# robotic-vision-lab/Edge-Informed-Contrast-Maximization

Measured on AMD Instinct MI355X. Metric: warped-events/sec/GPU + loss+grad eval ms, 1e6 events @ 346x260, higher is better.
Workload: dtype f32

## Files before the change

edge-informed-contrast-maximization_amd/csrc/eincm_api.hip:

```cpp
#include <hip/hip_runtime.h>
#include <hip/hip_ext.h>

#include <algorithm>
#include <array>
#include <chrono>
#include <cmath>
#include <cstdarg>
#include <cstdio>
#include <cstdlib>
#include <cstring>
#include <string>
#include <utility>
#include <vector>

#include "eincm.h"
#include "eincm_plan.h"
#include "eincm_kernels.hip.h"
#include "eincm_kernels_f64.hip.h"
#include "eincm_binning.hip.h"
#include "eincm_edges.hip.h"
#include "eincm_objectives.hip.h"
#include "eincm_splat_window.hip.h"
#include "eincm_canny.hip.h"
#include "eincm_preprocess.hip.h"
#include "eincm_gtflow.hip.h"
#include "eincm_dsec.hip.h"
#include "eincm_floweval.hip.h"
#include "eincm_bfgs.hip.h"
#include "eincm_lbfgs.hip.h"
#include "eincm_motion.hip.h"
#include "eincm_event_support.hip.h"
#include "eincm_event_filter.hip.h"
#include "eincm_event_scores.h"
#include "eincm_event_scores.hip.h"

using namespace eincm;

namespace {

thread_local std::string g_create_error;

struct Mem {
    struct Block { void* p; size_t bytes; };
    std::vector<Block> dev, pinned;
    size_t dev_bytes = 0, pinned_bytes = 0;

    template <typename T> hipError_t alloc_dev(T*& p, size_t n, bool zero = false) {
        p = nullptr;
        hipError_t e = hipMalloc(reinterpret_cast<void**>(&p), n * sizeof(T));
        if (e == hipSuccess && p && zero) e = hipMemset(p, 0, n * sizeof(T));
        return own(dev, dev_bytes, p, n * sizeof(T), e, hipFree);
    }
    template <typename T> hipError_t alloc_pinned(T*& p, size_t n, bool zero = false) {
        p = nullptr;
        const hipError_t e = hipHostMalloc(reinterpret_cast<void**>(&p), n * sizeof(T), hipHostMallocDefault);
        if (e == hipSuccess && p && zero) memset(p, 0, n * sizeof(T));
        return own(pinned, pinned_bytes, p, n * sizeof(T), e, hipHostFree);
    }
    void release(void* p) {
        if (!p) return;
        if (!drop(dev, dev_bytes, p, hipFree)) drop(pinned, pinned_bytes, p, hipHostFree);
    }
    void release_all() {
        for (const Block& b : dev) (void)hipFree(b.p);
        for (const Block& b : pinned) (void)hipHostFree(b.p);
        dev.clear(); pinned.clear();
        dev_bytes = pinned_bytes = 0;
    }

private:
    template <typename T> static hipError_t own(std::vector<Block>& v, size_t& total, T*& p, size_t bytes, hipError_t e, hipError_t (*free_fn)(void*)) {
        if (e != hipSuccess) { if (p) (void)free_fn(p); p = nullptr; return e; }
        if (p) { v.push_back(Block{p, bytes}); total += bytes; }
        return hipSuccess;
    }
    static bool drop(std::vector<Block>& v, size_t& total, void* p, hipError_t (*free_fn)(void*)) {
        for (size_t i = 0; i < v.size(); ++i)
            if (v[i].p == p) { (void)free_fn(p); total -= v[i].bytes; v.erase(v.begin() + i); return true; }
        return false;
    }
};

template <typename T, bool PINNED = false> struct Grow {
    T* p = nullptr;
    size_t n = 0;
};

struct StageArgs {
    int B, R; const int64_t* n_events;
    const int16_t* const* xs; const int16_t* const* ys; const double* const* ts; const double* const* edges; const double* edge_ts;
    uint32_t flags;
    const float* const* weights = nullptr;
};

struct StageScratch {
    std::vector<unsigned> cntmax; std::vector<double> dtmax;
    bool edge_ts_uploaded = false;
    std::vector<BinBlock> blks; std::vector<int32_t> win_blk; int32_t misc[4]; std::vector<double> mom;
    std::vector<uint32_t> sxy; std::vector<double> st; std::vector<float> ef; std::vector<float> sw;
    std::vector<int> ishift;
};

struct Flight {
    enum State { IDLE, FORWARD, LAUNCHED } state = IDLE;
    EvalPlan plan{};
    DevIo io{};
    const double* theta_dev = nullptr; ThetaArg targ{};
    int copy_mode = 0;
    int n_pieces = 0;
    size_t piece_len = 0;
    std::vector<uint8_t> theta_nan;
    bool timed_now = true;
    int ring_cur = 0;
    bool idle() const { return state == IDLE; }
    bool launched() const { return state == LAUNCHED; }
    void land() { state = IDLE; io = DevIo{}; }
    void abandon(hipStream_t stream) { (void)hipStreamSynchronize(stream); land(); }
};

}

struct eincm_ctx : PlanCtx {
    int device = 0;
    int maxR = 0, maxB = 0;
    int64_t maxN = 0;
    uint32_t cflags = 0;
    hipStream_t stream = nullptr;
    std::string err;
    Mem mem;

    bool staged = false;
    std::vector<int64_t> win_events;

    uint32_t* d_xy = nullptr;
    double* d_t = nullptr;
    uint32_t* d_xy_g = nullptr;
    double* d_t_g = nullptr;
    float* d_w = nullptr;
    float* d_w_g = nullptr;
    std::vector<int32_t> h_tilecount;
    bool policy_evaluated = false;
    int16_t* d_raw_x = nullptr; int16_t* d_raw_y = nullptr; double* d_raw_t = nullptr;
    BinBlock* d_binblocks = nullptr; int32_t* d_win_blk = nullptr; uint32_t* d_blockhist = nullptr;
    int32_t* d_tilecount = nullptr; int32_t* d_tilebase = nullptr; int32_t* d_bin_misc = nullptr;
    double* d_edges_raw = nullptr; double* d_edge_moments = nullptr;
    int64_t max_binblocks = 0;
    int64_t max_items = 0;
    float* d_edges = nullptr;
    double* d_edge_ts = nullptr;
    unsigned long long* d_acc = nullptr;
    float* d_iwe = nullptr;
    float* d_G = nullptr;
    float* d_zero_iwe = nullptr;
    double* d_Theta = nullptr;
    double* d_theta_in = nullptr;
    long long* d_gTheta = nullptr;
    double* d_g11 = nullptr;
    double* d_dtmax = nullptr;
    unsigned* d_gmax = nullptr;
    unsigned* d_cntmax = nullptr;
    unsigned* d_gticket = nullptr;
    double* d_tvg = nullptr;
    uint8_t* d_mask = nullptr;
    double* d_tmm = nullptr;
    StatPart* d_parts = nullptr;
    double* d_divparts = nullptr;
    double* d_g2parts = nullptr;
    Grow<float> d_gdiv;
    Grow<double> d_dgparts;
    double* d_tvparts = nullptr;
    WinConst* d_wc = nullptr;
    OutScal* d_outs = nullptr;
    Grow<long long> d_gth;
    double* d_grad = nullptr;
    Grow<double> d_AH, d_AW;
    int2* d_rowtap = nullptr; int2* d_coltap = nullptr;
    TileRange* d_tilerng = nullptr;
    int cur_h = -1, cur_w = -1, cur_method = -1;
    int64_t coarse_cap = 0;

    bool objc_valid = false;
    std::vector<ObjConst> h_objc;
    Grow<ObjConst> d_objc;
    Grow<double> d_oparts;
    Grow<double, true> h_ovals;

    Grow<char> scratch;
    struct {
        Grow<int32_t> p_nlm;
        std::vector<int32_t> h_pre_tab, h_nlm_tab;
        float nlm_hh = 0.0f;
        int nlm_tw = 0, nlm_sw = 0;
    } pre;
    struct {
        Grow<uint32_t> r_map;
        bool rect_map_set = false;
    } rect;
    struct {
        Grow<double> last_t;
        double last_time = es_no_event();
    } es;
    struct {
        Grow<double> maps;
        double last_time = es_no_event();
    } ef;
    struct {
        Grow<char> f_eval;
        int fe_n = 0;
        std::vector<int64_t> fe_ngt;
    } fe;

    double* h_theta = nullptr;
    double* h_grad = nullptr;
    OutScal* h_outs = nullptr;
    WinConst* h_wc = nullptr;
// ... 97 lines not shown
struct HostPhase {
    eincm_ctx* c; int phase; hp_clock::time_point t0;
    HostPhase(eincm_ctx* c_, int p) : c(c_), phase(p), t0(hp_clock::now()) {}
    ~HostPhase() { c->hp_us[phase] += std::chrono::duration<double, std::micro>(hp_clock::now() - t0).count(); }
};

int fail(eincm_ctx* c, int code, const char* fmt, ...) {
    char buf[512];
    va_list ap;
    va_start(ap, fmt);
    vsnprintf(buf, sizeof buf, fmt, ap);
    va_end(ap);
    if (c) c->err = buf; else g_create_error = buf;
    return code;
}

#define HIPCHK(c, expr)                                                                            \
    do {                                                                                           \
        hipError_t e_ = (expr);                                                                    \
        if (e_ != hipSuccess)                                                                      \
            return fail((c), EINCM_ERR_HIP, "%s failed: %s (%s:%d)", #expr, hipGetErrorString(e_), \
                        __FILE__, __LINE__);                                                       \
    } while (0)

template <typename T, bool PINNED> hipError_t ensure(eincm_ctx* c, Grow<T, PINNED>& g, size_t n, bool zero = false) {
    if (n <= g.n) return hipSuccess;
    if (const hipError_t e = hipStreamSynchronize(c->stream)) return e;
    c->mem.release(g.p);
    g.p = nullptr; g.n = 0;
    if (const hipError_t e = PINNED ? c->mem.alloc_pinned(g.p, n, zero) : c->mem.alloc_dev(g.p, n, zero)) return e;
    g.n = n;
    return hipSuccess;
}

hipError_t ensure_coarse(eincm_ctx* c, size_t cells) {
    if (const hipError_t e = ensure(c, c->d_gth, (size_t)2 * c->maxB * cells, true)) return e;
    c->coarse_cap = (int64_t)(c->d_gth.n / ((size_t)2 * c->maxB));
    return hipSuccess;
}

int not_in_flight(eincm_ctx* c, const char* who) {
    if (!c->fl.idle()) return fail(c, EINCM_ERR_STATE, "%s: an evaluation is in flight", who);
    return EINCM_OK;
}

struct FlightGuard {
    eincm_ctx* c; bool armed = true;
    explicit FlightGuard(eincm_ctx* c_) : c(c_) {}
    FlightGuard(const FlightGuard&) = delete;
    ~FlightGuard() { if (armed) c->fl.abandon(c->stream); }
    int keep(int rc = EINCM_OK) { armed = false; return rc; }
};

struct OneShot {
    eincm_ctx* c; size_t total = 0; bool pending = false;
    std::vector<std::vector<char>> host;
    explicit OneShot(eincm_ctx* c_) : c(c_) {}
    OneShot(const OneShot&) = delete;
    ~OneShot() { if (pending) (void)hipStreamSynchronize(c->stream); }
    template <typename T> struct Piece {
        const OneShot* op; size_t off; bool on;
        operator T*() const { return on ? reinterpret_cast<T*>(op->c->scratch.p + off) : nullptr; }
    };
    template <typename T> Piece<T> piece(size_t n, bool wanted = true) {
        const size_t off = total;
        if (wanted) total += (n * sizeof(T) + 255) & ~(size_t)255;
        return {this, off, wanted};
    }
    template <typename T> T* host_buf(size_t n) { host.emplace_back(n * sizeof(T), 0); return reinterpret_cast<T*>(host.back().data()); }
    hipError_t begin() { if (const hipError_t e = hipSetDevice(c->device)) return e; return ensure(c, c->scratch, total); }
    hipError_t up(void* dst, const void* src, size_t bytes) { pending = true; return hipMemcpyAsync(dst, src, bytes, hipMemcpyHostToDevice, c->stream); }
    hipError_t down(void* dst, const void* src, size_t bytes) { pending = true; return hipMemcpyAsync(dst, src, bytes, hipMemcpyDeviceToHost, c->stream); }
    hipError_t zero(void* dst, size_t bytes) { pending = true; return hipMemsetAsync(dst, 0, bytes, c->stream); }
    template <typename... P, typename... A> hipError_t launch(void (*k)(P...), dim3 grid, dim3 block, size_t lds, A&&... a) {
        pending = true;
        hipLaunchKernelGGL(k, grid, block, lds, c->stream, static_cast<P>(a)...);
        return hipGetLastError();
    }
    hipError_t sync() { pending = false; return hipStreamSynchronize(c->stream); }
};

const EvalKnobs& process_knobs() {
    static const EvalKnobs k{getenv("EINCM_NO_BIG_THETA_ARG") != nullptr, getenv("EINCM_NO_HOST_ASM") != nullptr,
                             getenv("EINCM_GATHER_ALL_R") ? atoi(getenv("EINCM_GATHER_ALL_R")) : -1};
    return k;
}
struct CreateKnobs { int seg = 0, seg_s = 0, wincap = 0; bool host_binning = false; };
CreateKnobs create_knobs() {
    CreateKnobs k;
    if (const char* s = getenv("EINCM_SEG")) k.seg = atoi(s);
    if (const char* s = getenv("EINCM_SEG_SPLAT")) k.seg_s = atoi(s);
    if (const char* s = getenv("EINCM_WINCAP")) k.wincap = atoi(s);
    k.host_binning = getenv("EINCM_HOST_BINNING") != nullptr;
    return k;
}
struct LiveKnobs { StageKnobs stage; bool no_proj_in_gather = false; };
LiveKnobs live_knobs() {
    LiveKnobs k;
    if (const char* e = getenv("EINCM_SEG_2DOF")) k.stage.seg_2 = atoi(e);
    if (const char* e = getenv("EINCM_PITCH_ALIGNED")) { k.stage.has_pitch = true; k.stage.pitch = atoi(e); }
    k.stage.no_segsort = getenv("EINCM_NO_SEGSORT") != nullptr;
    k.stage.no_spread = getenv("EINCM_NO_SPREAD") != nullptr;
    k.no_proj_in_gather = getenv("EINCM_NO_PROJ_IN_GATHER") != nullptr;
    return k;
}

void free_all(eincm_ctx* c) {
    if (c->have_events) {
        for (int k = 0; k < eincm_ctx::EV_RING; ++k)
            for (int i = 0; i <= EINCM_N_STAGES; ++i)
                for (int e = 0; e < 2; ++e)
                    if (c->ev[k][i][e]) { (void)hipEventDestroy(c->ev[k][i][e]); c->ev[k][i][e] = nullptr; }
        for (int k = 0; k < eincm_ctx::GRAD_PIECES; ++k) if (c->ev_piece[k]) { (void)hipEventDestroy(c->ev_piece[k]); c->ev_piece[k] = nullptr; }
        c->have_events = false;
    }
    if (c->stream) { (void)hipStreamDestroy(c->stream); c->stream = nullptr; }
    c->mem.release_all();
}

struct StageTimer {
    eincm_ctx* c; int stage; bool on, single;
    StageTimer(eincm_ctx* c_, int s, bool single_ = false) : c(c_), stage(s), on((c_->cflags & EINCM_CF_TIMING) != 0), single(single_) {
        if (on && single) c->attach_stage = stage;
        else if (on) { (void)hipEventRecord(c->ev[c->fl.ring_cur][stage][0], c->stream); }
    }
    ~StageTimer() {
        if (on && single) c->attach_stage = -1;
        else if (on) { (void)hipEventRecord(c->ev[c->fl.ring_cur][stage][1], c->stream); c->ev_used[c->fl.ring_cur][stage] = true; }
    }
};

static inline bool timing_on(const eincm_ctx* c) {
    return (c->cflags & EINCM_CF_TIMING) != 0 || ((c->cflags & EINCM_CF_TIMING_DOMINANT) != 0 && c->fl.timed_now);
}

template <typename K, typename... Args>
void launch_timed(eincm_ctx* c, int stage, K kernel, dim3 grid, dim3 block, size_t lds, Args... args) {
    const bool attach = (c->cflags & EINCM_CF_TIMING) ? c->attach_stage == stage
                      : ((c->cflags & EINCM_CF_TIMING_DOMINANT) && c->fl.timed_now) ? (stage == EINCM_STAGE_SPLAT ? c->time_splat : stage == EINCM_STAGE_GATHER && c->time_gather)
                      : false;
    if (attach) {
        hipExtLaunchKernelGGL(kernel, grid, block, (uint32_t)lds, c->stream, c->ev[c->fl.ring_cur][stage][0], c->ev[c->fl.ring_cur][stage][1], 0,
                              args...);
        c->ev_used[c->fl.ring_cur][stage] = true;
    } else {
        hipLaunchKernelGGL(kernel, grid, block, lds, c->stream, args...);
    }
}

int ensure_resample(eincm_ctx* c, int h, int w, int method) {
    if (c->cur_h == h && c->cur_w == w && c->cur_method == method) return EINCM_OK;
    static_assert(sizeof(Int2) == sizeof(int2) && sizeof(TileRange) == 4 * sizeof(int), "the tap tables go up as they are");
    ResampleTables t;
    build_resample(h, w, c->H, c->W, method, t);
    HIPCHK(c, ensure(c, c->d_AH, t.AH.size()));
    HIPCHK(c, ensure(c, c->d_AW, t.AW.size()));
    HIPCHK(c, hipMemcpyAsync(c->d_AH.p, t.AH.data(), t.AH.size() * sizeof(double), hipMemcpyHostToDevice, c->stream));
    HIPCHK(c, hipMemcpyAsync(c->d_AW.p, t.AW.data(), t.AW.size() * sizeof(double), hipMemcpyHostToDevice, c->stream));
    HIPCHK(c, hipMemcpyAsync(c->d_rowtap, t.rowtap.data(), t.rowtap.size() * sizeof(int2), hipMemcpyHostToDevice, c->stream));
    HIPCHK(c, hipMemcpyAsync(c->d_coltap, t.coltap.data(), t.coltap.size() * sizeof(int2), hipMemcpyHostToDevice, c->stream));
    HIPCHK(c, hipMemcpyAsync(c->d_tilerng, t.tilerng.data(), t.tilerng.size() * sizeof(TileRange), hipMemcpyHostToDevice, c->stream));
    c->proj_in_gather = t.fits && !live_knobs().no_proj_in_gather;
    HIPCHK(c, hipStreamSynchronize(c->stream));
    c->cur_h = h; c->cur_w = w; c->cur_method = method;
    return EINCM_OK;
}

int clear_accumulators(eincm_ctx* c) {
    const size_t img = (size_t)c->H * c->W;
    HIPCHK(c, hipMemsetAsync(c->d_acc, 0, (size_t)c->maxB * c->maxR * img * sizeof(unsigned long long), c->stream));
    HIPCHK(c, hipMemsetAsync(c->d_gTheta, 0, (size_t)c->maxB * img * 2 * sizeof(long long), c->stream));
    HIPCHK(c, hipMemsetAsync(c->d_gth.p, 0, (size_t)2 * c->maxB * c->coarse_cap * sizeof(long long), c->stream));
    c->acc_dirty = false;
    return EINCM_OK;
}

void launch_theta_image(eincm_ctx* c, int h, int w, bool identity, bool use_arg, const ThetaArgBig& targ, const double* theta_dev,
                        bool with_windows) {
    const Geom& g = c->g;
    const bool ww = with_windows && c->itembase_valid;
    auto go = [&](auto kernel, const auto& ta) {
        launch_timed(c, EINCM_STAGE_THETA, kernel, dim3(g.ntiles, g.B), dim3(NT), 0, g, h, w, identity ? 1 : 0, use_arg ? 1 : 0, ta,
                     theta_dev, c->d_AH.p, c->d_AW.p, c->d_rowtap, c->d_coltap, c->d_tilerng, c->d_Theta, c->d_tmm, c->d_edge_ts,
                     c->gather.n, c->gather.d_items, ww ? c->gather.d_itembase : nullptr, c->gather.d_wins,
                     c->splat.n, c->splat.d_items, ww ? c->splat.d_itembase : nullptr, c->splat.d_wins);
    };
    if (!use_arg || (size_t)g.B * h * w * 2 <= (size_t)THETA_ARG_MID) {
        ThetaArgMid mid;
        if (use_arg) memcpy(mid.v, targ.v, (size_t)g.B * h * w * 2 * sizeof(double));
        go(k_theta<ThetaArgMid>, mid);
    } else {
        go(k_theta<ThetaArgBig>, targ);
    }
    c->Theta_valid = true;
}

template <size_t... I> constexpr auto bind_splat(std::index_sequence<I...>) {
    return std::array{&k_splat<SPLAT_FORMS[I].mode, SPLAT_FORMS[I].threads, SPLAT_FORMS[I].weighted>...};
}
template <size_t... I> constexpr auto bind_splat_r(std::index_sequence<I...>) {
    return std::array{&k_splat_r<SPLAT_R_FORMS[I].mode, SPLAT_R_FORMS[I].rad>...};
}
template <size_t... I> constexpr auto bind_gather(std::index_sequence<I...>) {
    return std::array{&k_gather<GATHER_FORMS[I].mode, GATHER_FORMS[I].wide, GATHER_FORMS[I].threads, GATHER_FORMS[I].proj, GATHER_FORMS[I].all_r,
                                GATHER_FORMS[I].weighted>...};
}
template <size_t... I> constexpr auto bind_gather_r(std::index_sequence<I...>) {
    return std::array{&k_gather_r<GATHER_R_FORMS[I].mode, GATHER_R_FORMS[I].rad>...};
}
const auto SPLAT_KERNELS = bind_splat(std::make_index_sequence<std::size(SPLAT_FORMS)>{});
const auto SPLAT_R_KERNELS = bind_splat_r(std::make_index_sequence<std::size(SPLAT_R_FORMS)>{});
const auto GATHER_KERNELS = bind_gather(std::make_index_sequence<std::size(GATHER_FORMS)>{});
const auto GATHER_R_KERNELS = bind_gather_r(std::make_index_sequence<std::size(GATHER_R_FORMS)>{});
constexpr bool other_window_rows_plain() {
    for (const SplatKey& k : SPLAT_R_FORMS) if (k.threads != NT || k.weighted) return false;
    for (const GatherKey& k : GATHER_R_FORMS) if (k.threads != NT || k.wide || k.proj || k.all_r || k.weighted) return false;
    return true;
}
static_assert(other_window_rows_plain(), "a row of SPLAT_R_FORMS / GATHER_R_FORMS names a kernel that k_splat_r / k_gather_r are not");

int no_such_form(eincm_ctx* c, const char* kernel, const GatherKey& k) {
    return fail(c, EINCM_ERR_UNSUPPORTED, "internal: the library holds no %s kernel for theta mode %d, splat radius %d, wide %d, %d threads, "
                "proj %d, all_r %d, weighted %d (eincm_plan.h)", kernel, k.mode, k.rad, k.wide, k.threads, k.proj, k.all_r, k.weighted);
}

int launch_splat(eincm_ctx* c, const double* theta_dev, const ThetaArg& targ) {
    const EvalPlan& P = c->fl.plan;
    const SplatForm& F = P.splat;
    {
        StageTimer t(c, EINCM_STAGE_SPLAT, true);
        if (c->splat.n > 0) {
            if (F.row < 0) return no_such_form(c, "splat", GatherKey{F.key.mode, F.key.rad, 0, F.key.threads, 0, 0, F.key.weighted});
            const SegList& L = seg_list(*c, F.list);
            Geom gs = c->g;
            gs.wincap = F.wincap; gs.winmaxw = F.winmaxw;
            const dim3 grid(L.grid(gs.R)), block(F.key.threads);
            const int use_arg = P.use_arg ? 1 : 0;
            if (F.key.rad == 1)
                launch_timed(c, EINCM_STAGE_SPLAT, SPLAT_KERNELS[F.row], grid, block, F.lds, gs, L.n, L.d_items, c->d_xy, c->d_t, c->d_Theta,
                             c->d_edge_ts, c->splat.d_wins, c->d_acc, L.d_order, use_arg, theta_dev, targ,
                             (const float*)(F.key.weighted ? c->d_w : nullptr));
            else
                launch_timed(c, EINCM_STAGE_SPLAT, SPLAT_R_KERNELS[F.row], grid, block, F.lds, gs, L.n, L.d_items, c->d_xy, c->d_t, c->d_Theta,
                             c->d_tmm, c->d_edge_ts, c->d_acc, L.d_order, use_arg, theta_dev, targ);
        }
    }
    HIPCHK(c, hipGetLastError());
    c->fl.theta_dev = theta_dev; c->fl.targ = targ;
    return EINCM_OK;
}

int launch_forward(eincm_ctx* c, const double* theta_host) {
    const EvalPlan& P = c->fl.plan;
    const Geom& g = c->g;
    const bool two_dof = P.shape == EvalPlan::TWO_DOF;
    const size_t nall = (size_t)g.B * P.nth;
    c->acc_dirty = true;
    if (P.shape == EvalPlan::MOTION) {
        auto& mo = c->motion;
        ThetaArg ta{};
        ta.v[0] = mo.model.cx; ta.v[1] = mo.model.cy; ta.v[2] = mo.model.scale;
        const size_t nq = (size_t)g.B * MOTION_NQ;
        if (P.use_arg) memcpy(ta.v + POLY_ARG_Q0, theta_host, nq * sizeof(double));
        else memcpy(mo.h_q(c->maxB), theta_host, nq * sizeof(double));
        mo.last_q.assign(theta_host, theta_host + nq);
        c->last_theta11.clear();
        c->Theta_valid = false;
        return launch_splat(c, mo.h_q(c->maxB), ta);
    }
    ThetaArg targ;
    static thread_local ThetaArgBig targ_big;
    if (P.use_arg_big) memcpy(targ_big.v, theta_host, nall * sizeof(double));
    if (P.use_arg) memcpy(targ.v, theta_host, nall * sizeof(double));
    const double* theta_dev = P.use_arg ? c->d_theta_in : c->h_theta;
    if (P.theta_src == EvalPlan::THETA_DEVICE) {
        theta_dev = c->fl.io.theta;
    } else if (P.theta_src == EvalPlan::THETA_PINNED) {
        memcpy(c->h_theta, theta_host, nall * sizeof(double));
        theta_dev = c->h_theta;
    } else if (P.theta_src == EvalPlan::THETA_PIECES) {
        StageTimer t(c, EINCM_STAGE_COPY);
        const size_t piece = std::max<size_t>((nall + 5) / 6, (size_t)32768);
        for (size_t off = 0; off < nall; off += piece) {
            const size_t n = std::min(piece, nall - off);
            memcpy(c->h_theta + off, theta_host + off, n * sizeof(double));
            HIPCHK(c, hipMemcpyAsync(c->d_theta_in + off, c->h_theta + off, n * sizeof(double), hipMemcpyHostToDevice, c->stream));
        }
        theta_dev = c->d_theta_in;
    }
    {
        StageTimer t(c, EINCM_STAGE_THETA, two_dof ? !P.need_theta_image : c->itembase_valid);
        const SegList &ga = c->gather, &sp = c->splat;
        const int nwin_threads = (ga.n + sp.n) * g.R;
        if (two_dof) {
            if (theta_host) c->last_theta11.assign(theta_host, theta_host + (size_t)g.B * 2); else c->last_theta11.clear();
            c->motion.last_q.clear();
            c->Theta_valid = false;
            if (P.need_theta_image) launch_theta_image(c, P.h, P.w, false, P.use_arg_big, targ_big, theta_dev, false);
            if (!P.host_asm)
                launch_timed(c, EINCM_STAGE_THETA, k_theta_const, dim3((std::max(g.B * g.ntiles, nwin_threads) + NT - 1) / NT), dim3(NT), 0, g,
                                   P.use_arg ? 1 : 0, targ, theta_dev, c->d_tmm, c->d_edge_ts, ga.n, ga.d_items, ga.d_wins,
                                   sp.n, sp.d_items, sp.d_wins);
        } else {
            launch_theta_image(c, P.h, P.w, P.shape == EvalPlan::IDENTITY, P.use_arg_big, targ_big, theta_dev, true);
            if (nwin_threads > 0 && !c->itembase_valid)
                hipLaunchKernelGGL(k_windows, dim3((nwin_threads + NT - 1) / NT), dim3(NT), 0, c->stream, g, c->d_tmm, c->d_edge_ts,
                                   ga.n, ga.d_items, ga.d_wins, sp.n, sp.d_items, sp.d_wins);
        }
    }
    return launch_splat(c, theta_dev, targ);
}

int read_event_slot(eincm_ctx* c, int k) {
    memset(&c->last_t, 0, sizeof c->last_t);
    for (int s = 0; s <= EINCM_N_STAGES; ++s) {
        if (!c->ev_used[k][s]) continue;
        float ms = 0.f;
        HIPCHK(c, hipEventElapsedTime(&ms, c->ev[k][s][0], c->ev[k][s][1]));
        if (s < EINCM_N_STAGES) c->last_t.ms[s] = ms; else c->last_t.total_ms = ms;
    }
    for (int s = 0; s < EINCM_N_STAGES; ++s) c->sum_t.ms[s] += c->last_t.ms[s];
    c->sum_t.total_ms += c->last_t.total_ms;
    ++c->sum_n;
    return EINCM_OK;
}
int drain_event_ring(eincm_ctx* c, int keep) {
    while (c->ring_n > keep) {
// ... 223 lines not shown
    return EINCM_OK;
}

int eval_end_launch(eincm_ctx* c) {
    if (c->fl.idle()) return fail(c, EINCM_ERR_STATE, "no evaluation in flight");
    if (c->fl.launched()) return EINCM_OK;
    FlightGuard guard(c);
    HostPhase hp(c, EINCM_HP_LAUNCH);
    const EvalPlan& P = c->fl.plan;
    const EvalParams& ep = P.ep;
    Geom g = c->g;
    const bool identity = P.shape == EvalPlan::IDENTITY, want_grad = P.want_grad, host_asm = P.host_asm;
    const bool timing = timing_on(c);
    const int n_imwg = (g.nig + IG_NT / 64 - 1) / (IG_NT / 64);
    g.gmax_n = g.R * g.nig;
    {
        StageTimer t(c, EINCM_STAGE_STATS, P.stream_stats);
        if (P.stream_stats) {
            g.nparts = NSPART;
            launch_timed(c, EINCM_STAGE_STATS, k_stats_stream, dim3(NSPART, g.R, g.B), dim3(NT), 0, g, c->d_acc, c->d_iwe, c->d_edges,
                         c->d_parts);
        } else {
            g.nparts = g.ntiles;
            const size_t ntot = (size_t)g.B * g.R * g.H * g.W;
            hipLaunchKernelGGL(k_iwe_finish, dim3((unsigned)std::min<size_t>((ntot + NT - 1) / NT, 2048)), dim3(NT), 0, c->stream, g,
                               c->d_acc, c->d_iwe);
            hipLaunchKernelGGL(k_stats, dim3(g.ntiles, g.R, g.B), dim3(NT), 0, c->stream, g, c->d_iwe, c->d_edges, c->d_parts,
                               P.g2_from_imgrad ? 0 : 1);
        }
        c->last_nparts = g.nparts;
    }

    if (ep.want_div) {
        hipLaunchKernelGGL(k_div, dim3(g.ntiles, g.R, g.B), dim3(NT), 0, c->stream, g, c->d_iwe, c->d_parts, c->d_divparts);
    }
    if (ep.want_tv) {
        StageTimer t(c, EINCM_STAGE_TV, true);
        auto go = [&](auto kernel) {
            launch_timed(c, EINCM_STAGE_TV, kernel, dim3(g.ntiles, g.B), dim3(NT), 0, g, c->d_Theta, c->d_mask, c->d_tvg, c->d_tvparts,
                         P.full_aux ? 1 : 0, P.h, P.w, c->d_AH.p, c->d_AW.p, c->d_tilerng, c->d_gth.p + (size_t)c->maxB * c->coarse_cap,
                         (int)c->coarse_cap, host_asm ? c->h_tvparts : nullptr);
        };
        P.tv_proj ? go(k_tv<1>) : go(k_tv<0>);
    }
    if (P.obj && !want_grad) {
        const ObjGeom& og = P.og;
        hipLaunchKernelGGL(k_obj_parts, dim3(og.ncells, g.R, g.B), dim3(NT), 0, c->stream, g, og, c->d_iwe, 1, c->d_edges, c->d_oparts.p);
        hipLaunchKernelGGL(k_obj_grad, dim3(1, g.R, g.B), dim3(IG_NT), 0, c->stream, g, ep, og, c->d_iwe, c->d_edges, c->d_oparts.p,
                           c->d_wc, c->d_objc.p, c->d_gdiv.p, c->d_dgparts.p, c->d_G, c->d_gmax, c->h_ovals.p, 0);
    }
    if (want_grad) {
        {
            StageTimer t(c, EINCM_STAGE_IMGRAD, !P.div_grad && !P.obj);
            if (P.div_grad)
                hipLaunchKernelGGL(k_divgrad, dim3(g.ntiles, g.R, g.B), dim3(NT), 0, c->stream, g, c->d_iwe, c->d_parts,
                                   c->d_gdiv.p, c->d_dgparts.p);
            if (P.obj) {
                const ObjGeom& og = P.og;
                hipLaunchKernelGGL(k_obj_parts, dim3(og.ncells, g.R, g.B), dim3(NT), 0, c->stream, g, og, c->d_iwe, 1, c->d_edges, c->d_oparts.p);
                hipLaunchKernelGGL(k_obj_grad, dim3(n_imwg, g.R, g.B), dim3(IG_NT), 0, c->stream, g, ep, og, c->d_iwe, c->d_edges, c->d_oparts.p,
                                   c->d_wc, c->d_objc.p, c->d_gdiv.p, c->d_dgparts.p, c->d_G, c->d_gmax, c->h_ovals.p, 1);
            } else {
                launch_timed(c, EINCM_STAGE_IMGRAD, k_imgrad, dim3(n_imwg, g.R, g.B), dim3(IG_NT), 0, g, ep, c->d_iwe, c->d_edges,
                                   c->d_parts, c->d_wc, c->d_gdiv.p, c->d_dgparts.p, host_asm ? c->h_g2 : c->d_g2parts, c->d_G, c->d_gmax,
                                   host_asm ? c->h_img : nullptr, host_asm ? 1 : 0);
            }
        }
        {
            StageTimer t(c, EINCM_STAGE_GATHER, true);
            if (c->gather.n > 0) {
                const GatherForm& F = P.gather;
                if (F.row < 0) return no_such_form(c, "gather", F.key);
                const SegList& L = seg_list(*c, F.list);
                const bool own_copy = F.copy == EventCopy::GATHER;
                const uint32_t* xy_g = own_copy ? c->d_xy_g : c->d_xy;
                const double* t_g = own_copy ? c->d_t_g : c->d_t;
                Geom gg = g;
                gg.pitch_aligned = F.pitch_aligned; gg.wincap_a = F.wincap; gg.winmaxw_a = F.winmaxw;
                const dim3 grid(L.grid(F.wg_per_seg)), block(F.key.threads);
                double* g11 = P.shape == EvalPlan::MOTION ? c->motion.h_fpart.p : host_asm ? c->h_g11 : c->d_g11;
                const int use_arg = P.use_arg ? 1 : 0;
                if (F.key.rad == 1)
                    launch_timed(c, EINCM_STAGE_GATHER, GATHER_KERNELS[F.row], grid, block, F.lds, gg, L.n, L.d_items, xy_g, t_g, c->d_Theta,
                                 c->d_edge_ts, c->d_G, c->gather.d_wins, c->d_gTheta, g11, c->d_wc, c->d_gmax, L.d_order, use_arg,
                                 c->fl.theta_dev, c->fl.targ, P.h, P.w, c->d_AH.p, c->d_AW.p, c->d_tilerng, c->d_gth.p, (int)c->coarse_cap,
                                 P.grid_tail ? 1 : 0, c->d_gticket, c->gather.d_win_item0, c->h_grad,
                                 (P.grid_tail && ep.use_tv_grad) ? ep.gamma : 0.0, c->d_tvparts, c->d_gth.p + (size_t)c->maxB * c->coarse_cap,
                                 (const float*)(F.key.weighted ? (own_copy ? c->d_w_g : c->d_w) : nullptr));
                else
                    launch_timed(c, EINCM_STAGE_GATHER, GATHER_R_KERNELS[F.row], grid, block, F.lds, gg, L.n, L.d_items, xy_g, t_g, c->d_Theta,
                                 c->d_tmm, c->d_edge_ts, c->d_G, c->d_gTheta, g11, c->d_wc, c->d_gmax, c->stage.wide ? 1 : 0, use_arg,
                                 c->fl.theta_dev, c->fl.targ);
            }
        }
        if (P.nsrc > 0) {
            StageTimer t(c, EINCM_STAGE_PROJECT, true);
            launch_timed(c, EINCM_STAGE_PROJECT, k_project, dim3(g.ntiles, g.B, P.nsrc), dim3(NT), 0, g, P.h, P.w,
                               (int)c->coarse_cap, P.events_projected ? 1 : 0, c->stage.wide ? 1 : 0, c->d_AH.p, c->d_AW.p, c->d_rowtap, c->d_coltap, c->d_gTheta, c->d_tvg,
                               c->d_wc, c->d_gmax, c->d_gth.p, c->d_gth.p + (size_t)c->maxB * c->coarse_cap);
        }
    }
    if (!host_asm) {
        StageTimer t(c, EINCM_STAGE_FINAL, !(want_grad && identity));
        launch_timed(c, EINCM_STAGE_FINAL, k_final, dim3(g.B), dim3(FT), 0, g, ep, c->d_parts, c->d_divparts, c->d_tvparts,
                           P.shape == EvalPlan::MOTION ? c->motion.tmm_zero.p : c->d_tmm, c->d_wc, P.g2_from_imgrad ? c->d_g2parts : nullptr, c->d_gth.p, c->d_gth.p + (size_t)c->maxB * c->coarse_cap, (int)c->coarse_cap,
                           c->d_g11, c->gather_2.d_win_item0, c->gather_2.n, c->d_gmax,
                           P.zero_copy_out ? c->h_outs : c->d_outs, P.zero_copy_out ? c->h_grad : c->d_grad, want_grad ? 1 : 0);
        if (want_grad && identity) {
            hipLaunchKernelGGL(k_final_dense, dim3(256, g.B), dim3(NT), 0, c->stream, g, ep.use_tv_grad, c->stage.wide ? 1 : 0, c->d_gTheta,
                               c->d_tvg, c->d_wc, c->d_gmax, c->d_outs, c->d_grad);
        }
    }
    HIPCHK(c, hipGetLastError());
    c->fl.n_pieces = 0;
    c->fl.copy_mode = (P.zero_copy_out || host_asm) ? 0 : 1;
    if (c->fl.copy_mode && !c->device_results) { const int rcc = enqueue_result_copies(c); if (rcc) return rcc; c->fl.copy_mode = 0; }
    if (timing && c->ring_size == 1) { (void)hipEventRecord(c->ev[c->fl.ring_cur][EINCM_N_STAGES][1], c->stream); c->ev_used[c->fl.ring_cur][EINCM_N_STAGES] = true; }
    c->fl.state = Flight::LAUNCHED;
    c->acc_dirty = false;
    return guard.keep();
}

int eval_end_collect(eincm_ctx* c, double* value, double* grad, eincm_aux* aux) {
    if (!c->fl.launched()) return fail(c, EINCM_ERR_STATE, "no evaluation in flight");
    FlightGuard guard(c);
    Flight& fl = c->fl;
    const Geom& g = c->g;
    const bool want_grad = fl.plan.want_grad;
    const size_t nth = fl.plan.nth, total = (size_t)g.B * nth;
    if (fl.copy_mode) { fl.copy_mode = 0; if (const int rcc = enqueue_result_copies(c)) return rcc; }
    bool nonfinite = false;
    if (fl.n_pieces > 0 && want_grad && grad) {
        for (int k = 0; k < fl.n_pieces; ++k) {
            if (hipEventSynchronize(c->ev_piece[k]) != hipSuccess) break;
            const size_t off = (size_t)k * fl.piece_len;
            if (copy_scan_finite(grad + off, c->h_grad + off, std::min(fl.piece_len, total - off))) nonfinite = true;
        }
    }
    {
        HostPhase hp(c, EINCM_HP_WAIT);
        HIPCHK(c, hipStreamSynchronize(c->stream));
    }
    const bool dev_io = fl.io.theta != nullptr || fl.plan.shape == EvalPlan::MOTION;
    fl.land();
    guard.keep();
    ++c->hp_n;
    const bool whole_grad = want_grad && fl.n_pieces == 0 && !dev_io;
    if (want_grad && !grad && !dev_io) return fail(c, EINCM_ERR_ARG, "the evaluation was begun with a gradient but grad is NULL");
    HostPhase hp(c, EINCM_HP_COLLECT);
    const LossView v = loss_view(c);
    if (fl.plan.host_asm) host_assemble(v);
    else if (c->fp64) f64_assemble(v);
    if (fl.plan.obj) obj_assemble(v);
    if (const int rc = collect_timings(c)) return rc;
    c->have_eval = true;
    c->G_valid = want_grad;

    if (hand_over(v, whole_grad, value, aux)) nonfinite = true;
    if (whole_grad && copy_scan_finite(grad, c->h_grad, total)) nonfinite = true;
    if (nonfinite) return fail(c, EINCM_ERR_NONFINITE, "loss or gradient is not finite");
    return EINCM_OK;
}

int eval_end(eincm_ctx* c, double* value, double* grad, eincm_aux* aux) {
    if (!c->fl.idle() && c->fl.plan.want_grad && !grad) {
        c->fl.abandon(c->stream);
        return fail(c, EINCM_ERR_ARG, "the evaluation was begun with a gradient but grad is NULL");
    }
// ... 62 lines not shown

int window_constants(eincm_ctx* c) {
    if (const int rc = preset_constants(c)) return rc;
    const std::vector<double> zero((size_t)c->g.B * 2, 0.0);
    std::vector<double> val((size_t)c->g.B);
    const eincm_params p = zero_pass_params();
    const int rc = evaluate(c, zero.data(), 1, 1, &p, val.data(), nullptr, nullptr);
    if (rc != EINCM_OK && rc != EINCM_ERR_NONFINITE) c->staged = false;
    return store_constants(c, rc);
}

}

extern "C" {

int eincm_abi_version(void) { return EINCM_ABI_VERSION; }

const char* eincm_last_error(const eincm_ctx* ctx) { return ctx ? ctx->err.c_str() : g_create_error.c_str(); }

int eincm_multi_ref_weights(int n_refs, double* w) {
    if (n_refs < 1 || n_refs > EINCM_MAX_REFS || !w) return EINCM_ERR_ARG;
    multi_ref_weights(n_refs, w);
    return EINCM_OK;
}

int eincm_resample_matrix(int n_in, int n_out, int method, double* A) {
    if (n_in < 1 || n_out < 1 || !A || method < 0 || method > EINCM_METHOD_CUBIC) return EINCM_ERR_ARG;
    std::vector<double> M;
    resample_matrix(n_in, n_out, method, M);
    memcpy(A, M.data(), M.size() * sizeof(double));
    return EINCM_OK;
}

eincm_ctx* eincm_create(int device, int H, int W, int max_refs, int max_windows, int64_t max_events_total, uint32_t flags) {
    if (H < 3 || W < 3 || H > 32767 || W > 32767 || max_refs < 1 || max_refs > EINCM_MAX_REFS || max_windows < 1 ||
        max_events_total < 1 || max_events_total > (int64_t)2000000000) {
        fail(nullptr, EINCM_ERR_ARG, "eincm_create: bad argument (H=%d W=%d max_refs=%d max_windows=%d max_events=%lld)",
             H, W, max_refs, max_windows, (long long)max_events_total);
        return nullptr;
    }
    int ndev = 0;
    hipError_t e = hipGetDeviceCount(&ndev);
    if (e != hipSuccess || ndev < 1) {
        fail(nullptr, EINCM_ERR_HIP, "eincm_create: no HIP device visible (%s); this engine has no CPU fallback",
             hipGetErrorString(e));
        return nullptr;
    }
    if (device < 0 || device >= ndev) {
        fail(nullptr, EINCM_ERR_ARG, "eincm_create: device %d out of range (0..%d)", device, ndev - 1);
        return nullptr;
    }
    if ((flags & EINCM_CF_FP64) && (flags & (EINCM_CF_TIMING | EINCM_CF_TIMING_DOMINANT))) {
        fail(nullptr, EINCM_ERR_UNSUPPORTED, "eincm_create: the timing flags are not supported with EINCM_CF_FP64");
        return nullptr;
    }
    eincm_ctx* c = new eincm_ctx();
    c->fp64 = (flags & EINCM_CF_FP64) != 0;
    c->device = device; c->H = H; c->W = W; c->maxR = max_refs; c->maxB = max_windows; c->maxN = max_events_total;
    c->cflags = flags;
    auto bail = [&](const char* what, hipError_t err) -> eincm_ctx* {
        fail(nullptr, EINCM_ERR_HIP, "eincm_create: %s failed: %s", what, hipGetErrorString(err));
        free_all(c);
        delete c;
        return nullptr;
    };
#define TRY(expr) do { hipError_t e2_ = (expr); if (e2_ != hipSuccess) return bail(#expr, e2_); } while (0)
    TRY(hipSetDevice(device));
    TRY(hipStreamCreateWithFlags(&c->stream, hipStreamNonBlocking));
    const int tilesX = (W + TS - 1) / TS, tilesY = (H + TS - 1) / TS, ntiles = tilesX * tilesY;
    const size_t B = max_windows, R = max_refs, img = (size_t)H * W;
    const CreateKnobs k = create_knobs();
    if (k.seg >= MIN_SEG && k.seg <= MAX_SEG) c->seg = k.seg;
    if (k.seg_s >= MIN_SEG && k.seg_s <= MAX_CHUNK) c->seg_s = k.seg_s;
    if (k.wincap >= 1024 && k.wincap <= 6912) { c->wincap = (k.wincap / 4) * 4; c->wincap_fixed = true; }
    c->host_binning = (ntiles > BIN_MAX_TILES) || k.host_binning;
    c->max_items = (int64_t)B * ntiles + max_events_total / MIN_SEG + 1;
    TRY(c->mem.alloc_dev(c->d_xy, (size_t)max_events_total));
    TRY(c->mem.alloc_dev(c->d_t, (size_t)max_events_total));
    TRY(c->mem.alloc_dev(c->d_xy_g, (size_t)max_events_total));
    TRY(c->mem.alloc_dev(c->d_t_g, (size_t)max_events_total));
    for (SegList* L : {&c->gather, &c->splat, &c->splat_sh, &c->gather_2}) {
        TRY(c->mem.alloc_dev(L->d_items, (size_t)c->max_items));
        TRY(c->mem.alloc_dev(L->d_order, (size_t)c->max_items));
    }
    for (SegList* L : {&c->gather, &c->gather_2}) TRY(c->mem.alloc_dev(L->d_win_item0, B + 1));
    for (SegList* L : {&c->gather, &c->splat}) {
        TRY(c->mem.alloc_dev(L->d_wins, (size_t)c->max_items * max_refs));
        if (!c->host_binning) TRY(c->mem.alloc_dev(L->d_itembase, B * ntiles));
    }
    TRY(c->mem.alloc_dev(c->d_raw_x, (size_t)max_events_total));
    TRY(c->mem.alloc_dev(c->d_raw_y, (size_t)max_events_total));
    TRY(c->mem.alloc_dev(c->d_raw_t, (size_t)max_events_total));
    if (!c->host_binning) {
        c->max_binblocks = max_events_total / BIN_CHUNK + (int64_t)B + 1;
        TRY(c->mem.alloc_dev(c->d_binblocks, (size_t)c->max_binblocks));
        TRY(c->mem.alloc_dev(c->d_win_blk, B + 1));
        TRY(c->mem.alloc_dev(c->d_blockhist, (size_t)c->max_binblocks * ntiles));
        TRY(c->mem.alloc_dev(c->d_tilecount, B * ntiles));
        TRY(c->mem.alloc_dev(c->d_tilebase, B * ntiles));
        TRY(c->mem.alloc_dev(c->d_bin_misc, (size_t)8));
        TRY(c->mem.alloc_dev(c->d_edges_raw, B * R * img));
        TRY(c->mem.alloc_dev(c->d_edge_moments, B * R * EDGE_PARTS * EDGE_MOM));
    }
    TRY(c->mem.alloc_dev(c->d_edges, B * R * img));
    TRY(c->mem.alloc_dev(c->d_edge_ts, B * R));
    TRY(c->mem.alloc_dev(c->d_acc, B * R * img, true));
    TRY(c->mem.alloc_dev(c->d_iwe, B * R * img));
    TRY(c->mem.alloc_dev(c->d_G, B * R * img));
    TRY(c->mem.alloc_dev(c->d_g11, (size_t)(c->max_items + NXCD) * R * 2));
    TRY(c->mem.alloc_dev(c->d_dtmax, B));
    TRY(c->mem.alloc_dev(c->d_cntmax, B));
    const size_t nig = (size_t)((W + IG_COLS - 1) / IG_COLS) * ((H + IG_ROWS - 1) / IG_ROWS);
    TRY(c->mem.alloc_dev(c->d_gmax, B * R * nig, true));
    TRY(c->mem.alloc_dev(c->d_zero_iwe, B * img));
    TRY(c->mem.alloc_dev(c->d_Theta, B * img * 2));
    TRY(c->mem.alloc_dev(c->d_theta_in, B * img * 2));
    TRY(c->mem.alloc_dev(c->d_gTheta, B * img * 2, true));
    TRY(c->mem.alloc_dev(c->d_tvg, B * img * 2));
    TRY(c->mem.alloc_dev(c->d_mask, B * img));
    TRY(c->mem.alloc_dev(c->d_tmm, B * ntiles * 4));
    const size_t pstride = (size_t)std::max(ntiles, NSPART);
    TRY(c->mem.alloc_dev(c->d_parts, B * R * pstride));
    TRY(c->mem.alloc_dev(c->d_gticket, B, true));
    TRY(c->mem.alloc_dev(c->d_divparts, B * R * ntiles));
    TRY(c->mem.alloc_dev(c->d_g2parts, B * R * nig));
    TRY(c->mem.alloc_dev(c->d_tvparts, B * ntiles * 3));
    TRY(c->mem.alloc_dev(c->d_wc, B));
    {
        char* blk = nullptr;
        TRY(c->mem.alloc_dev(blk, B * sizeof(OutScal) + B * img * 2 * sizeof(double)));
        c->d_outs = reinterpret_cast<OutScal*>(blk);
        c->d_grad = reinterpret_cast<double*>(blk + B * sizeof(OutScal));
        char* hblk = nullptr;
        TRY(c->mem.alloc_pinned(hblk, B * sizeof(OutScal) + B * img * 2 * sizeof(double)));
        c->h_outs = reinterpret_cast<OutScal*>(hblk);
        c->h_grad = reinterpret_cast<double*>(hblk + B * sizeof(OutScal));
    }
    TRY(ensure_coarse(c, 64 * 64 * 2));
    TRY(c->mem.alloc_dev(c->d_rowtap, (size_t)H));
    TRY(c->mem.alloc_dev(c->d_coltap, (size_t)W));
    TRY(c->mem.alloc_dev(c->d_tilerng, (size_t)ntiles));
    TRY(c->mem.alloc_pinned(c->h_theta, B * img * 2));
    TRY(c->mem.alloc_pinned(c->h_wc, B));
    TRY(c->mem.alloc_pinned(c->h_g11, (size_t)(c->max_items + NXCD) * R * 2));
    TRY(c->mem.alloc_pinned(c->h_g2, B * R * nig));
    TRY(c->mem.alloc_pinned(c->h_img, B * R * IMGSCAL_N));
    TRY(c->mem.alloc_pinned(c->h_tvparts, B * ntiles * 3));
    c->have_events = true;
    for (int k = 0; k < eincm_ctx::GRAD_PIECES; ++k) TRY(hipEventCreateWithFlags(&c->ev_piece[k], hipEventDisableTiming));
    c->ring_size = (flags & EINCM_CF_TIMING_DOMINANT) && !(flags & EINCM_CF_TIMING) ? eincm_ctx::EV_RING : 1;
    if (flags & (EINCM_CF_TIMING | EINCM_CF_TIMING_DOMINANT))
        for (int k = 0; k < c->ring_size; ++k)
            for (int i = 0; i <= EINCM_N_STAGES; ++i) {
                const bool needed = (flags & EINCM_CF_TIMING) || i == EINCM_STAGE_SPLAT || i == EINCM_STAGE_GATHER || i == EINCM_N_STAGES;
                if (needed) { TRY(hipEventCreate(&c->ev[k][i][0])); TRY(hipEventCreate(&c->ev[k][i][1])); }
            }
    if (c->fp64) {
        const int P = (int)((img + F64_PIX - 1) / F64_PIX);
        c->f64.P = P;
        TRY(c->mem.alloc_dev(c->f64.acc, B * R * img, true));
        TRY(c->mem.alloc_dev(c->f64.iwe, B * R * img));
        TRY(c->mem.alloc_dev(c->f64.zero_iwe, B * img));
        TRY(c->mem.alloc_dev(c->f64.edges, B * R * img));
        TRY(c->mem.alloc_dev(c->f64.G, B * R * img));
        TRY(c->mem.alloc_dev(c->f64.sgn, B * R * img));
        TRY(c->mem.alloc_dev(c->f64.gacc, B * img * 4, true));
        TRY(c->mem.alloc_dev(c->f64.gTh, B * img * 2));
        TRY(c->mem.alloc_dev(c->f64.T, B * img * 2));
        TRY(c->mem.alloc_dev(c->f64.grad, B * img * 2));
        TRY(c->mem.alloc_dev(c->f64.partA, B * R * P * F64_PA));
        TRY(c->mem.alloc_dev(c->f64.partB, B * R * P * F64_PB));
        TRY(c->mem.alloc_dev(c->f64.partC, B * R * P * F64_PC));
        TRY(c->mem.alloc_dev(c->f64.scal, B * R));
        TRY(c->mem.alloc_pinned(c->f64.h_scal, B * R));
        TRY(c->mem.alloc_dev(c->f64.gmax, B));
        TRY(c->mem.alloc_dev(c->f64.ishift, B));
        TRY(c->mem.alloc_dev(c->f64.bad, B));
    }
#undef TRY
    return c;
}

void eincm_destroy(eincm_ctx* ctx) {
    if (!ctx) return;
    (void)hipSetDevice(ctx->device);
    if (ctx->stream) (void)hipStreamSynchronize(ctx->stream);
    free_all(ctx);
    delete ctx;
}

static int build_list(eincm_ctx* c, SegList& L, int seg, bool on_host, int ntiles, const double* ev_t, int64_t N)
{
    std::vector<int32_t> lens;
    cut_segments(c->h_tilecount.data(), c->h_tilecount.size(), ntiles, seg, N, on_host, L, lens);
    if ((int64_t)lens.size() > c->max_items) return fail(c, EINCM_ERR_ARG, "internal: %zu segments exceed capacity", lens.size());
    if (on_host) L.n = (int)lens.size();
    else if ((int)lens.size() != L.n) return fail(c, EINCM_ERR_ARG, "internal: segment lists disagree (%zu, %d)", lens.size(), L.n);
    if (on_host) {
        if (L.d_win_item0)
            HIPCHK(c, hipMemcpyAsync(L.d_win_item0, L.h_win_item0.data(), L.h_win_item0.size() * sizeof(int32_t), hipMemcpyHostToDevice, c->stream));
        if (L.n > 0) HIPCHK(c, hipMemcpyAsync(L.d_items, L.h_items.data(), (size_t)L.n * sizeof(Item), hipMemcpyHostToDevice, c->stream));
    }
    if (L.n == 0) return EINCM_OK;
    HIPCHK(c, hipMemcpyAsync(L.d_order, L.h_order.data(), (size_t)L.n * sizeof(int32_t), hipMemcpyHostToDevice, c->stream));
    hipLaunchKernelGGL(k_seg_minmax, dim3(std::min(L.n, 4096)), dim3(NT), 0, c->stream, L.n, L.d_items, ev_t);
    HIPCHK(c, hipGetLastError());
    return EINCM_OK;
}


static int check_staging(eincm_ctx* c, const StageArgs& a) {
    if (!c) return EINCM_ERR_ARG;
    if (c->fl.launched())
        return fail(c, EINCM_ERR_STATE, "an asynchronous evaluation is in flight: call eincm_loss_grad_wait first");
    if (a.B < 1 || a.B > c->maxB) return fail(c, EINCM_ERR_ARG, "n_windows %d outside 1..%d", a.B, c->maxB);
    if (a.R < 1 || a.R > c->maxR) return fail(c, EINCM_ERR_ARG, "n_refs %d outside 1..%d", a.R, c->maxR);
    if (!a.n_events || !a.xs || !a.ys || !a.ts || !a.edges || !a.edge_ts) return fail(c, EINCM_ERR_ARG, "null pointer argument");
    for (int b = 0; b < a.B; ++b)
        if (!a.edges[b] || (a.n_events[b] > 0 && (!a.xs[b] || !a.ys[b] || !a.ts[b]))) return fail(c, EINCM_ERR_ARG, "null pointer argument (window %d)", b);
    int64_t N = 0;
    for (int b = 0; b < a.B; ++b) {
        if (a.n_events[b] < 0) return fail(c, EINCM_ERR_ARG, "n_events[%d] negative", b);
        N += a.n_events[b];
    }
    if (N > c->maxN) return fail(c, EINCM_ERR_ARG, "total events %lld exceed capacity %lld", (long long)N, (long long)c->maxN);
    for (int b = 0; b < a.B; ++b)
        for (int r = 0; r < a.R; ++r)
            if (!std::isfinite(a.edge_ts[b * a.R + r])) return fail(c, EINCM_ERR_ARG, "edge_ts[%d,%d] is not finite", b, r);
    if (c->fp64) {
        if (a.flags & EINCM_SW_DEFER_CONSTANTS) return fail(c, EINCM_ERR_UNSUPPORTED, "event-sharded staging is not supported in fp64 mode");
        for (int b = 0; b < a.B; ++b)
            if (f64_ishift(a.n_events[b]) < 40)
                return fail(c, EINCM_ERR_UNSUPPORTED, "window %d: %lld events exceed the fp64 mode's IWE scale (2^-40 per tap)", b, (long long)a.n_events[b]);
    }
    if (const WeightRefusal r = check_weights(a.B, a.n_events, a.weights))
        return fail(c, EINCM_ERR_ARG, "weight %lld of window %d is %g: weights are finite and within [0, 1]", (long long)r.index, r.win, (double)r.value);
    if (batch_weighted(a.B, a.n_events, a.weights)) {
        if (c->fp64) return fail(c, EINCM_ERR_UNSUPPORTED, "per-event weights are not supported in fp64 mode (EINCM_CF_FP64)");
        if (c->splat_size != 3)
            return fail(c, EINCM_ERR_UNSUPPORTED, "per-event weights have the 3x3 splat window only, the context has %d (eincm_set_splat_window)", c->splat_size);
        if (a.flags & EINCM_SW_DEFER_CONSTANTS) return fail(c, EINCM_ERR_UNSUPPORTED, "per-event weights are not supported in an event-sharded staging");
    }
    return EINCM_OK;
}

static int ensure_weights(eincm_ctx* c) {
    if (!c->d_w) HIPCHK(c, c->mem.alloc_dev(c->d_w, (size_t)c->maxN));
    if (!c->d_w_g) HIPCHK(c, c->mem.alloc_dev(c->d_w_g, (size_t)c->maxN));
    return EINCM_OK;
}

static int refuse_event(eincm_ctx* c, const StageArgs& a, int b, int64_t i, bool bad_xy) {
    if (!bad_xy) return fail(c, EINCM_ERR_ARG, "event %lld of window %d has a non-finite timestamp", (long long)i, b);
    return fail(c, EINCM_ERR_ARG, "event %lld of window %d at (x=%d, y=%d) outside the %dx%d sensor", (long long)i, b, (int)a.xs[b][i],
                (int)a.ys[b][i], c->H, c->W);
}
static int refuse_event_at(eincm_ctx* c, const StageArgs& a, int64_t e, bool bad_xy) {
    int b = 0;
    while (b < a.B - 1 && e >= a.n_events[b]) { e -= a.n_events[b]; ++b; }
    return refuse_event(c, a, b, e, bad_xy);
}

static int upload_raw_events(eincm_ctx* c, const StageArgs& a) {
    int64_t off = 0;
    for (int b = 0; b < a.B; ++b) {
        const size_t nb = (size_t)a.n_events[b];
        if (nb > 0) {
            HIPCHK(c, hipMemcpyAsync(c->d_raw_x + off, a.xs[b], nb * sizeof(int16_t), hipMemcpyHostToDevice, c->stream));
            HIPCHK(c, hipMemcpyAsync(c->d_raw_y + off, a.ys[b], nb * sizeof(int16_t), hipMemcpyHostToDevice, c->stream));
            HIPCHK(c, hipMemcpyAsync(c->d_raw_t + off, a.ts[b], nb * sizeof(double), hipMemcpyHostToDevice, c->stream));
        }
        off += (int64_t)nb;
    }
    return EINCM_OK;
}

static int upload_raw_weights(eincm_ctx* c, const StageArgs& a) {
    int64_t off = 0;
    for (int b = 0; b < a.B; ++b) {
        const size_t nb = (size_t)a.n_events[b];
        if (nb > 0 && a.weights[b]) HIPCHK(c, hipMemcpyAsync(c->d_w_g + off, a.weights[b], nb * sizeof(float), hipMemcpyHostToDevice, c->stream));
        else if (nb > 0) HIPCHK(c, hipMemsetD32Async(reinterpret_cast<hipDeviceptr_t>(c->d_w_g + off), 0x3f800000 , nb, c->stream));
        off += (int64_t)nb;
    }
    return EINCM_OK;
}

static int copy_for_gather(eincm_ctx* c) {
// ... 1 lines not shown
    const bool wt = c->stage.weighted;
    if (c->stage.sort_segments) {
        const dim3 grid(std::min(c->gather.n, 8192));
        if (wt) hipLaunchKernelGGL(k_segsort<1>, grid, dim3(SORT_NT), 0, c->stream, c->gather.n, c->gather.d_items,
                                   c->d_xy, c->d_t, c->d_xy_g, c->d_t_g, (const float*)c->d_w, c->d_w_g);
        else hipLaunchKernelGGL(k_segsort<0>, grid, dim3(SORT_NT), 0, c->stream, c->gather.n, c->gather.d_items,
                                c->d_xy, c->d_t, c->d_xy_g, c->d_t_g, (const float*)nullptr, (float*)nullptr);
        return EINCM_OK;
    }
    if (wt) HIPCHK(c, hipMemcpyAsync(c->d_w_g, c->d_w, (size_t)c->stage.N * sizeof(float), hipMemcpyDeviceToDevice, c->stream));
    HIPCHK(c, hipMemcpyAsync(c->d_xy_g, c->d_xy, (size_t)c->stage.N * sizeof(uint32_t), hipMemcpyDeviceToDevice, c->stream));
    HIPCHK(c, hipMemcpyAsync(c->d_t_g, c->d_t, (size_t)c->stage.N * sizeof(double), hipMemcpyDeviceToDevice, c->stream));
    return EINCM_OK;
}

static int bin_on_device(eincm_ctx* c, const StageArgs& a, StageScratch& sc) {
    const StagePlan& P = c->stage;
    const Geom& g = P.g;
    const size_t img = (size_t)g.H * g.W;
    int rc = EINCM_OK;
    sc.win_blk.resize((size_t)a.B + 1);
    int64_t base = 0;
    for (int b = 0; b < a.B; ++b) {
        sc.win_blk[b] = (int32_t)sc.blks.size();
        for (int64_t s0 = 0; s0 < a.n_events[b]; s0 += BIN_CHUNK) {
            BinBlock bb; bb.win = b; bb.start = (int32_t)(base + s0); bb.count = (int32_t)std::min<int64_t>(BIN_CHUNK, a.n_events[b] - s0);
            bb.first_blk = sc.win_blk[b];
            sc.blks.push_back(bb);
        }
        base += a.n_events[b];
    }
    sc.win_blk[a.B] = (int32_t)sc.blks.size();
    const int nblk = (int)sc.blks.size();
    if (nblk > c->max_binblocks) return fail(c, EINCM_ERR_ARG, "internal: %d staging blocks exceed capacity", nblk);
    static const int32_t misc_init[4] = {0, 0, 0x7fffffff, 0x7fffffff};
    HIPCHK(c, hipMemcpyAsync(c->d_bin_misc, misc_init, sizeof misc_init, hipMemcpyHostToDevice, c->stream));
    HIPCHK(c, hipMemcpyAsync(c->d_win_blk, sc.win_blk.data(), sc.win_blk.size() * sizeof(int32_t), hipMemcpyHostToDevice, c->stream));
    for (int b = 0; b < a.B; ++b)
        HIPCHK(c, hipMemcpyAsync(c->d_edges_raw + (size_t)b * a.R * img, a.edges[b], (size_t)a.R * img * sizeof(double), hipMemcpyHostToDevice, c->stream));
    hipLaunchKernelGGL(k_edges, dim3(EDGE_PARTS, a.R, a.B), dim3(NT), 0, c->stream, g, c->d_edges_raw, c->d_edges, c->d_edge_moments);
    if (nblk > 0) {
        HIPCHK(c, hipMemcpyAsync(c->d_binblocks, sc.blks.data(), sc.blks.size() * sizeof(BinBlock), hipMemcpyHostToDevice, c->stream));
        if ((rc = upload_raw_events(c, a))) return rc;
        hipLaunchKernelGGL(k_bin_hist, dim3(nblk), dim3(BIN_NT), g.ntiles * sizeof(uint32_t), c->stream, g, c->d_binblocks, c->d_raw_x, c->d_raw_y,
                           c->d_raw_t, c->d_blockhist, c->d_bin_misc + 2);
    } else {
        HIPCHK(c, hipMemsetAsync(c->d_blockhist, 0, sizeof(uint32_t), c->stream));
    }
    const int M = a.B * g.ntiles;
    hipLaunchKernelGGL(k_bin_scan, dim3((M + 255) / 256), dim3(256), 0, c->stream, g, c->d_win_blk, c->d_blockhist, c->d_tilecount);
    hipLaunchKernelGGL(k_bin_tilescan, dim3(1), dim3(1024), 0, c->stream, M, P.seg, c->d_tilecount, c->d_tilebase, c->gather.d_itembase, c->d_bin_misc);
    HIPCHK(c, hipGetLastError());
    sc.mom.resize((size_t)a.B * a.R * EDGE_PARTS * EDGE_MOM);
    HIPCHK(c, hipMemcpyAsync(sc.misc, c->d_bin_misc, sizeof sc.misc, hipMemcpyDeviceToHost, c->stream));
    HIPCHK(c, hipMemcpyAsync(sc.mom.data(), c->d_edge_moments, sc.mom.size() * sizeof(double), hipMemcpyDeviceToHost, c->stream));
    c->h_tilecount.resize((size_t)M);
    HIPCHK(c, hipMemcpyAsync(c->h_tilecount.data(), c->d_tilecount, (size_t)M * sizeof(int32_t), hipMemcpyDeviceToHost, c->stream));
    HIPCHK(c, hipStreamSynchronize(c->stream));
    if (sc.misc[2] != 0x7fffffff) return refuse_event_at(c, a, sc.misc[2], true);
    if (sc.misc[3] != 0x7fffffff) return refuse_event_at(c, a, sc.misc[3], false);
    c->gather.n = sc.misc[1];
    if (c->gather.n > c->max_items) return fail(c, EINCM_ERR_ARG, "internal: %d segments exceed capacity", c->gather.n);
    for (int b = 0; b < a.B; ++b)
        for (int r = 0; r < a.R; ++r) {
            double sE = 0.0, sEE = 0.0, eabs = 0.0;
            for (int k = 0; k < EDGE_PARTS; ++k) {
                const double* m = &sc.mom[(((size_t)b * a.R + r) * EDGE_PARTS + k) * EDGE_MOM];
                sE += m[0]; sEE += m[1]; eabs = std::max(eabs, m[2]);
            }
            c->h_wc[b].sE[r] = sE; c->h_wc[b].sEE[r] = sEE; c->h_wc[b].eabs[r] = eabs;
        }
    if (nblk > 0) {
        if (P.weighted) {
            if ((rc = upload_raw_weights(c, a))) return rc;
            hipLaunchKernelGGL(k_bin_scatter<1>, dim3(nblk), dim3(BIN_NT), g.ntiles * sizeof(uint32_t), c->stream, g, c->d_binblocks, c->d_raw_x,
                               c->d_raw_y, c->d_raw_t, c->d_blockhist, c->d_tilebase, c->d_xy, c->d_t, (const float*)c->d_w_g, c->d_w);
        } else
        hipLaunchKernelGGL(k_bin_scatter<0>, dim3(nblk), dim3(BIN_NT), g.ntiles * sizeof(uint32_t), c->stream, g, c->d_binblocks, c->d_raw_x, c->d_raw_y,
                           c->d_raw_t, c->d_blockhist, c->d_tilebase, c->d_xy, c->d_t, (const float*)nullptr, (float*)nullptr);
        hipLaunchKernelGGL(k_items, dim3((M + 255) / 256), dim3(256), 0, c->stream, g, P.seg, c->d_tilecount, c->d_tilebase, c->gather.d_itembase,
                           c->gather.d_items);
        if ((rc = copy_for_gather(c))) return rc;
    }
    if ((rc = build_list(c, c->gather, P.seg, false, g.ntiles, c->d_t_g, P.N))) return rc;
    c->splat.n = 0;
    if (nblk > 0) {
        if (P.spread && P.weighted)
            hipLaunchKernelGGL(k_spread<1>, dim3(M, SPREAD_Y), dim3(256), 0, c->stream, g, c->d_tilecount, c->d_tilebase, c->d_xy, c->d_t, c->d_w);
        else if (P.spread)
            hipLaunchKernelGGL(k_spread<0>, dim3(M, SPREAD_Y), dim3(256), 0, c->stream, g, c->d_tilecount, c->d_tilebase, c->d_xy, c->d_t, (float*)nullptr);
        HIPCHK(c, hipMemcpyAsync(c->d_edge_ts, a.edge_ts, (size_t)a.B * a.R * sizeof(double), hipMemcpyHostToDevice, c->stream));
        sc.edge_ts_uploaded = true;
        hipLaunchKernelGGL(k_win_consts, dim3(a.B), dim3(NT), 0, c->stream, g, c->gather.n, c->gather.d_items, c->gather.d_itembase,
                           c->d_edge_ts, c->gather.d_win_item0, c->d_dtmax);
        HIPCHK(c, hipMemcpyAsync(sc.dtmax.data(), c->d_dtmax, (size_t)a.B * sizeof(double), hipMemcpyDeviceToHost, c->stream));
        hipLaunchKernelGGL(k_bin_tilescan, dim3(1), dim3(1024), 0, c->stream, M, P.seg_s, c->d_tilecount, c->d_tilebase, c->splat.d_itembase, c->d_bin_misc);
        for (const int32_t cnt : c->h_tilecount) c->splat.n += (cnt + P.seg_s - 1) / P.seg_s;
        if (c->splat.n > c->max_items) return fail(c, EINCM_ERR_ARG, "internal: %d splat segments exceed capacity", c->splat.n);
        hipLaunchKernelGGL(k_items, dim3((M + 255) / 256), dim3(256), 0, c->stream, g, P.seg_s, c->d_tilecount, c->d_tilebase, c->splat.d_itembase,
                           c->splat.d_items);
    } else {
        HIPCHK(c, hipMemsetAsync(c->gather.d_win_item0, 0, (size_t)(a.B + 1) * sizeof(int32_t), c->stream));
    }
    return build_list(c, c->splat, P.seg_s, false, g.ntiles, c->d_t, P.N);
}

static int bin_on_host(eincm_ctx* c, const StageArgs& a, StageScratch& sc) {
    const StagePlan& P = c->stage;
    const Geom& g = P.g;
    const size_t img = (size_t)g.H * g.W;
    int rc = EINCM_OK;
    if (const EventRefusal r = bin_events(g, a.n_events, a.xs, a.ys, a.ts, a.edge_ts, P.N, c->h_tilecount, sc.sxy, sc.st, sc.cntmax, sc.dtmax,
                                          a.weights, P.weighted ? &sc.sw : nullptr))
        return refuse_event(c, a, r.win, r.index, r.bad_xy);
    sc.ef.resize((size_t)a.B * a.R * img);
    for (int b = 0; b < a.B; ++b) {
        WinConst& wc = c->h_wc[b];
        for (int r = 0; r < a.R; ++r)
            edge_moments(a.edges[b] + (size_t)r * img, img, sc.ef.data() + ((size_t)b * a.R + r) * img, wc.sE[r], wc.sEE[r], wc.eabs[r]);
    }
    if (P.N > 0) {
        HIPCHK(c, hipMemcpyAsync(c->d_xy, sc.sxy.data(), (size_t)P.N * sizeof(uint32_t), hipMemcpyHostToDevice, c->stream));
        HIPCHK(c, hipMemcpyAsync(c->d_t, sc.st.data(), (size_t)P.N * sizeof(double), hipMemcpyHostToDevice, c->stream));
        if (P.weighted) HIPCHK(c, hipMemcpyAsync(c->d_w, sc.sw.data(), (size_t)P.N * sizeof(float), hipMemcpyHostToDevice, c->stream));
        if ((rc = upload_raw_events(c, a))) return rc;
    }
    if ((rc = build_list(c, c->gather, P.seg, true, g.ntiles, c->d_t, P.N))) return rc;
    if ((rc = copy_for_gather(c))) return rc;
    if ((rc = build_list(c, c->splat, P.seg_s, true, g.ntiles, c->d_t, P.N))) return rc;
    HIPCHK(c, hipMemcpyAsync(c->d_edges, sc.ef.data(), sc.ef.size() * sizeof(float), hipMemcpyHostToDevice, c->stream));
    return EINCM_OK;
}

static int finish_lists(eincm_ctx* c, const StageArgs& a, StageScratch& sc) {
    const StagePlan& P = c->stage;
    const Geom& g = P.g;
    int rc = EINCM_OK;
    if (!sc.edge_ts_uploaded)
        HIPCHK(c, hipMemcpyAsync(c->d_edge_ts, a.edge_ts, (size_t)a.B * a.R * sizeof(double), hipMemcpyHostToDevice, c->stream));
    HIPCHK(c, hipMemsetAsync(c->d_mask, 0, (size_t)a.B * g.H * g.W, c->stream));
    if ((rc = build_list(c, c->gather_2, P.seg_2, true, g.ntiles, c->d_t, P.N))) return rc;
    c->splat_sh.n = 0;
    if (P.splat_short && (rc = build_list(c, c->splat_sh, SEG_SHORT, true, g.ntiles, c->d_t, P.N))) return rc;
    if (c->gather.n > 0 && !P.host_binning) {
        HIPCHK(c, hipMemsetAsync(c->d_cntmax, 0, (size_t)a.B * sizeof(unsigned), c->stream));
        hipLaunchKernelGGL(k_tile_counts, dim3(g.ntiles, a.B), dim3(NT), 0, c->stream, g, c->d_tilebase, c->d_tilecount, c->d_xy,
                           c->d_mask, c->d_cntmax, (const float*)(P.weighted ? c->d_w : nullptr));
        HIPCHK(c, hipGetLastError());
        HIPCHK(c, hipMemcpyAsync(sc.cntmax.data(), c->d_cntmax, (size_t)a.B * sizeof(unsigned), hipMemcpyDeviceToHost, c->stream));
    }
    HIPCHK(c, hipStreamSynchronize(c->stream));
    c->policy_evaluated = false;
    c->g = g;
    c->itembase_valid = !P.host_binning && c->gather.n > 0 && c->splat.n > 0;
    c->win_events.assign(a.n_events, a.n_events + a.B);
    if (c->gather.n > 0 && P.host_binning) {
        hipLaunchKernelGGL(k_mask, dim3(std::min(c->gather.n, 2048)), dim3(NT), 0, c->stream, g, c->gather.d_items, c->gather.n, c->d_xy, c->d_mask,
                           (const float*)(P.weighted ? c->d_w : nullptr));
        HIPCHK(c, hipGetLastError());
    }
    return EINCM_OK;
}

static int stage_fp64(eincm_ctx* c, const StageArgs& a, StageScratch& sc) {
    const size_t img = (size_t)c->H * c->W;
    for (int b = 0; b < a.B; ++b) sc.ishift.push_back(f64_ishift(a.n_events[b]));
    HIPCHK(c, hipMemcpyAsync(c->f64.ishift, sc.ishift.data(), sc.ishift.size() * sizeof(int), hipMemcpyHostToDevice, c->stream));
    for (int b = 0; b < a.B; ++b)
        HIPCHK(c, hipMemcpyAsync(c->f64.edges + (size_t)b * a.R * img, a.edges[b], (size_t)a.R * img * sizeof(double), hipMemcpyHostToDevice, c->stream));
    return EINCM_OK;
}

static int stage_windows(eincm_ctx* c, const StageArgs& a) {
    int rc = check_staging(c, a);
    if (rc) return rc;
    c->staged = false;
    c->objc_valid = false;
    c->Theta_valid = false;
    c->motion.last_q.clear(); c->motion.seg0.clear();
    c->bfgs.begun = false;
    c->stage = plan_staging(*c, a.B, a.R, a.n_events, a.flags, live_knobs().stage, a.weights);
    const StagePlan& P = c->stage;
    HIPCHK(c, hipSetDevice(c->device));
    if (P.weighted && (rc = ensure_weights(c))) return rc;
    StageScratch sc;
    struct DrainOnExit { hipStream_t s; ~DrainOnExit() { (void)hipStreamSynchronize(s); } } drain_on_exit{c->stream};
    if (c->acc_dirty && (rc = clear_accumulators(c))) return rc;
    for (int b = 0; b < a.B; ++b) {
        memset(&c->h_wc[b], 0, sizeof(WinConst));
        multi_ref_weights(a.R, c->h_wc[b].mrw);
    }
    sc.cntmax.assign((size_t)a.B, 0u);
    sc.dtmax.assign((size_t)a.B, 0.0);
    if ((rc = P.host_binning ? bin_on_host(c, a, sc) : bin_on_device(c, a, sc))) return rc;
    if ((rc = finish_lists(c, a, sc))) return rc;
    if (c->fp64 && (rc = stage_fp64(c, a, sc))) return rc;
    for (int b = 0; b < a.B; ++b) {
        WinConst& wc = c->h_wc[b];
        wc.nev = (double)std::max<int64_t>(a.n_events[b], 1);
        wc.cntmax = (double)std::max(sc.cntmax[b], 1u);
        wc.dtmax = sc.dtmax[b];
    }
    c->staged = true;
    c->have_eval = false;
    c->err.clear();
    c->sharded_staging = P.defer_constants;
    if (!P.defer_constants) return window_constants(c);
    if ((rc = preset_constants(c))) return rc;
    c->constants_pending = true;
    HIPCHK(c, hipStreamSynchronize(c->stream));
    return EINCM_OK;
}

int eincm_set_windows_ex(eincm_ctx* c, int n_windows, int n_refs, const int64_t* n_events, const int16_t* xs, const int16_t* ys,
                         const double* ts, const double* edges, const double* edge_ts, uint32_t flags) {
    const bool sane = c && n_events && xs && ys && ts && edges && n_windows >= 1 && n_windows <= c->maxB;
    const size_t nb = sane ? (size_t)n_windows : 0, img = c ? (size_t)c->H * c->W : 0;
    std::vector<const int16_t*> xw(nb), yw(nb);
    std::vector<const double*> tw(nb), ew(nb);
    int64_t base = 0;
    for (size_t b = 0; b < nb; ++b) {
        xw[b] = xs + base; yw[b] = ys + base; tw[b] = ts + base; ew[b] = edges + b * (size_t)std::max(n_refs, 0) * img;
        base += std::max<int64_t>(n_events[b], 0);
    }
    return stage_windows(c, StageArgs{n_windows, n_refs, n_events, sane ? xw.data() : nullptr, sane ? yw.data() : nullptr,
                                      sane ? tw.data() : nullptr, sane ? ew.data() : nullptr, edge_ts, flags});
}

int eincm_set_windows(eincm_ctx* c, int n_windows, int n_refs, const int64_t* n_events, const int16_t* xs, const int16_t* ys,
                      const double* ts, const double* edges, const double* edge_ts) {
    return eincm_set_windows_ex(c, n_windows, n_refs, n_events, xs, ys, ts, edges, edge_ts, 0u);
}

int eincm_set_windows_ptrs(eincm_ctx* c, int n_windows, int n_refs, const int64_t* n_events, const int16_t* const* xs,
                           const int16_t* const* ys, const double* const* ts, const double* const* edges, const double* edge_ts,
                           uint32_t flags) {
    return stage_windows(c, StageArgs{n_windows, n_refs, n_events, xs, ys, ts, edges, edge_ts, flags});
}
// ... 1700 lines not shown
```

edge-informed-contrast-maximization_amd/csrc/eincm_binning.hip.h:

```cpp
#pragma once
#include <hip/hip_runtime.h>
#include <stdint.h>

#include "eincm_kernels.hip.h"

namespace eincm {

constexpr int BIN_CHUNK = 1024;
constexpr int BIN_NT = 64;
constexpr int BIN_TRIPS = BIN_CHUNK / BIN_NT;
constexpr int BIN_MAX_TILES = 12288;

struct BinBlock { int32_t win, start, count, first_blk; };

__global__ __launch_bounds__(BIN_NT) void k_bin_hist(Geom g, const BinBlock* __restrict__ blks, const int16_t* __restrict__ xs,
                                                  const int16_t* __restrict__ ys, const double* __restrict__ ts,
                                                  uint32_t* __restrict__ blockhist, int* __restrict__ err)
{
    extern __shared__ uint32_t hist[];
    const BinBlock bb = blks[blockIdx.x];
    uint32_t xy[BIN_TRIPS]; double tt[BIN_TRIPS];
#pragma unroll
    for (int k = 0; k < BIN_TRIPS; ++k) {
        const int i = k * BIN_NT + (int)threadIdx.x;
// ... 197 lines not shown
        for (int q = 0; q < 4; ++q)
#pragma unroll
            for (int w = 0; w < SORT_NW; ++w) { c[q][w] = cnt[w][4 * threadIdx.x + q]; tot += c[q][w]; }
        wsum[threadIdx.x] = tot;
        __syncthreads();
        for (int off = 1; off < SORT_NT; off <<= 1) {
            const uint32_t v = (threadIdx.x >= off) ? wsum[threadIdx.x - off] : 0u;
            __syncthreads();
            wsum[threadIdx.x] += v;
            __syncthreads();
        }
        uint32_t run = wsum[threadIdx.x] - tot;
#pragma unroll
        for (int q = 0; q < 4; ++q)
#pragma unroll
            for (int w = 0; w < SORT_NW; ++w) { cnt[w][4 * threadIdx.x + q] = run; run += c[q][w]; }
        __syncthreads();
        const SegLayout L(n);
        uint32_t nxy = 0u; double nt = 0.0; float nw = 0.0f;
        if (lo + lane < hi) { nxy = src_xy[begin + lo + lane]; nt = src_t[begin + lo + lane]; if (WT) nw = src_w[begin + lo + lane]; }
        for (int i0 = lo; i0 < hi; i0 += 64) {
            const int i = i0 + lane;
            const bool valid = i < hi;
            const uint32_t xy = nxy; const double t = nt; const float wgt = nw;
            if (i + 64 < hi) { nxy = src_xy[begin + i + 64]; nt = src_t[begin + i + 64]; if (WT) nw = src_w[begin + i + 64]; }
            const int key = valid ? (int)pixkey(xy) : -1;
            unsigned long long grp = __ballot(valid);
#pragma unroll
            for (int bit = 0; bit < SORT_KEY_BITS; ++bit) {
                const bool one = ((key >> bit) & 1) != 0;
                const unsigned long long bal = __ballot(one);
                grp &= one ? bal : ~bal;
            }
            uint32_t rank = 0u, base = 0u;
            if (valid) { base = cnt[wv][key]; rank = base + (uint32_t)__popcll(grp & lt_mask); }
            __builtin_amdgcn_wave_barrier();
            if (valid && (grp & lt_mask) == 0ull) cnt[wv][key] = base + (uint32_t)__popcll(grp);
            __builtin_amdgcn_wave_barrier();
            if (valid) {
                const int pos = L.position((int)rank);
                dst_xy[begin + pos] = xy;
                dst_t[begin + pos] = t;
                if (WT) dst_w[begin + pos] = wgt;
            }
        }
        __syncthreads();
    }
}

__global__ void k_items(Geom g, int seg, const int32_t* __restrict__ tilecount, const int32_t* __restrict__ tilebase,
                        const int32_t* __restrict__ itembase, Item* __restrict__ items)
{
    const int idx = blockIdx.x * blockDim.x + threadIdx.x;
    if (idx >= g.B * g.ntiles) return;
    const int c = tilecount[idx], base = tilebase[idx];
    int k = itembase[idx];
    const int len = balanced_seg_len(c, seg);
    for (int s = 0; s < c; s += len, ++k) {
        Item it;
        it.win = idx / g.ntiles; it.tile = idx % g.ntiles; it.begin = base + s; it.count = min(len, c - s);
        it.t_lo = 0.0; it.t_hi = 0.0;
        items[k] = it;
    }
}

__global__ __launch_bounds__(NT) void k_seg_minmax(int n_items, Item* __restrict__ items, const double* __restrict__ ev_t)
{
    __shared__ double smn[NWAVE], smx[NWAVE];
    for (int k = blockIdx.x; k < n_items; k += gridDim.x) {
        const int begin = items[k].begin, count = items[k].count;
        double mn = INFINITY, mx = -INFINITY;
        for (int i = threadIdx.x; i < count; i += NT) { const double t = ev_t[begin + i]; mn = fmin(mn, t); mx = fmax(mx, t); }
        mn = wave_min(mn); mx = wave_max(mx);
        __syncthreads();
        if ((threadIdx.x & 63) == 0) { smn[threadIdx.x >> 6] = mn; smx[threadIdx.x >> 6] = mx; }
        __syncthreads();
        if (threadIdx.x == 0) {
            for (int i = 1; i < NWAVE; ++i) { mn = fmin(mn, smn[i]); mx = fmax(mx, smx[i]); }
            items[k].t_lo = mn; items[k].t_hi = mx;
        }
    }
}

constexpr int EDGE_PARTS = 32;
constexpr int EDGE_MOM = 3;
__global__ __launch_bounds__(NT) void k_edges(Geom g, const double* __restrict__ src, float* __restrict__ dst, double* __restrict__ moments)
{
    __shared__ double scratch[NWAVE];
    const int r = blockIdx.y, b = blockIdx.z;
    const size_t n = (size_t)g.H * g.W, base = ((size_t)b * g.R + r) * n;
    double s = 0.0, ss = 0.0, mx = 0.0;
    for (size_t i = (size_t)blockIdx.x * NT + threadIdx.x; i < n; i += (size_t)gridDim.x * NT) {
        const float f = (float)src[base + i];
        dst[base + i] = f;
        s += (double)f; ss += (double)f * (double)f;
        mx = fmax(mx, fabs((double)f));
    }
    s = block_sum(s, scratch);
    ss = block_sum(ss, scratch);
    mx = wave_max(mx);
    __syncthreads();
    if ((threadIdx.x & 63) == 0) scratch[threadIdx.x >> 6] = mx;
    __syncthreads();
    if (threadIdx.x == 0) {
        for (int i = 1; i < NWAVE; ++i) mx = fmax(mx, scratch[i]);
        double* o = moments + (((size_t)b * g.R + r) * EDGE_PARTS + blockIdx.x) * EDGE_MOM;
        o[0] = s; o[1] = ss; o[2] = mx;
    }
}

__global__ __launch_bounds__(NT) void k_win_consts(Geom g, int n_items, const Item* __restrict__ items, const int32_t* __restrict__ itembase,
                                                    const double* __restrict__ edge_ts, int32_t* __restrict__ win_item0,
                                                    double* __restrict__ dtmax)
{
    __shared__ double smn[NWAVE], smx[NWAVE];
    const int b = blockIdx.x;
    const int lo = itembase[(size_t)b * g.ntiles], hi = (b + 1 < g.B) ? itembase[(size_t)(b + 1) * g.ntiles] : n_items;
    double mn = INFINITY, mx = -INFINITY;
    for (int k = lo + threadIdx.x; k < hi; k += NT) { mn = fmin(mn, items[k].t_lo); mx = fmax(mx, items[k].t_hi); }
    mn = wave_min(mn); mx = wave_max(mx);
    if ((threadIdx.x & 63) == 0) { smn[threadIdx.x >> 6] = mn; smx[threadIdx.x >> 6] = mx; }
    __syncthreads();
    if (threadIdx.x == 0) {
        for (int i = 1; i < NWAVE; ++i) { mn = fmin(mn, smn[i]); mx = fmax(mx, smx[i]); }
        double d = 0.0;
        if (hi > lo)
            for (int r = 0; r < g.R; ++r) { const double tau = edge_ts[b * g.R + r]; d = fmax(d, fmax(fabs(mn - tau), fabs(mx - tau))); }
        win_item0[b] = lo;
        dtmax[b] = d;
    }
}

}
```

edge-informed-contrast-maximization_amd/csrc/eincm_kernels.hip.h:

```cpp
#pragma once
#include <hip/hip_runtime.h>
#include <stdint.h>

#include "eincm_types.h"
#include "eincm_loss.h"

namespace eincm {

constexpr int NWAVE = NT / 64;
constexpr int WIN_CAP_MAX = 9216;
constexpr float INV_2PI = 0.15915494309189535f;
constexpr int MAX_CHUNK = 16384;
__device__ __forceinline__ int fix_shift(int count) {
    const unsigned c = (unsigned)ceilf((float)count * 0.16f);
    const int ceillog2 = (c <= 1u) ? 0 : (32 - __clz(c - 1u));
    return min(30, 32 - ceillog2);
}
constexpr float EXP_M05 = 0.6065306597126334f;

__device__ __forceinline__ bool win_active(const Geom& g, int b) { return b >= 64 || ((g.wmask >> b) & 1ull) != 0ull; }

constexpr int ACC_SHIFT = 30;

__device__ __forceinline__ int fix64_shift(double bound) {
    if (!(bound > 0.0) || !(bound < 1.0e300)) return 0;
    int e;
    (void)frexp(bound, &e);
    return 50 - e;
}
constexpr double FIX64_MAGIC = 6755399441055744.0;
__device__ __forceinline__ long long fix64(double scaled) {
    return __double_as_longlong(scaled + FIX64_MAGIC) - __double_as_longlong(FIX64_MAGIC);
}
__device__ __forceinline__ int fix64_wide_shift(double bound) {
    if (!(bound > 0.0) || !(bound < 1.0e300)) return 0;
    int e;
    (void)frexp(bound, &e);
    return 61 - e;
}
__device__ __forceinline__ long long fix64_wide(double scaled) {
    const long long hi = fix64(scaled * (1.0 / 4294967296.0));
    const double rem = fma(-(double)hi, 4294967296.0, scaled);
    return hi * 4294967296ll + fix64(rem);
}
__device__ __forceinline__ double gmax_of(const unsigned* __restrict__ gmax_win, int n, unsigned* lds_scratch ) {
    unsigned m = 0u;
    for (int i = threadIdx.x; i < n; i += blockDim.x) m = max(m, gmax_win[i]);
#pragma unroll
    for (int o = 32; o > 0; o >>= 1) m = max(m, (unsigned)__shfl_xor((int)m, o, 64));
    if ((threadIdx.x & 63) == 0) lds_scratch[threadIdx.x >> 6] = m;
    __syncthreads();
    const int nw = (blockDim.x + 63) >> 6;
    m = lds_scratch[0];
    for (int i = 1; i < nw; ++i) m = max(m, lds_scratch[i]);
    return (double)__uint_as_float(m);
}
__device__ __forceinline__ int grad_shift_pixel(const WinConst& c, double gm, int R, bool wide) {
    const double bound = 2.15 * gm * c.dtmax * fmax(c.cntmax, 1.0) * (double)R;
    return wide ? fix64_wide_shift(bound) : fix64_shift(bound);
}
__device__ __forceinline__ int grad_shift(const WinConst& c, double gm, int R) {
    return fix64_wide_shift(2.15 * gm * c.dtmax * fmax(c.nev, 1.0) * (double)R * 4.0);
}

struct ThetaArg { double v[THETA_ARG_MAX]; };
struct ThetaArgBig { double v[THETA_ARG_BIG]; };
struct ThetaArgMid { double v[THETA_ARG_MID]; };

__device__ __forceinline__ int wrap_drop(int p, int n) {
    p += (p < 0) ? n : 0;
    return (p >= 0 && p < n) ? p : -1;
}

__device__ __forceinline__ double wave_sum(double v) {
#pragma unroll
    for (int o = 32; o > 0; o >>= 1) v += __shfl_down(v, o, 64);
    return v;
}
__device__ __forceinline__ double wave_min(double v) {
#pragma unroll
    for (int o = 32; o > 0; o >>= 1) v = fmin(v, __shfl_down(v, o, 64));
    return v;
}
__device__ __forceinline__ double wave_max(double v) {
#pragma unroll
    for (int o = 32; o > 0; o >>= 1) v = fmax(v, __shfl_down(v, o, 64));
    return v;
}

template <int NW = NWAVE>
__device__ __forceinline__ double block_sum(double v, double* scratch) {
    v = wave_sum(v);
    const int lane = threadIdx.x & 63, wv = threadIdx.x >> 6;
    __syncthreads();
    if (lane == 0) scratch[wv] = v;
    __syncthreads();
    double r = 0.0;
    if (threadIdx.x == 0) {
#pragma unroll
        for (int i = 0; i < NW; ++i) r += scratch[i];
    }
    return r;
}

__device__ __forceinline__ int win_pitch(const Geom& g, int ww) { return g.pitch_aligned ? ((ww + 31) & ~31) : ww; }

__device__ __forceinline__ Window item_window(const Geom& g, const Item& it, const double* __restrict__ mm4, double tau, int wincap, int winmaxw,
                                              bool aligned_list = true) {
    const bool aligned = aligned_list && g.pitch_aligned != 0;
    const int tx = it.tile % g.tilesX, ty = it.tile / g.tilesX;
    const int x0 = tx * TS, y0 = ty * TS;
    const int x1 = min(x0 + TS, g.W) - 1, y1 = min(y0 + TS, g.H) - 1;
    const double dlo = it.t_lo - tau, dhi = it.t_hi - tau;
    const double LIM = 4096.0;
    double lo[2], hi[2];
#pragma unroll
    for (int c = 0; c < 2; ++c) {
        const double vmin = mm4[2 * c], vmax = mm4[2 * c + 1];
        const double a = -vmin * dlo, b = -vmin * dhi, cc = -vmax * dlo, d = -vmax * dhi;
        double mn = fmin(fmin(a, b), fmin(cc, d)), mx = fmax(fmax(a, b), fmax(cc, d));
        if (!(mn == mn) || !(mx == mx)) { mn = 0.0; mx = 0.0; }
        lo[c] = floor(fmin(fmax(mn, -LIM), LIM));
        hi[c] = ceil(fmin(fmax(mx, -LIM), LIM));
    }
    int bx0 = x0 + (int)lo[0] - 2, bx1 = x1 + (int)hi[0] + 2;
    int by0 = y0 + (int)lo[1] - 2, by1 = y1 + (int)hi[1] + 2;
    int ww = bx1 - bx0 + 1, wh = by1 - by0 + 1;
    if ((aligned ? win_pitch(g, ww) : ww) * wh > wincap || ww > winmaxw) {
        int nww = min(ww, winmaxw);
        if (aligned && nww >= 64) nww &= ~31;
        const int nwh = min(wh, wincap / (aligned ? win_pitch(g, nww) : nww));
        bx0 = (bx0 + bx1) / 2 - nww / 2;
        by0 = (by0 + by1) / 2 - nwh / 2;
        ww = nww; wh = nwh;
    }
    Window w; w.ox = bx0; w.oy = by0; w.ww = ww; w.wh = wh;
    return w;
}

__device__ __forceinline__ void warp_axis(int x, double v, double dt, int& ir, float& f) {
#ifndef EINCM_ABL_WARP_FMA
#pragma clang fp contract(off)
#endif
    const double w = (double)x - v * dt;
    const double r = rint(w);
    f = (float)(w - r);
    ir = (int)r;
}
__device__ __forceinline__ int clamp_far(int ir) { return min(max(ir, -(1 << 20)), 1 << 20); }

struct f2v { float x, y; };

__device__ __forceinline__ void taps3x2(float fx, float fy, float scale_y, f2v& km, f2v& k0, f2v& kp) {
    constexpr float L2E = 1.4426950408889634f, EXP_M1 = 0.36787944117144233f;
    const float bx = __builtin_amdgcn_exp2f(fmaf(fx, L2E, -0.5f * L2E)), by = __builtin_amdgcn_exp2f(fmaf(fy, L2E, -0.5f * L2E));
    const float ax = EXP_M1 * __builtin_amdgcn_rcpf(bx), ay = EXP_M1 * __builtin_amdgcn_rcpf(by);
    const float s = __builtin_amdgcn_exp2f(fmaf(fx, fx, fy * fy) * (-0.5f * L2E)) * scale_y;
    km.x = ax; km.y = s * ay;
    k0.x = 1.0f; k0.y = s;
    kp.x = bx; kp.y = s * by;
}

struct EvReg { uint32_t xy; double t; float w; };

__device__ __forceinline__ double motion_coord(int x, double c, double s) {
#pragma clang fp contract(off)
    return __ddiv_rn((double)x - c, s);
}
__device__ __forceinline__ void motion_products(double u, double v, double& uu, double& uv, double& vv) {
#pragma clang fp contract(off)
    uu = u * u; uv = u * v; vv = v * v;
}
__device__ __forceinline__ double2 motion_poly(const double* q, double u, double v, double uu, double uv, double vv) {
#pragma clang fp contract(off)
    double2 t;
    t.x = ((((q[0] + q[1] * u) + q[2] * v) + q[3] * uu) + q[4] * uv) + q[5] * vv;
    t.y = ((((q[6] + q[7] * u) + q[8] * v) + q[9] * uu) + q[10] * uv) + q[11] * vv;
    return t;
}

constexpr int POLY_NQ = 12;
constexpr int POLY_ARG_Q0 = 4;
constexpr int POLY_ARG_WINDOWS = (THETA_ARG_MAX - POLY_ARG_Q0) / POLY_NQ;

template <int NTH>
__device__ __forceinline__ void poly_tile_bounds(const double* uv, double* mm4) {
    const double* red = uv + 2 * TS;
    mm4[0] = red[0]; mm4[1] = red[1]; mm4[2] = red[2]; mm4[3] = red[3];
    for (int i = 1; i < NTH / 64; ++i) {
        mm4[0] = fmin(mm4[0], red[4 * i]); mm4[1] = fmax(mm4[1], red[4 * i + 1]);
        mm4[2] = fmin(mm4[2], red[4 * i + 2]); mm4[3] = fmax(mm4[3], red[4 * i + 3]);
    }
}

template <int NTH>
__device__ __forceinline__ void poly_fill_tile(const Geom& g, int win, int tx0, int ty0, int use_arg, const double* __restrict__ theta_c,
                                               const ThetaArg& targ, double2* thtile, double* uv, double* mm4) {
#pragma clang fp contract(off)
    static_assert(NTH <= 512 && TS == 32, "the bounds' scratch holds 8 waves; one wave divides for 2 x 32 coordinates");
    const int tid = threadIdx.x;
    if (tid < 2 * TS) {
        const bool row = tid >= TS;
        uv[tid] = motion_coord((row ? ty0 : tx0) + (tid & (TS - 1)), row ? targ.v[1] : targ.v[0], targ.v[2]);
    }
    double q[POLY_NQ];
#pragma unroll
    for (int j = 0; j < POLY_NQ; ++j) q[j] = use_arg ? targ.v[POLY_ARG_Q0 + POLY_NQ * win + j] : theta_c[(size_t)POLY_NQ * win + j];
    __syncthreads();
    double mnx = INFINITY, mxx = -INFINITY, mny = INFINITY, mxy = -INFINITY;
    for (int p = tid; p < TS * TS; p += NTH) {
        const int ly = p / TS, lx = p % TS;
        double2 t = make_double2(0.0, 0.0);
        if (ty0 + ly < g.H && tx0 + lx < g.W) {
            const double u = uv[lx], v = uv[TS + ly];
            double uu, uvp, vv;
            motion_products(u, v, uu, uvp, vv);
            t = motion_poly(q, u, v, uu, uvp, vv);
            mnx = fmin(mnx, t.x); mxx = fmax(mxx, t.x); mny = fmin(mny, t.y); mxy = fmax(mxy, t.y);
        }
        thtile[p] = t;
// ... 194 lines not shown
    const double nanf = wave_max(nan ? 1.0 : 0.0);
    const int lane = threadIdx.x & 63, wv = threadIdx.x >> 6;
    if (lane == 0) { red[0][wv] = mnx; red[1][wv] = mxx; red[2][wv] = mny; red[3][wv] = mxy; nanred[wv] = nanf; }
    __syncthreads();
    if (threadIdx.x == 0) {
        double a = red[0][0], bq = red[1][0], c = red[2][0], d = red[3][0], nf = nanred[0];
        for (int i = 1; i < NWAVE; ++i) {
            a = fmin(a, red[0][i]); bq = fmax(bq, red[1][i]); c = fmin(c, red[2][i]); d = fmax(d, red[3][i]);
            nf = fmax(nf, nanred[i]);
        }
        double* o = tmm + ((size_t)b * g.ntiles + tile) * 4;
        if (nf > 0.0) { a = bq = c = d = NAN; }
        o[0] = a; o[1] = bq; o[2] = c; o[3] = d;
        mm4s[0] = a; mm4s[1] = bq; mm4s[2] = c; mm4s[3] = d;
    }
    if (itembase_a == nullptr) return;
    __syncthreads();
    const double mm4[4] = {mm4s[0], mm4s[1], mm4s[2], mm4s[3]};
    const int na = (a1 - a0) * g.R, nb = (b1 - b0) * g.R;
    for (int k = threadIdx.x; k < na + nb; k += NT) {
        const bool first = k < na;
        const int kk = first ? k : k - na;
        const int item = (first ? a0 : b0) + kk / g.R, r = kk % g.R;
        const Item it = (first ? items_a : items_b)[item];
        (first ? wins_a : wins_b)[(size_t)item * g.R + r] = item_window(g, it, mm4, edge_ts[it.win * g.R + r], first ? g.wincap_a : g.wincap,
                                                                          first ? g.winmaxw_a : g.winmaxw, !first);
    }
}

__device__ __forceinline__ void windows_of(const Geom& g, int idx, int n_a, const Item* __restrict__ items_a, Window* __restrict__ wins_a,
                                           int n_b, const Item* __restrict__ items_b, Window* __restrict__ wins_b,
                                           const double* __restrict__ tmm, const double* __restrict__ edge_ts, bool const_theta, const ThetaArg& targ,
                                           const double* __restrict__ theta, int use_arg) {
    const bool first = idx < n_a * g.R;
    const int k = first ? idx : idx - n_a * g.R;
    if (!first && k >= n_b * g.R) return;
    const Item it = (first ? items_a : items_b)[k / g.R];
    if (!win_active(g, it.win)) return;
    const int r = k % g.R;
    double mm4[4];
    if (const_theta) {
        const double vx = use_arg ? targ.v[2 * it.win] : theta[2 * it.win], vy = use_arg ? targ.v[2 * it.win + 1] : theta[2 * it.win + 1];
        mm4[0] = vx; mm4[1] = vx; mm4[2] = vy; mm4[3] = vy;
    } else {
        const double* mm = tmm + ((size_t)it.win * g.ntiles + it.tile) * 4;
        mm4[0] = mm[0]; mm4[1] = mm[1]; mm4[2] = mm[2]; mm4[3] = mm[3];
    }
    (first ? wins_a : wins_b)[k] = item_window(g, it, mm4, edge_ts[it.win * g.R + r], first ? g.wincap_a : g.wincap, first ? g.winmaxw_a : g.winmaxw, !first);
}

__global__ __launch_bounds__(NT) void k_theta_const(Geom g, int use_arg, ThetaArg targ, const double* __restrict__ theta,
                                                     double* __restrict__ tmm, const double* __restrict__ edge_ts,
                                                     int n_a, const Item* __restrict__ items_a, Window* __restrict__ wins_a,
                                                     int n_b, const Item* __restrict__ items_b, Window* __restrict__ wins_b)
{
    const int i = blockIdx.x * NT + threadIdx.x;
    if (i < g.B * g.ntiles && win_active(g, i / g.ntiles)) {
        const int b = i / g.ntiles;
        const double vx = use_arg ? targ.v[2 * b] : theta[2 * b], vy = use_arg ? targ.v[2 * b + 1] : theta[2 * b + 1];
        double* o = tmm + (size_t)i * 4;
        o[0] = vx; o[1] = vx; o[2] = vy; o[3] = vy;
    }
    windows_of(g, i, n_a, items_a, wins_a, n_b, items_b, wins_b, tmm, edge_ts, true, targ, theta, use_arg);
}

__global__ __launch_bounds__(NT) void k_windows(Geom g, const double* __restrict__ tmm, const double* __restrict__ edge_ts,
                                                 int n_a, const Item* __restrict__ items_a, Window* __restrict__ wins_a,
                                                 int n_b, const Item* __restrict__ items_b, Window* __restrict__ wins_b)
{
    ThetaArg none;
    windows_of(g, blockIdx.x * NT + threadIdx.x, n_a, items_a, wins_a, n_b, items_b, wins_b, tmm, edge_ts, false, none, nullptr, 0);
}

__device__ __forceinline__ bool block_to_work(int n_items, int R, const int32_t* __restrict__ order, int& item, int& r) {
    const int b = blockIdx.x;
    const int xcd = b % NXCD, slot = b / NXCD;
    const int rank = (slot / R) * NXCD + xcd;
    r = slot % R;
    if (rank >= n_items) return false;
    item = order ? order[rank] : rank;
    return true;
}

template <int NTH> struct WinWalkT {
    int i, row, col, q, rem, ww;
    __device__ __forceinline__ WinWalkT(int tid, int ww_) : ww(ww_) {
        const float inv = 1.0f / (float)ww_;
        row = (int)((float)tid * inv); col = tid - row * ww_;
        if (col < 0) { col += ww_; --row; } else if (col >= ww_) { col -= ww_; ++row; }
        q = (int)((float)NTH * inv); rem = NTH - q * ww_;
        if (rem < 0) { rem += ww_; --q; } else if (rem >= ww_) { rem -= ww_; ++q; }
        i = tid;
    }
    __device__ __forceinline__ void next() {
        i += NTH; col += rem; row += q;
        if (col >= ww) { col -= ww; ++row; }
    }
};
using WinWalk = WinWalkT<NT>;

template <int NTH> struct SegWalk {
    static_assert(NTH == 256 || NTH == 512, "the staged layout is dealt to groups of 256 threads");
    int n0, K0, K1, rem0, rem1, tt, half;
    __device__ __forceinline__ SegWalk(int n, int tid) {
        n0 = (n + 1) >> 1;
        const int n1 = n - n0;
        K0 = (n0 + 255) >> 8; K1 = (n1 + 255) >> 8;
        rem0 = n0 - 256 * (K0 - 1); rem1 = n1 - 256 * (K1 - 1);
        tt = tid & 255; half = tid >> 8;
    }
    __device__ __forceinline__ int iters() const { return NTH == 512 ? K0 : K0 + K1; }
    __device__ __forceinline__ int index(int i) const {
        const int c = (NTH == 512) ? half : (i >= K0 ? 1 : 0);
        const int j = (NTH == 512) ? i : (c ? i - K0 : i);
        const int K = c ? K1 : K0, rem = c ? rem1 : rem0;
        const bool ok = j < K - 1 || (j == K - 1 && tt < rem);
        return ok ? (c ? n0 : 0) + j * 256 + tt : -1;
    }
};

template <bool PIPE, typename Load, typename Body>
__device__ __forceinline__ void event_trips(int nfull, bool tail, const Load& load, const Body& body) {
    EvReg T; T.xy = 0u; T.t = 0.0; T.w = 0.0f;
    if (tail) load(T, nfull);
    if (PIPE) {
        if (nfull > 0) {
            const int last = nfull - 1;
            EvReg A, B, C;
            load(A, 0); load(B, min(1, last));
            int j = 0;
            for (; j + 3 <= nfull; j += 3) {
                load(C, min(j + 2, last)); body(A);
                load(A, min(j + 3, last)); body(B);
                load(B, min(j + 4, last)); body(C);
            }
            if (j < nfull) body(A);
            if (j + 1 < nfull) body(B);
        }
    } else {
#pragma unroll 2
        for (int j = 0; j < nfull; ++j) { EvReg ev; load(ev, j); body(ev); }
    }
    if (tail) body(T);
}
struct EvBuf { __amdgpu_buffer_rsrc_t xy, t, w; };
__device__ __forceinline__ EvBuf ev_buf(const uint32_t* __restrict__ xy, const double* __restrict__ t, int n) {
    constexpr int RSRC_WORD3 = 0x00020000;
    EvBuf b;
    b.xy = __builtin_amdgcn_make_buffer_rsrc(const_cast<uint32_t*>(xy), 0, n * 4, RSRC_WORD3);
    b.t = __builtin_amdgcn_make_buffer_rsrc(const_cast<double*>(t), 0, n * 8, RSRC_WORD3);
    return b;
}
__device__ __forceinline__ void ev_buf_weights(EvBuf& b, const float* __restrict__ w, int n) {
    b.w = __builtin_amdgcn_make_buffer_rsrc(const_cast<float*>(w), 0, n * 4, 0x00020000);
}
template <int WT = 0>
__device__ __forceinline__ void ev_load(EvReg& r, const EvBuf& b, int base, uint32_t off4, uint32_t off8) {
    r.xy = __builtin_amdgcn_raw_buffer_load_b32(b.xy, off4, base * 4, 0);
    r.t = __builtin_bit_cast(double, __builtin_amdgcn_raw_buffer_load_b64(b.t, off8, base * 8, 0));
    if (WT) r.w = __builtin_bit_cast(float, __builtin_amdgcn_raw_buffer_load_b32(b.w, off4, base * 4, 0));
}

template <int TM, int NTH, int WT = 0>
__global__ __launch_bounds__(NTH) void k_splat(Geom g, int n_items,
        const Item* __restrict__ items,
        const uint32_t* __restrict__ ev_xy,
        const double* __restrict__ ev_t,
        const double* __restrict__ Theta,
        const double* __restrict__ edge_ts,
        const Window* __restrict__ wins,
        unsigned long long* __restrict__ acc,
        const int32_t* __restrict__ order,
        int use_arg, const double* __restrict__ theta_c, ThetaArg targ,
        const float* __restrict__ ev_w = nullptr)
{
    constexpr int theta_mode = TM;
    extern __shared__ __attribute__((aligned(16))) uint32_t ldsu[];
    double2* thtile = reinterpret_cast<double2*>(ldsu + g.wincap);
    int item, r;
    if (!block_to_work(n_items, g.R, order, item, r)) return;
    const Item it = items[item];
    if (!win_active(g, it.win)) return;
    const double tau = edge_ts[it.win * g.R + r];
    const int tx0 = (it.tile % g.tilesX) * TS, ty0 = (it.tile / g.tilesX) * TS;
    double2 vconst = make_double2(0.0, 0.0);
    Window wn;
    if (theta_mode == THETA_CONST) {
        vconst = use_arg ? make_double2(targ.v[2 * it.win], targ.v[2 * it.win + 1]) : make_double2(theta_c[2 * it.win], theta_c[2 * it.win + 1]);
        const double mm4[4] = {vconst.x, vconst.x, vconst.y, vconst.y};
        wn = item_window(g, it, mm4, tau, g.wincap, g.winmaxw);
    } else if (theta_mode == THETA_POLY) {
        double mm4[4];
        poly_fill_tile<NTH>(g, it.win, tx0, ty0, use_arg, theta_c, targ, thtile, reinterpret_cast<double*>(thtile + TS * TS), mm4);
        wn = item_window(g, it, mm4, tau, g.wincap, g.winmaxw);
    } else {
        const double* __restrict__ ThW = Theta + (size_t)it.win * g.H * g.W * 2;
        for (int p = threadIdx.x; p < TS * TS; p += NTH) {
            const int y = ty0 + p / TS, x = tx0 + p % TS;
            thtile[p] = (y < g.H && x < g.W) ? *reinterpret_cast<const double2*>(ThW + ((size_t)y * g.W + x) * 2) : make_double2(0.0, 0.0);
        }
        wn = wins[(size_t)item * g.R + r];
    }
    const int nwin = wn.ww * wn.wh;
    const int wp = win_pitch(g, wn.ww), wp4 = wp * 4, nlds = wp * wn.wh;
    {
        uint4* z = reinterpret_cast<uint4*>(ldsu);
        const int nq = (nlds + 3) >> 2;
        for (int i = threadIdx.x; i < nq; i += NTH) z[i] = make_uint4(0u, 0u, 0u, 0u);
    }
    __syncthreads();

    unsigned long long* __restrict__ img = acc + ((size_t)it.win * g.R + r) * g.H * g.W;
    const uint32_t* __restrict__ exy = ev_xy + it.begin;
    const double* __restrict__ et = ev_t + it.begin;
    const int n = it.count;
    const int fshift = fix_shift(n);
    const float FIX_SCALE = ldexpf(1.0f, fshift);
    const int up = ACC_SHIFT - fshift;

    const int tid = threadIdx.x;
    const int nfull = n / NTH;
    const uint32_t off4 = (uint32_t)tid * 4u, off8 = (uint32_t)tid * 8u;
#if defined(EINCM_ABL_S_NOLOADT)
    auto load_ev = [&](EvReg& r, int j) { const int e = j * NTH + tid; r.xy = exy[e]; r.t = it.t_lo + 1e-9 * (double)e; };
#elif defined(EINCM_ABL_S_NOLOAD)
    auto load_ev = [&](EvReg& r, int j) { const int e = j * NTH + tid; r.xy = ((uint32_t)(ty0 + ((e * 7) & 31)) << 16) | (uint32_t)(tx0 + (e & 31)); r.t = it.t_lo + 1e-9 * (double)e; };
#else
    EvBuf evb = ev_buf(exy, et, n);
    if (WT) ev_buf_weights(evb, ev_w + it.begin, n);
    auto load_ev = [&](EvReg& r, int j) { ev_load<WT>(r, evb, j * NTH, off4, off8); };
#endif
    const float scy = INV_2PI * FIX_SCALE;
    auto splat_ev = [&](const EvReg& ev) {
        const double dt = ev.t - tau;
        const int x = ev.xy & 0xffff, y = ev.xy >> 16;
        const double2 v = (theta_mode == THETA_CONST) ? vconst : thtile[((ev.xy >> 11) & (31u << 5)) | (ev.xy & 31u)];
        int irx, iry; float fx, fy;
        warp_axis(x, v.x, dt, irx, fx);
        warp_axis(y, v.y, dt, iry, fy);
        f2v km, k0, kp;
#ifdef EINCM_ABL_S_NOMATH
        km.x = km.y = k0.x = k0.y = kp.x = kp.y = 3.0f;
#else
        taps3x2(fx, fy, WT ? scy * ev.w : scy, km, k0, kp);
#endif
        const int lx = irx - 1 - wn.ox, ly = iry - 1 - wn.oy;
        if ((unsigned)lx < (unsigned)(wn.ww - 2) && (unsigned)ly < (unsigned)(wn.wh - 2)) {
            uint32_t* p = reinterpret_cast<uint32_t*>(reinterpret_cast<char*>(ldsu) + (__mul24(ly, wp4) + (lx << 2)));
            uint32_t* p1 = p + wp; uint32_t* p2 = p1 + wp;
#ifdef EINCM_ABL_S_NOATOMIC
            *p = fix_u32(km.y, km.x) + fix_u32(km.y, k0.x) + fix_u32(km.y, kp.x) + fix_u32(k0.y, km.x) + fix_u32(k0.y, k0.x) + fix_u32(k0.y, kp.x)
               + fix_u32(kp.y, km.x) + fix_u32(kp.y, k0.x) + fix_u32(kp.y, kp.x) + (uint32_t)(p1 - p2);
#else
            atomicAdd(p, fix_u32(km.y, km.x)); atomicAdd(p + 1, fix_u32(km.y, k0.x)); atomicAdd(p + 2, fix_u32(km.y, kp.x));
            atomicAdd(p1, fix_u32(k0.y, km.x)); atomicAdd(p1 + 1, fix_u32(k0.y, k0.x)); atomicAdd(p1 + 2, fix_u32(k0.y, kp.x));
            atomicAdd(p2, fix_u32(kp.y, km.x)); atomicAdd(p2 + 1, fix_u32(kp.y, k0.x)); atomicAdd(p2 + 2, fix_u32(kp.y, kp.x));
#endif
        } else {
            const float kx[3] = {km.x, k0.x, kp.x}, ky[3] = {km.y, k0.y, kp.y};
            const int sx = clamp_far(irx), sy = clamp_far(iry), lxs = sx - 1 - wn.ox, lys = sy - 1 - wn.oy;
#pragma unroll
            for (int dy = 0; dy < 3; ++dy) {
#pragma unroll
                for (int dx = 0; dx < 3; ++dx) {
                    const int cx = lxs + dx, cy = lys + dy;
                    if (cx >= 0 && cy >= 0 && cx < wn.ww && cy < wn.wh) {
                        atomicAdd(ldsu + cy * wp + cx, fix_u32(ky[dy], kx[dx]));
                    } else {
                        const int gx = wrap_drop(sx - 1 + dx, g.W), gy = wrap_drop(sy - 1 + dy, g.H);
                        if (gx >= 0 && gy >= 0)
                            atomicAdd(img + (size_t)gy * g.W + gx, (unsigned long long)fix_u32(ky[dy], kx[dx]) << up);
                    }
                }
            }
        }
    };
#ifndef EINCM_ABL_S_NOEVENTS
    event_trips<true>(nfull, nfull * NTH + tid < n, load_ev, splat_ev);
#endif
    __syncthreads();
#ifdef EINCM_ABL_S_NOFLUSH
    return;
#endif
    const int lane = threadIdx.x & 63, wv = threadIdx.x >> 6;
    auto to_acc = [&](int i) -> unsigned long long { return (unsigned long long)ldsu[i] << up; };
    if (wn.ox >= 0 && wn.oy >= 0 && wn.ox + wn.ww <= g.W && wn.oy + wn.wh <= g.H) {
        unsigned long long* __restrict__ dst = img + (size_t)wn.oy * g.W + wn.ox;
        for (WinWalkT<NTH> w(threadIdx.x, wn.ww); w.i < nwin; w.next()) {
            const unsigned long long v = to_acc(w.row * wp + w.col);
            if (v != 0ull) atomicAdd(dst + w.row * g.W + w.col, v);
        }
        return;
    }
    for (int row = wv; row < wn.wh; row += NTH / 64) {
        const int gy = wrap_drop(wn.oy + row, g.H);
        if (gy < 0) continue;
        for (int col = lane; col < wn.ww; col += 64) {
            const unsigned long long v = to_acc(row * wp + col);
            if (v != 0ull) {
// ... 461 lines not shown
            for (int dx = 0; dx < 3; ++dx) {
                const int cx = lxs + dx, cy = lys + dy;
                float val = 0.0f;
                if (cx >= 0 && cy >= 0 && cx < wn.ww && cy < wn.wh) {
                    val = lds[cy * wp + cx];
                } else {
                    const int gx = wrap_drop(sx - 1 + dx, g.W), gy = wrap_drop(sy - 1 + dy, g.H);
                    if (gx >= 0 && gy >= 0) val = Gi((size_t)gy * g.W + gx);
                }
                gv[dy][dx] = val;
            }
        }
    }
    const float c0 = fmaf(by, gv[2][0], fmaf(ay, gv[0][0], gv[1][0]));
    const float c1 = fmaf(by, gv[2][1], fmaf(ay, gv[0][1], gv[1][1]));
    const float c2 = fmaf(by, gv[2][2], fmaf(ay, gv[0][2], gv[1][2]));
    const float u0 = ax * c0, u2 = bx * c2;
    const float S = (u0 + u2) + c1;
    gwx = scale * fmaf(-fx, S, u2 - u0);
    const float r0 = fmaf(bx, gv[0][2], fmaf(ax, gv[0][0], gv[0][1]));
    const float r2 = fmaf(bx, gv[2][2], fmaf(ax, gv[2][0], gv[2][1]));
    gwy = scale * fmaf(-fy, S, fmaf(by, r2, -(ay * r0)));}

__host__ __device__ __forceinline__ int tv_shift(int H, int W) {
    int e = 0;
    while ((double)(1ull << e) <= 256.0 * (double)H * (double)W) ++e;
    return 61 - e;
}

constexpr int PROJ_SCRATCH_BYTES = 2 * TS * PG_MAXC * 8 + 2 * TS * PG_MAXC * 16;
template <int NTH>
__device__ __forceinline__ void project_tile_to_cells(const Geom& g, int h, int w, const TileRange& tr, int x0, int y0,
                                                      const double* __restrict__ AH, const double* __restrict__ AW,
                                                      const double2* vals, void* scratch, unsigned long long* __restrict__ cells) {
    const int ni = tr.ni, nj = tr.nj;
    double* ahs = reinterpret_cast<double*>(scratch);
    double* aws = ahs + TS * PG_MAXC;
    double2* st = reinterpret_cast<double2*>(aws + TS * PG_MAXC);
    for (int k = threadIdx.x; k < TS * ni; k += NTH) {
        const int ly = k / ni, i = k - ly * ni;
        ahs[k] = (y0 + ly < g.H) ? AH[(size_t)(y0 + ly) * h + tr.ilo + i] : 0.0;
    }
    for (int k = threadIdx.x; k < TS * nj; k += NTH) {
        const int lx = k / nj, j = k - lx * nj;
        aws[k] = (x0 + lx < g.W) ? AW[(size_t)(x0 + lx) * w + tr.jlo + j] : 0.0;
    }
    __syncthreads();
    for (int k = threadIdx.x; k < 2 * TS * nj; k += NTH) {
        const int q = k / (TS * nj), kk = k - q * (TS * nj);
        const int ly = kk / nj, jj = kk - ly * nj;
        double ax = 0.0, ay = 0.0;
#pragma unroll 4
        for (int lx = 16 * q; lx < 16 * q + 16; ++lx) {
            const double wgt = aws[lx * nj + jj];
            const double2 v = vals[(ly << 5) + (lx ^ ly)];
            ax += wgt * v.x; ay += wgt * v.y;
        }
        st[k] = make_double2(ax, ay);
    }
    __syncthreads();
    for (int k = threadIdx.x; k < ni * nj; k += NTH) {
        const int ii = k / nj, jj = k - ii * nj;
        double ax = 0.0, ay = 0.0;
#pragma unroll 4
        for (int ly = 0; ly < TS; ++ly) {
            const double wgt = ahs[ly * ni + ii];
            const double2 v0 = st[ly * nj + jj], v1 = st[TS * nj + ly * nj + jj];
            ax += wgt * (v0.x + v1.x); ay += wgt * (v0.y + v1.y);
        }
        unsigned long long* o = cells + ((size_t)(tr.ilo + ii) * w + (tr.jlo + jj)) * 2;
        if (ax != 0.0) atomicAdd(o, (unsigned long long)fix64_wide(ax));
        if (ay != 0.0) atomicAdd(o + 1, (unsigned long long)fix64_wide(ay));
    }
}
template <int TM, int WIDE, int NTH, int PROJ, int ALLR = 0, int WT = 0>
__global__ __launch_bounds__(NTH, (ALLR ? 6 : 1)) void k_gather(Geom g, int n_items,
        const Item* __restrict__ items, const uint32_t* __restrict__ ev_xy, const double* __restrict__ ev_t,
        const double* __restrict__ Theta, const double* __restrict__ edge_ts,
        const float* __restrict__ G,
        const Window* __restrict__ wins,
        long long* __restrict__ gTheta,
        double* __restrict__ g11,
        const WinConst* __restrict__ wc, const unsigned* __restrict__ gmax,
        const int32_t* __restrict__ order,
        int use_arg, const double* __restrict__ theta_c, ThetaArg targ,
        int h, int w, const double* __restrict__ AH, const double* __restrict__ AW, const TileRange* __restrict__ tilerng,
        long long* __restrict__ gth_main, int gth_cap,
        int tail, unsigned* __restrict__ ticket, const int32_t* __restrict__ win_item0, double* __restrict__ grad_out,
        double tv_gamma, const double* __restrict__ tvparts, long long* __restrict__ gth_tv,
        const float* __restrict__ ev_w = nullptr)
{
    constexpr int theta_mode = TM;
    constexpr bool direct11 = TM == THETA_CONST;
    const int wincap = g.wincap_a, winmaxw = g.winmaxw_a;
    extern __shared__ __attribute__((aligned(16))) float lds[];
    __shared__ double red11[NTH / 64];
    unsigned long long* accum = reinterpret_cast<unsigned long long*>(lds + wincap);
    double2* thtile = reinterpret_cast<double2*>(lds + wincap + (direct11 ? 0 : TS * TS * 4));
    float f11x = 0.0f, f11y = 0.0f;
    int item, r;
    constexpr bool all_r = ALLR != 0;
    if (!block_to_work(n_items, all_r ? 1 : g.R, order, item, r)) return;
    const Item it = items[item];
    if (!win_active(g, it.win)) return;
    double tau = edge_ts[it.win * g.R + r];
    const int lane = threadIdx.x & 63, wv = threadIdx.x >> 6;
    double2 vconst = make_double2(0.0, 0.0);
    Window wn;
    if (theta_mode == THETA_CONST) {
        vconst = use_arg ? make_double2(targ.v[2 * it.win], targ.v[2 * it.win + 1]) : make_double2(theta_c[2 * it.win], theta_c[2 * it.win + 1]);
        const double mm4[4] = {vconst.x, vconst.x, vconst.y, vconst.y};
        wn = item_window(g, it, mm4, tau, wincap, winmaxw);
    } else if (theta_mode == THETA_POLY) {
        double mm4[4];
        poly_fill_tile<NTH>(g, it.win, (it.tile % g.tilesX) * TS, (it.tile / g.tilesX) * TS, use_arg, theta_c, targ, thtile,
                            reinterpret_cast<double*>(thtile + TS * TS), mm4);
        wn = item_window(g, it, mm4, tau, wincap, winmaxw, false);
    } else {
        wn = wins[(size_t)item * g.R + r];
    }
    int wp = (theta_mode == THETA_CONST) ? win_pitch(g, wn.ww) : wn.ww;
    size_t img = ((size_t)it.win * g.R + r) * g.H * g.W;
    const float* __restrict__ Gi = G + img;
    const int tx = it.tile % g.tilesX, ty = it.tile / g.tilesX;
    const int x0 = tx * TS, y0 = ty * TS;
    if (theta_mode == THETA_TILE) {
        const double* __restrict__ ThW = Theta + (size_t)it.win * g.H * g.W * 2;
        for (int p = threadIdx.x; p < TS * TS; p += NTH) {
            const int y = y0 + p / TS, x = x0 + p % TS;
            thtile[p] = (y < g.H && x < g.W) ? *reinterpret_cast<const double2*>(ThW + ((size_t)y * g.W + x) * 2) : make_double2(0.0, 0.0);
        }
    }
    if (!direct11) for (int i = threadIdx.x; i < TS * TS * 2; i += NTH) accum[i] = 0ull;
    auto G_at = [&](size_t p) -> float { return Gi[p]; };
    auto load_window = [&]() {
    if (wn.ox >= 0 && wn.oy >= 0 && wn.ox + wn.ww <= g.W && wn.oy + wn.wh <= g.H) {
        const size_t o0 = (size_t)wn.oy * g.W + wn.ox;
        for (WinWalkT<NTH> w(threadIdx.x, wn.ww); w.i < wn.ww * wn.wh; w.next()) lds[w.row * wp + w.col] = G_at(o0 + w.row * g.W + w.col);
    } else {
        for (int row = wv; row < wn.wh; row += NTH / 64) {
            const int gy = wrap_drop(wn.oy + row, g.H);
            for (int col = lane; col < wn.ww; col += 64) {
                const int gx = wrap_drop(wn.ox + col, g.W);
                lds[row * wp + col] = (gx >= 0 && gy >= 0) ? G_at((size_t)gy * g.W + gx) : 0.0f;
            }
        }
    }
    };
    load_window();
    double gscale = 0.0;
    double gm_used = 0.0;
    int gshift = 0;
    if (!direct11) {
        __shared__ unsigned gms[NTH / 64];
        const double gm = gmax_of(gmax + (size_t)it.win * g.gmax_n, g.gmax_n, gms);
        gshift = grad_shift_pixel(wc[it.win], gm, g.R, WIDE != 0);
        gscale = ldexp(1.0, gshift);
        gm_used = gm;
    }
    __syncthreads();

    const uint32_t* __restrict__ exy = ev_xy + it.begin;
    const double* __restrict__ et = ev_t + it.begin;
    const int n = it.count;
    const int tid = threadIdx.x;
    uint32_t cur_key = 0xffffffffu;
    double run_x = 0.0, run_y = 0.0;
    double2 vcur = vconst;
    auto flush_run = [&]() {
        if (cur_key == 0xffffffffu) return;
        unsigned long long* a = accum + (cur_key << 1);
        atomicAdd(a, (unsigned long long)(WIDE ? fix64_wide(run_x) : fix64(run_x)));
        atomicAdd(a + 1, (unsigned long long)(WIDE ? fix64_wide(run_y) : fix64(run_y)));
    };
    auto gather_ev = [&](const EvReg& ev) {
        const double dt = ev.t - tau;
        const int x = ev.xy & 0xffff, y = ev.xy >> 16;
        if (theta_mode != THETA_CONST) {
            const uint32_t key = ((ev.xy >> 11) & (31u << 5)) | (ev.xy & 31u);
#ifdef EINCM_ABL_G_NORUN
            vcur = thtile[key];
#else
            if (key != cur_key) {
                flush_run();
                cur_key = key; run_x = 0.0; run_y = 0.0;
                vcur = thtile[key];
            }
#endif
        }
        float gwx, gwy;
        event_dLdw(g, wn, wp, lds, G_at, x, y, vcur, dt, gwx, gwy);
        if (WT) { gwx *= ev.w; gwy *= ev.w; }
        if (direct11) {
            const float ndt = (float)(-dt);
            f11x = fmaf(ndt, gwx, f11x); f11y = fmaf(ndt, gwy, f11y);
        } else {
            const double sdt = -dt * gscale;
            run_x = fma(sdt, (double)gwx, run_x); run_y = fma(sdt, (double)gwy, run_y);
        }
    };
    const SegWalk<NTH> walk(n, tid);
    EvBuf evb = ev_buf(exy, et, n);
    if (WT) ev_buf_weights(evb, ev_w + it.begin, n);
    auto walk_half = [&](int c) {
        const int K = c ? walk.K1 : walk.K0, rem = c ? walk.rem1 : walk.rem0;
        const uint32_t off = (uint32_t)((c ? walk.n0 : 0) + walk.tt), off4 = off * 4u, off8 = off * 8u;
        event_trips<false>(max(K - 1, 0), K > 0 && walk.tt < rem,
                              [&](EvReg& ev, int j) { ev_load<WT>(ev, evb, j * 256, off4, off8); }, gather_ev);
    };
    for (int rr = r; ; ) {
#ifndef EINCM_ABL_G_NOEVENTS
    if (NTH == 512) walk_half(walk.half);
    else {
#pragma unroll 1
        for (int c = 0; c < 2; ++c) walk_half(c);
    }
    if (!direct11) { flush_run(); cur_key = 0xffffffffu; run_x = 0.0; run_y = 0.0; }
#endif
    if (!all_r || ++rr >= g.R) break;
    __syncthreads();
    tau = edge_ts[it.win * g.R + rr];
    if (theta_mode == THETA_POLY) {
        double mm4[4];
        poly_tile_bounds<NTH>(reinterpret_cast<const double*>(thtile + TS * TS), mm4);
        wn = item_window(g, it, mm4, tau, wincap, winmaxw, false);
    } else {
        wn = wins[(size_t)item * g.R + rr];
    }
    wp = wn.ww;
    img = ((size_t)it.win * g.R + rr) * g.H * g.W;
    Gi = G + img;
    load_window();
    __syncthreads();
    }
    if (direct11) {
        double sum11x = block_sum<NTH / 64>((double)f11x, red11);
        double sum11y = block_sum<NTH / 64>((double)f11y, red11);
        if (threadIdx.x == 0) {
            double* dst = g11 + ((size_t)item * g.R + r) * 2;
            dst[0] = sum11x; dst[1] = sum11y;
        }
        return;
    }
    __syncthreads();
#ifdef EINCM_ABL_G_NOFLUSH
    return;
#endif
    if (theta_mode == THETA_POLY) {
        static_assert((NTH / 64) * POLY_NQ * 8 <= WIN_CAP_DEFAULT * 4, "the waves' sums fit the smallest G window");
        poly_project_moments<NTH>(accum, reinterpret_cast<const double*>(thtile + TS * TS), gshift, reinterpret_cast<double*>(lds),
                                  g11 + ((size_t)item * (all_r ? 1 : g.R) + (all_r ? 0 : r)) * POLY_NQ);
        return;
    }
    if (PROJ) {
        const TileRange tr = tilerng[it.tile];
        static_assert(PROJ_SCRATCH_BYTES <= WIN_CAP_DEFAULT * 4, "the projection's scratch fits the smallest G window");
        const double gmd = gm_used;
        const double scale = ldexp(1.0, grad_shift(wc[it.win], gmd, g.R) - grad_shift_pixel(wc[it.win], gmd, g.R, WIDE != 0));
        for (int p = threadIdx.x; p < TS * TS; p += NTH) {
            const int ly = p >> 5, lx = p & 31;
            const long long vx = (long long)accum[p * 2], vy = (long long)accum[p * 2 + 1];
            thtile[(ly << 5) + (lx ^ ly)] = make_double2((double)vx * scale, (double)vy * scale);
        }
        unsigned long long* __restrict__ out = reinterpret_cast<unsigned long long*>(gth_main) + (size_t)it.win * gth_cap;
        project_tile_to_cells<NTH>(g, h, w, tr, x0, y0, AH, AW, thtile, lds, out);
        if (!tail) return;
        __shared__ int s_last;
        asm volatile("s_waitcnt vmcnt(0)" ::: "memory");
        __syncthreads();
        if (threadIdx.x == 0) {
            const int n_it = ((it.win + 1 < g.B) ? win_item0[it.win + 1] : n_items) - win_item0[it.win];
            const unsigned old = __hip_atomic_fetch_add(ticket + it.win, 1u, __ATOMIC_RELAXED, __HIP_MEMORY_SCOPE_AGENT);
            const bool last = old == (unsigned)(n_it * (all_r ? 1 : g.R)) - 1u;
            if (last) __hip_atomic_store(ticket + it.win, 0u, __ATOMIC_RELAXED, __HIP_MEMORY_SCOPE_AGENT);
            s_last = last ? 1 : 0;
        }
        __syncthreads();
        if (!s_last) return;
        const double inv = ldexp(1.0, -grad_shift(wc[it.win], gmd, g.R));
        const int ncell = h * w * 2;
        double stv = 0.0;
        if (tv_gamma != 0.0) {
            double nz = 0.0;
            for (int i = threadIdx.x; i < g.ntiles; i += NTH) nz += tvparts[((size_t)it.win * g.ntiles + i) * 3 + 1];
            __shared__ double tvred[NTH / 64];
            nz = block_sum<NTH / 64>(nz, tvred);
            __shared__ double s_stv;
            if (threadIdx.x == 0) s_stv = tv_grad_scale(tv_gamma, nz) * ldexp(1.0, -tv_shift(g.H, g.W));
            __syncthreads();
            stv = s_stv;
        }
        unsigned long long* __restrict__ out_tv = reinterpret_cast<unsigned long long*>(gth_tv) + (size_t)it.win * gth_cap;
        for (int i = threadIdx.x; i < ncell; i += NTH) {
            const long long q = (long long)atomicExch(out + i, 0ull);
            double v = (double)q * inv;
            if (tv_gamma != 0.0) v += stv * (double)(long long)atomicExch(out_tv + i, 0ull);
            grad_out[(size_t)it.win * ncell + i] = v;
        }
        return;
    }
    unsigned long long* __restrict__ gT = reinterpret_cast<unsigned long long*>(gTheta) + (size_t)it.win * g.H * g.W * 2;
    const int tw = min(TS, g.W - x0), th = min(TS, g.H - y0);
    for (int i = threadIdx.x; i < TS * TS * 2; i += NTH) {
        const int c = i & 1, px = (i >> 1) % TS, py = (i >> 1) / TS;
// ... 508 lines not shown
```

edge-informed-contrast-maximization_amd/csrc/eincm_plan.h:

```cpp
#pragma once
#include <algorithm>
#include <cmath>
#include <cstdint>
#include <cstring>
#include <vector>

#include "eincm.h"
#include "eincm_types.h"

namespace eincm {

struct Packer {
    std::vector<char> buf;
    size_t add(const void* p, size_t bytes, size_t align = 1) {
        const size_t off = (buf.size() + align - 1) / align * align;
        buf.resize(off + bytes, 0);
        if (bytes) std::memcpy(buf.data() + off, p, bytes);
        return off;
    }
    static const int32_t* i32(const char* base, size_t off) { return reinterpret_cast<const int32_t*>(base + off); }
    static const double* f64(const char* base, size_t off) { return reinterpret_cast<const double*>(base + off); }
};

struct SegList {
    int seg = 0;
    int n = 0;
    double tspan = 1.0;
    Item* d_items = nullptr;
    int32_t* d_order = nullptr;
    std::vector<Item> h_items;
    std::vector<int32_t> h_order;
    int32_t* d_win_item0 = nullptr;
    std::vector<int32_t> h_win_item0;
    Window* d_wins = nullptr;
    int32_t* d_itembase = nullptr;
    unsigned grid(int R) const { return (unsigned)(((n + NXCD - 1) / NXCD) * NXCD * R); }
};

constexpr int SEG_SHORT = 8192;
constexpr int MIN_SEG = 64;

inline void cut_segments(const int32_t* counts, size_t nbins, int ntiles, int seg, int64_t N, bool want_items, SegList& L,
                         std::vector<int32_t>& lens) {
    constexpr int K = 64;
    int64_t by_nseg[K + 1] = {0};
    lens.clear();
    L.h_items.clear(); L.h_win_item0.clear();
    int64_t base = 0;
    for (size_t idx = 0; idx < nbins; ++idx) {
        if (want_items && idx % (size_t)ntiles == 0) L.h_win_item0.push_back((int32_t)lens.size());
        const int cnt = counts[idx], len = balanced_seg_len(cnt, seg);
        if (cnt > 0) by_nseg[std::min<int64_t>(((int64_t)cnt + seg - 1) / seg, K)] += cnt;
        for (int s0 = 0; s0 < cnt; s0 += len) {
            lens.push_back(std::min(len, cnt - s0));
            if (want_items) L.h_items.push_back(Item{(int32_t)(idx / ntiles), (int32_t)(idx % ntiles), (int32_t)(base + s0), lens.back(), 0.0, 0.0});
        }
        base += cnt;
    }
    if (want_items) L.h_win_item0.push_back((int32_t)lens.size());
    L.seg = seg;
    L.tspan = 1.0 / K;
    int64_t beyond = 0;
    const int64_t allow = (int64_t)(0.03 * (double)N);
    for (int k = 1; k <= K; ++k)
        if ((beyond += by_nseg[k]) > allow) { L.tspan = 1.0 / k; break; }
    int32_t maxlen = 0;
    for (const int32_t l : lens) maxlen = std::max(maxlen, l);
    std::vector<int32_t> start((size_t)maxlen + 2, 0);
    for (const int32_t l : lens) ++start[(size_t)(maxlen - l) + 1];
    for (size_t k = 1; k < start.size(); ++k) start[k] += start[k - 1];
    L.h_order.resize(lens.size());
    for (size_t i = 0; i < lens.size(); ++i) L.h_order[(size_t)start[(size_t)(maxlen - lens[i])]++] = (int32_t)i;
}

inline double kern_eval(int method, double x) {
    switch (method) {
        case EINCM_METHOD_BILINEAR: return std::max(0.0, 1.0 - std::fabs(x));
        case EINCM_METHOD_LANCZOS3:
        case EINCM_METHOD_LANCZOS5: {
            const double radius = (method == EINCM_METHOD_LANCZOS3) ? 3.0 : 5.0;
            if (x > radius) return 0.0;
            if (!(x > 1e-3)) return 1.0;
            const double y = radius * std::sin(M_PI * x) * std::sin(M_PI * x / radius);
            return y / (M_PI * M_PI * x * x);
        }
        case EINCM_METHOD_CUBIC: {
            if (x >= 2.0) return 0.0;
            if (x >= 1.0) return ((-0.5 * x + 2.5) * x - 4.0) * x + 2.0;
            return ((1.5 * x - 2.5) * x) * x + 1.0;
        }
    }
    return 0.0;
}

inline void resample_matrix(int n_in, int n_out, int method, std::vector<double>& A) {
    A.assign((size_t)n_out * n_in, 0.0);
    const double scale = (double)n_out / (double)n_in;
    const double inv_scale = 1.0 / scale;
    const double kernel_scale = std::max(inv_scale, 1.0);
    const double thresh = 1000.0 * 1.1920928955078125e-07;
    for (int o = 0; o < n_out; ++o) {
        const double sample_f = ((double)o + 0.5) * inv_scale - 0.5;
        double total = 0.0;
        for (int i = 0; i < n_in; ++i) {
            const double x = std::fabs(sample_f - (double)i) / kernel_scale;
            const double wgt = kern_eval(method, x);
            A[(size_t)o * n_in + i] = wgt;
            total += wgt;
        }
        const bool inside = (sample_f >= -0.5) && (sample_f <= (double)n_in - 0.5);
        for (int i = 0; i < n_in; ++i) {
            double& a = A[(size_t)o * n_in + i];
// ... 260 lines not shown
    return P;
}

struct DevIo {
    const double* theta = nullptr;
    double* grad = nullptr;
    double vmax = -1.0;
};


struct SplatKey {
    int mode;
    int rad;
    int threads;
    int weighted;
};
struct GatherKey {
    int mode, rad;
    int wide;
    int threads;
    int proj, all_r;
    int weighted;
};
constexpr bool operator==(const SplatKey& a, const SplatKey& b) {
    return a.mode == b.mode && a.rad == b.rad && a.threads == b.threads && a.weighted == b.weighted;
}
constexpr bool operator==(const GatherKey& a, const GatherKey& b) {
    return a.mode == b.mode && a.rad == b.rad && a.wide == b.wide && a.threads == b.threads && a.proj == b.proj && a.all_r == b.all_r &&
           a.weighted == b.weighted;
}
constexpr int NT_TILE = 512;
inline constexpr SplatKey SPLAT_FORMS[] = {
    {THETA_CONST, 1, NT_TILE, 0}, {THETA_CONST, 1, NT_TILE, 1}, {THETA_TILE, 1, NT_TILE, 0}, {THETA_TILE, 1, NT_TILE, 1},
    {THETA_POLY, 1, NT_TILE, 0},
};
inline constexpr SplatKey SPLAT_R_FORMS[] = {
    {THETA_CONST, 0, NT, 0}, {THETA_CONST, 2, NT, 0}, {THETA_CONST, 3, NT, 0}, {THETA_TILE, 0, NT, 0}, {THETA_TILE, 2, NT, 0}, {THETA_TILE, 3, NT, 0},
};
inline constexpr GatherKey GATHER_FORMS[] = {
    {THETA_CONST, 1, 0, NT, 0, 0, 0},      {THETA_CONST, 1, 0, NT, 0, 0, 1},
    {THETA_TILE, 1, 0, NT_TILE, 0, 0, 0},  {THETA_TILE, 1, 0, NT_TILE, 0, 0, 1},  {THETA_TILE, 1, 1, NT_TILE, 0, 0, 0},  {THETA_TILE, 1, 1, NT_TILE, 0, 0, 1},
    {THETA_TILE, 1, 0, NT_TILE, 1, 0, 0},  {THETA_TILE, 1, 0, NT_TILE, 1, 0, 1},  {THETA_TILE, 1, 1, NT_TILE, 1, 0, 0},  {THETA_TILE, 1, 1, NT_TILE, 1, 0, 1},
    {THETA_TILE, 1, 0, NT_TILE, 1, 1, 0},  {THETA_TILE, 1, 0, NT_TILE, 1, 1, 1},  {THETA_TILE, 1, 1, NT_TILE, 1, 1, 0},  {THETA_TILE, 1, 1, NT_TILE, 1, 1, 1},
    {THETA_POLY, 1, 0, NT_TILE, 0, 0, 0},  {THETA_POLY, 1, 1, NT_TILE, 0, 0, 0},  {THETA_POLY, 1, 0, NT_TILE, 0, 1, 0},  {THETA_POLY, 1, 1, NT_TILE, 0, 1, 0},
};
inline constexpr GatherKey GATHER_R_FORMS[] = {
    {THETA_CONST, 0, 0, NT, 0, 0, 0}, {THETA_CONST, 2, 0, NT, 0, 0, 0}, {THETA_CONST, 3, 0, NT, 0, 0, 0},
    {THETA_TILE, 0, 0, NT, 0, 0, 0},  {THETA_TILE, 2, 0, NT, 0, 0, 0},  {THETA_TILE, 3, 0, NT, 0, 0, 0},
};
template <typename K, size_t N> constexpr int form_row(const K (&rows)[N], const K& k) {
    for (size_t i = 0; i < N; ++i) if (rows[i] == k) return (int)i;
    return -1;
}

enum class ListId { GATHER, SPLAT, SPLAT_SHORT, GATHER_2DOF };
enum class EventCopy { SPLAT, GATHER };

struct SplatForm {
    SplatKey key{};
    int row = -1;
    size_t lds = 0;
    ListId list = ListId::SPLAT;
    int wincap = 0, winmaxw = 0;
};
struct GatherForm {
    GatherKey key{};
    int row = -1;
    size_t lds = 0;
    ListId list = ListId::GATHER;
    EventCopy copy = EventCopy::GATHER;
    int wg_per_seg = 0;
    int wincap = 0, winmaxw = 0, pitch_aligned = 0;
};

struct EvalPlan {
    enum Shape { IDENTITY, TWO_DOF, GRID, MOTION } shape = GRID;
    enum ThetaSrc { THETA_DEVICE, THETA_ARGS, THETA_PINNED, THETA_PIECES } theta_src = THETA_PIECES;
    int h = 0, w = 0; size_t nth = 0;
    bool want_grad = false, full_aux = false, div_grad = false;
    EvalParams ep{};
    bool obj = false; ObjGeom og{};
    int wincap = 0, winmaxw = 0, pitch_aligned = 0, wincap_a = 0, winmaxw_a = 0;
    WinFit win_2{}; bool splat_short = false;
    bool use_arg = false, use_arg_big = false;
    bool need_theta_image = false;
    bool host_asm = false;
    bool grid_tail = false;
    bool stream_stats = false, g2_from_imgrad = false;
    bool tv_proj = false, proj = false;
    bool all_r = false;
    bool events_projected = false; int nsrc = 0;
    bool zero_copy_out = false;
    SplatForm splat; GatherForm gather;
};

constexpr int MOTION_PLAN_ARG_WINDOWS = (THETA_ARG_MAX - 4) / 12;
constexpr size_t ZERO_COPY_MAX = 65536;

inline EvalPlan::Shape theta_shape(const Geom& g, int h, int w) {
    return (h == g.H && w == g.W) ? EvalPlan::IDENTITY : (h == 1 && w == 1) ? EvalPlan::TWO_DOF : EvalPlan::GRID;
}
inline int correlation_kind(const eincm_params* p) { return (int)((p->flags & EINCM_PF_CORRELATION_MASK) >> 8); }
inline bool other_kinds(const eincm_params* p) { return p->contrast_kind > EINCM_CONTRAST_VARIANCE || correlation_kind(p) != EINCM_CORRELATION_MSE; }

inline ObjGeom obj_geom(const PlanCtx& c, int ck, int rk, int need) {
    ObjGeom og{};
    og.th = c.obj_th; og.tw = c.obj_tw;
    og.nty = c.g.H / og.th; og.ntx = c.g.W / og.tw; og.ncells = og.nty * og.ntx;
    og.ck = ck; og.rk = rk; og.need = need;
    return og;
}

struct EvalKnobs {
    bool no_big_arg = false;
    bool no_host_asm = false;
    int all_r = -1;
};

inline void plan_windows_preset(const PlanCtx& c, EvalPlan& P) {
    const Geom& g = c.g;
    P.wincap = g.wincap; P.winmaxw = g.winmaxw; P.wincap_a = g.wincap_a; P.winmaxw_a = g.winmaxw_a;
    P.pitch_aligned = c.stage.pitch != 0 ? 1 : 0;
    P.win_2 = WinFit{c.wincap, win_maxw(c.wincap), c.stage.pitch >= 2, true};
}
inline void plan_windows(const PlanCtx& c, EvalPlan& P, double vmax, bool two_dof) {
    const double margin = 2.0 * (c.splat_rad + 1);
    const int floor_s = two_dof ? 2 : 0, pitch_s = c.stage.pitch != 0 ? 1 : 0;
    WinFit s = fit_window(vmax, c.splat.tspan, margin, floor_s, pitch_s);
    P.splat_short = two_dof && c.splat_sh.n > 0 && !s.fits;
    if (P.splat_short) s = fit_window(vmax, c.splat_sh.tspan, margin, floor_s, pitch_s);
    P.wincap = s.cap; P.winmaxw = s.maxw; P.pitch_aligned = s.pal ? 1 : 0;
    const WinFit a = fit_window(vmax, c.gather.tspan, margin, 2, -1);
    P.wincap_a = a.cap; P.winmaxw_a = a.maxw;
    P.win_2 = fit_window(vmax, c.gather_2.tspan, margin, 2, c.stage.pitch >= 2 ? 1 : 0);
}

inline const SegList& seg_list(const PlanCtx& c, ListId id) {
    return id == ListId::GATHER ? c.gather : id == ListId::SPLAT ? c.splat : id == ListId::SPLAT_SHORT ? c.splat_sh : c.gather_2;
}

inline void plan_forms(const PlanCtx& c, EvalPlan& P) {
    const bool two_dof = P.shape == EvalPlan::TWO_DOF, fused = P.shape == EvalPlan::MOTION;
    const int mode = two_dof ? THETA_CONST : fused ? THETA_POLY : THETA_TILE, rad = c.splat_rad, wt = c.stage.weighted ? 1 : 0;
    const size_t theta_tile = two_dof ? 0 : TS * TS * 2 * sizeof(double);
    const size_t scratch = fused ? POLY_SCRATCH_BYTES : 0;
    SplatForm& s = P.splat;
    s.list = P.splat_short ? ListId::SPLAT_SHORT : ListId::SPLAT;
    if (rad == 1) {
        s.key = SplatKey{mode, rad, NT_TILE, wt};
        s.row = form_row(SPLAT_FORMS, s.key);
        s.wincap = P.wincap; s.winmaxw = P.winmaxw;
        s.lds = (size_t)s.wincap * sizeof(float) + theta_tile + scratch;
    } else {
        s.key = SplatKey{mode, rad, NT, wt};
        s.row = form_row(SPLAT_R_FORMS, s.key);
        s.wincap = std::min(P.wincap, two_dof ? SW_CAP_CONST : SW_CAP_TILE); s.winmaxw = win_maxw(s.wincap);
        s.lds = (size_t)s.wincap * sizeof(unsigned long long) + theta_tile + scratch;
    }
    if (!P.want_grad) return;
    GatherForm& a = P.gather;
    a.list = two_dof ? ListId::GATHER_2DOF : ListId::GATHER;
    a.copy = two_dof ? EventCopy::SPLAT : EventCopy::GATHER;
    a.wg_per_seg = P.all_r ? 1 : c.g.R;
    a.wincap = two_dof ? P.win_2.cap : P.wincap_a; a.winmaxw = two_dof ? P.win_2.maxw : P.winmaxw_a;
    a.pitch_aligned = two_dof ? (P.win_2.pal ? 1 : 0) : P.pitch_aligned;
    a.lds = (size_t)a.wincap * sizeof(float) + (two_dof ? 0 : TS * TS * 2 * sizeof(double) + theta_tile) + scratch;
    const bool templated = rad == 1 && !two_dof;
    a.key = GatherKey{mode, rad, templated && c.stage.wide ? 1 : 0, templated ? NT_TILE : NT, P.proj ? 1 : 0, P.all_r ? 1 : 0, wt};
    a.row = rad == 1 ? form_row(GATHER_FORMS, a.key) : form_row(GATHER_R_FORMS, a.key);
}

inline EvalPlan plan_eval(const PlanCtx& c, const DevIo& io, const EvalKnobs& knobs, const double* theta_host, int h, int w,
                          const eincm_params* p, bool want_grad) {
    const Geom& g = c.g;
    EvalPlan P;
    P.shape = theta_shape(g, h, w);
    const bool identity = P.shape == EvalPlan::IDENTITY, two_dof = P.shape == EvalPlan::TWO_DOF;
    P.h = h; P.w = w; P.nth = (size_t)h * w * 2;
    P.want_grad = want_grad;
    P.full_aux = (p->flags & EINCM_PF_FULL_AUX) != 0;
    P.div_grad = p->delta != 0.0 && want_grad;
    EvalParams& ep = P.ep;
    ep.alpha = p->alpha; ep.beta = p->beta; ep.gamma = p->gamma; ep.delta = p->delta;
    ep.cur_pyr_lvl = p->cur_pyr_lvl; ep.contrast_kind = p->contrast_kind;
    ep.want_div = (P.full_aux || p->delta != 0.0) ? 1 : 0;
    ep.want_tv = ((p->cur_pyr_lvl <= 0) && (p->gamma != 0.0 || P.full_aux)) ? 1 : 0;
    ep.use_tv_grad = (ep.want_tv && p->gamma != 0.0 && want_grad && !(p->flags & EINCM_PF_NO_TV_GRAD)) ? 1 : 0;
    ep.h = h; ep.w = w; ep.identity = identity ? 1 : 0;
    P.obj = other_kinds(p);
    const int ck = p->contrast_kind, rk = correlation_kind(p);
    if (P.obj) P.og = obj_geom(c, ck, rk, (ck == EINCM_CONTRAST_ADAPTIVE_GRAD_MAG ? OBJ_NEED_TILE_GM : 0) |
                                          ((ck == EINCM_CONTRAST_GRAD_MAG || rk == EINCM_CORRELATION_JOINT_CONTRAST) ? OBJ_NEED_GM : 0) |
                                          (rk == EINCM_CORRELATION_JOINT_CONTRAST ? OBJ_NEED_JOINT : 0));
    if (c.fp64) return P;
    const size_t nall = (size_t)g.B * P.nth;

    P.use_arg = !io.theta && !identity && nall <= (size_t)THETA_ARG_MAX;
    P.use_arg_big = !io.theta && !identity && nall <= (size_t)THETA_ARG_BIG && !knobs.no_big_arg;
    P.theta_src = io.theta ? EvalPlan::THETA_DEVICE
                : (P.use_arg_big && (P.use_arg || !two_dof)) ? EvalPlan::THETA_ARGS
                : nall <= ZERO_COPY_MAX ? EvalPlan::THETA_PINNED : EvalPlan::THETA_PIECES;
    P.need_theta_image = !two_dof || ep.want_tv || io.theta;

    plan_windows_preset(c, P);
    if (!c.wincap_fixed) {
        double vmax = 0.0;
        const size_t stride = nall > 8192 ? nall / 8192 : 1;
        if (io.theta) vmax = (io.vmax >= 0.0 && std::isfinite(io.vmax)) ? io.vmax : 1e9;
        else if (stride == 1) { for (size_t i = 0; i < nall; ++i) { const double a = std::fabs(theta_host[i]); vmax = std::max(vmax, a <= 1.7e308 ? a : 0.0); } }
        else for (size_t i = 0; i < nall; i += stride) { const double a = std::fabs(theta_host[i]); if (a > vmax && std::isfinite(a)) vmax = a; }
        plan_windows(c, P, vmax, two_dof);
    }

    const bool tail_ok = c.splat_rad == 1 && P.shape == EvalPlan::GRID && c.proj_in_gather && c.itembase_valid && nall <= ZERO_COPY_MAX &&
                         !io.theta;
    P.host_asm = want_grad && ((two_dof && !ep.want_tv) || tail_ok) && !ep.want_div && !P.full_aux && !knobs.no_host_asm && !c.device_results &&
                 !io.theta;
    P.grid_tail = P.host_asm && P.shape == EvalPlan::GRID;
    P.g2_from_imgrad = want_grad && ep.contrast_kind == EINCM_CONTRAST_GRAD_MAG && !P.obj;
    P.stream_stats = P.host_asm || (P.g2_from_imgrad && g.ntiles >= NSPART) || P.obj;
    P.tv_proj = ep.use_tv_grad && P.shape == EvalPlan::GRID && c.proj_in_gather;
    P.proj = want_grad && P.shape == EvalPlan::GRID && c.proj_in_gather && c.splat_rad == 1;
    P.all_r = P.proj && (knobs.all_r >= 0 ? knobs.all_r != 0 : c.gather.n >= 700);
    P.events_projected = two_dof || P.proj;
    P.nsrc = (!want_grad || identity) ? 0 : (P.events_projected ? 0 : 1) + ((ep.use_tv_grad && !P.tv_proj) ? 1 : 0);
    P.zero_copy_out = !c.device_results && !io.theta && !identity && nall <= ZERO_COPY_MAX;
    plan_forms(c, P);
    return P;
}

inline EvalPlan plan_motion(const PlanCtx& c, const EvalKnobs& knobs, double vmax, const eincm_params* p, bool want_grad) {
    static const double no_theta = 0.0;
    DevIo io;
    io.theta = &no_theta; io.vmax = vmax;
    EvalPlan P = plan_eval(c, io, knobs, nullptr, c.g.H, c.g.W, p, want_grad);
    P.shape = EvalPlan::MOTION;
    P.theta_src = EvalPlan::THETA_ARGS;
    P.use_arg = c.g.B <= MOTION_PLAN_ARG_WINDOWS;
    P.need_theta_image = false;
    P.all_r = want_grad && c.g.R > 1 && (knobs.all_r >= 0 ? knobs.all_r != 0 : c.gather.n >= 700);
    P.events_projected = true;
    P.zero_copy_out = true;
    plan_forms(c, P);
    return P;
}

inline void launch_policy(const PlanCtx& c, const EvalPlan& P, bool evaluated, double* out) {
    const StagePlan& S = c.stage;
    out[EINCM_LP_SEG_GATHER] = S.seg; out[EINCM_LP_SEG_SPLAT] = S.seg_s; out[EINCM_LP_SEG_GATHER_2DOF] = S.seg_2;
    out[EINCM_LP_SEG_SPLAT_SHORT] = S.splat_short ? SEG_SHORT : 0; out[EINCM_LP_PITCH_POLICY] = S.pitch;
    out[EINCM_LP_SPAN_SPLAT] = c.splat.tspan; out[EINCM_LP_SPAN_GATHER] = c.gather.tspan; out[EINCM_LP_SPAN_GATHER_2DOF] = c.gather_2.tspan;
    out[EINCM_LP_CAP_SPLAT] = evaluated ? P.wincap : 0; out[EINCM_LP_CAP_GATHER] = evaluated ? P.wincap_a : 0;
    out[EINCM_LP_CAP_GATHER_2DOF] = evaluated ? P.win_2.cap : 0;
    out[EINCM_LP_PITCH_ALIGNED] = evaluated ? ((P.pitch_aligned ? 1 : 0) | (P.win_2.pal ? 2 : 0)) : 0;
    out[EINCM_LP_SPLAT_SHORT] = evaluated && P.splat_short ? 1 : 0;
}

}
```

edge-informed-contrast-maximization_amd/csrc/eincm_splat_window.hip.h:

```cpp
#pragma once
#include "eincm_kernels.hip.h"

namespace eincm {

constexpr int SPLAT_RADIUS_MAX = 3;

__device__ __forceinline__ Window item_window_r(const Geom& g, const Item& it, const double* mm4, double tau, int wincap, int winmaxw, int rad) {
    const int tx = it.tile % g.tilesX, ty = it.tile / g.tilesX;
    const int x0 = tx * TS, y0 = ty * TS;
    const int x1 = min(x0 + TS, g.W) - 1, y1 = min(y0 + TS, g.H) - 1;
    const double dlo = it.t_lo - tau, dhi = it.t_hi - tau;
    const double LIM = 4096.0;
    double lo[2], hi[2];
#pragma unroll
    for (int c = 0; c < 2; ++c) {
        const double vmin = mm4[2 * c], vmax = mm4[2 * c + 1];
        const double a = -vmin * dlo, b = -vmin * dhi, cc = -vmax * dlo, d = -vmax * dhi;
        double mn = fmin(fmin(a, b), fmin(cc, d)), mx = fmax(fmax(a, b), fmax(cc, d));
        if (!(mn == mn) || !(mx == mx)) { mn = 0.0; mx = 0.0; }
        lo[c] = floor(fmin(fmax(mn, -LIM), LIM));
        hi[c] = ceil(fmin(fmax(mx, -LIM), LIM));
    }
    const int m = rad + 1;
    int bx0 = x0 + (int)lo[0] - m, bx1 = x1 + (int)hi[0] + m;
    int by0 = y0 + (int)lo[1] - m, by1 = y1 + (int)hi[1] + m;
    int ww = bx1 - bx0 + 1, wh = by1 - by0 + 1;
    if (ww * wh > wincap || ww > winmaxw) {
        const int nww = min(ww, winmaxw);
        const int nwh = min(wh, wincap / nww);
        bx0 = (bx0 + bx1) / 2 - nww / 2;
        by0 = (by0 + by1) / 2 - nwh / 2;
        ww = nww; wh = nwh;
    }
    Window w; w.ox = bx0; w.oy = by0; w.ww = ww; w.wh = wh;
    return w;
}

template <int RAD>
__device__ __forceinline__ void taps_axis(float f, float* k) {
    constexpr float HL2E = 0.5f * 1.4426950408889634f;
#pragma unroll
    for (int d = -RAD; d <= RAD; ++d) {
        const float q = (float)d - f;
        k[d + RAD] = __builtin_amdgcn_exp2f(-(q * q) * HL2E);
    }
}

template <int TM>
__device__ __forceinline__ double2 window_velocity(const Geom& g, const Item& it, int use_arg, const double* __restrict__ theta_c,
                                                   const ThetaArg& targ, const double* __restrict__ tmm, double mm4[4]) {
    if (TM == THETA_CONST) {
        const double2 v = use_arg ? make_double2(targ.v[2 * it.win], targ.v[2 * it.win + 1])
                                  : make_double2(theta_c[2 * it.win], theta_c[2 * it.win + 1]);
        mm4[0] = v.x; mm4[1] = v.x; mm4[2] = v.y; mm4[3] = v.y;
        return v;
    }
    const double* mm = tmm + ((size_t)it.win * g.ntiles + it.tile) * 4;
    mm4[0] = mm[0]; mm4[1] = mm[1]; mm4[2] = mm[2]; mm4[3] = mm[3];
    return make_double2(0.0, 0.0);
}

__device__ __forceinline__ void stage_theta_tile(const Geom& g, const Item& it, const double* __restrict__ Theta, double2* thtile) {
    const int tx0 = (it.tile % g.tilesX) * TS, ty0 = (it.tile / g.tilesX) * TS;
    const double* __restrict__ ThW = Theta + (size_t)it.win * g.H * g.W * 2;
    for (int p = threadIdx.x; p < TS * TS; p += NT) {
        const int y = ty0 + p / TS, x = tx0 + p % TS;
        thtile[p] = (y < g.H && x < g.W) ? *reinterpret_cast<const double2*>(ThW + ((size_t)y * g.W + x) * 2) : make_double2(0.0, 0.0);
    }
}

template <int TM, int RAD>
__global__ __launch_bounds__(NT) void k_splat_r(Geom g, int n_items, const Item* __restrict__ items,
        const uint32_t* __restrict__ ev_xy, const double* __restrict__ ev_t,
        const double* __restrict__ Theta,
        const double* __restrict__ tmm,
        const double* __restrict__ edge_ts,
        unsigned long long* __restrict__ acc,
        const int32_t* __restrict__ order,
        int use_arg, const double* __restrict__ theta_c, ThetaArg targ)
{
    constexpr int K = 2 * RAD + 1;
    extern __shared__ __attribute__((aligned(16))) unsigned long long lds64[];
    double2* thtile = reinterpret_cast<double2*>(lds64 + g.wincap);
    int item, r;
    if (!block_to_work(n_items, g.R, order, item, r)) return;
    const Item it = items[item];
    if (!win_active(g, it.win)) return;
    const double tau = edge_ts[it.win * g.R + r];
    double mm4[4];
    const double2 vconst = window_velocity<TM>(g, it, use_arg, theta_c, targ, tmm, mm4);
    if (TM == THETA_TILE) stage_theta_tile(g, it, Theta, thtile);
    const Window wn = item_window_r(g, it, mm4, tau, g.wincap, g.winmaxw, RAD);
    const int nwin = wn.ww * wn.wh;
    for (int i = threadIdx.x; i < nwin; i += NT) lds64[i] = 0ull;
    __syncthreads();

    unsigned long long* __restrict__ img = acc + ((size_t)it.win * g.R + r) * g.H * g.W;
    const float scy = INV_2PI * 1073741824.0f;
    for (int e = threadIdx.x; e < it.count; e += NT) {
        const uint32_t xy = ev_xy[it.begin + e];
        const double dt = ev_t[it.begin + e] - tau;
        const int x = xy & 0xffff, y = xy >> 16;
        const double2 v = (TM == THETA_CONST) ? vconst : thtile[((xy >> 11) & (31u << 5)) | (xy & 31u)];
        int irx, iry; float fx, fy;
        warp_axis(x, v.x, dt, irx, fx);
        warp_axis(y, v.y, dt, iry, fy);
        float kx[K], ky[K];
        taps_axis<RAD>(fx, kx);
        taps_axis<RAD>(fy, ky);
#pragma unroll
        for (int d = 0; d < K; ++d) ky[d] *= scy;
        const int sx = clamp_far(irx), sy = clamp_far(iry);
        const int lx0 = sx - RAD - wn.ox, ly0 = sy - RAD - wn.oy;
        if (lx0 >= 0 && ly0 >= 0 && lx0 + K <= wn.ww && ly0 + K <= wn.wh) {
            unsigned long long* p = lds64 + ly0 * wn.ww + lx0;
#pragma unroll
            for (int dy = 0; dy < K; ++dy) {
#pragma unroll
                for (int dx = 0; dx < K; ++dx) atomicAdd(p + dx, (unsigned long long)fix_u32(ky[dy], kx[dx]));
                p += wn.ww;
            }
        } else {
#pragma unroll
            for (int dy = 0; dy < K; ++dy) {
#pragma unroll
                for (int dx = 0; dx < K; ++dx) {
                    const unsigned long long q = (unsigned long long)fix_u32(ky[dy], kx[dx]);
                    const int cx = lx0 + dx, cy = ly0 + dy;
                    if (cx >= 0 && cy >= 0 && cx < wn.ww && cy < wn.wh) {
                        atomicAdd(lds64 + cy * wn.ww + cx, q);
                    } else {
                        const int gx = wrap_drop(sx - RAD + dx, g.W), gy = wrap_drop(sy - RAD + dy, g.H);
                        if (gx >= 0 && gy >= 0) atomicAdd(img + (size_t)gy * g.W + gx, q);
                    }
                }
            }
        }
    }
    __syncthreads();
    for (WinWalk w(threadIdx.x, wn.ww); w.i < nwin; w.next()) {
        const unsigned long long q = lds64[w.i];
        if (q == 0ull) continue;
        const int gx = wrap_drop(wn.ox + w.col, g.W), gy = wrap_drop(wn.oy + w.row, g.H);
        if (gx >= 0 && gy >= 0) atomicAdd(img + (size_t)gy * g.W + gx, q);
    }
}

template <int TM, int RAD>
__global__ __launch_bounds__(NT) void k_gather_r(Geom g, int n_items, const Item* __restrict__ items,
        const uint32_t* __restrict__ ev_xy, const double* __restrict__ ev_t,
        const double* __restrict__ Theta, const double* __restrict__ tmm, const double* __restrict__ edge_ts,
        const float* __restrict__ G,
        long long* __restrict__ gTheta,
        double* __restrict__ g11,
        const WinConst* __restrict__ wc, const unsigned* __restrict__ gmax, int wide,
        int use_arg, const double* __restrict__ theta_c, ThetaArg targ)
{
    constexpr int K = 2 * RAD + 1;
    constexpr bool direct11 = TM == THETA_CONST;
    extern __shared__ __attribute__((aligned(16))) float lds[];
    __shared__ double red[NWAVE];
    __shared__ unsigned gms[NWAVE];
    unsigned long long* accum = reinterpret_cast<unsigned long long*>(lds + g.wincap_a);
    double2* thtile = reinterpret_cast<double2*>(lds + g.wincap_a + TS * TS * 4);
    int item, r;
    if (!block_to_work(n_items, g.R, nullptr, item, r)) return;
    const Item it = items[item];
    if (!win_active(g, it.win)) return;
    const double tau = edge_ts[it.win * g.R + r];
    double mm4[4];
    const double2 vconst = window_velocity<TM>(g, it, use_arg, theta_c, targ, tmm, mm4);
// ... 93 lines not shown
```

edge-informed-contrast-maximization_amd/csrc/eincm_types.h:

```cpp
#pragma once
#include <stddef.h>
#include <stdint.h>

#if defined(__HIPCC__)
#define EINCM_HD __host__ __device__ inline __attribute__((always_inline))
#else
#define EINCM_HD inline
#endif

namespace eincm {

constexpr int TS = 32;
constexpr int WIN_CAP_DEFAULT = 2304;
constexpr int NXCD = 8;
constexpr int MAX_SEG = 1 << 20;
EINCM_HD int balanced_seg_len(int c, int seg) {
    const int nseg = (c + seg - 1) / seg;
    if (nseg <= 1) return seg;
    const int len = (((c + nseg - 1) / nseg + 255) / 256) * 256;
    return len < seg ? len : seg;
}

struct Geom {
    int H, W, R, B;
    int tilesX, tilesY, ntiles;
    int wincap, winmaxw;
    int wincap_a, winmaxw_a;
    int nparts;
    int pstride;
    int gmax_n;
    unsigned long long wmask;
    int igx, nig;
    int pitch_aligned;
};

struct Item {
    int32_t win, tile, begin, count;
    double t_lo, t_hi;
};

struct EvalParams {
    double alpha, beta, gamma, delta;
    int cur_pyr_lvl, contrast_kind;
    int want_div, want_tv, use_tv_grad;
    int h, w, identity;
};

constexpr int THETA_ARG_MAX = 128;
constexpr int THETA_ARG_BIG = 4096;
constexpr int THETA_ARG_MID = 512;

constexpr int NT = 256;

constexpr int THETA_CONST = 1;
constexpr int THETA_TILE = 2;
constexpr int THETA_POLY = 3;
constexpr int POLY_SCRATCH = 2 * TS + 4 * 8;
constexpr size_t POLY_SCRATCH_BYTES = POLY_SCRATCH * sizeof(double);
constexpr int SW_CAP_TILE = 4608;
constexpr int SW_CAP_CONST = 6912;

struct Window { int ox, oy, ww, wh; };

struct TileRange { int ilo, ni, jlo, nj; };

constexpr int NSPART = 32;
constexpr int IG_ROWS = 12, IG_COLS = 60, IG_NT = 256;
constexpr int PG_MAXC = 6;

struct ObjGeom {
    int th, tw;
    int nty, ntx;
    int ncells;
    int ck, rk;
    int need;
};
constexpr int OBJ_NEED_TILE_GM = 1;
constexpr int OBJ_NEED_GM = 2;
constexpr int OBJ_NEED_JOINT = 4;

constexpr double EPSN = 2.220446049250313e-16;

struct StatPart {
    double mn, mx, cmn, cmx;
    double sI, sII, sEI, sG2;
};

struct ImgScal {
    double m, M, D, cm, cM, sI, sII, sEI, sG2;
};
constexpr int IMGSCAL_N = 9;

struct WinConst {
    double c0_gradmag, c0_var, d0;
    double zc[16];
    double sE[16], sEE[16];
    double eabs[16];
    double inv_c0_gradmag, inv_c0_var, inv_zc[16];
    double mrw[16];
    double dtmax;
    double nev;
    double cntmax;
};

struct OutScal {
    double value, mean_rel_corr, mean_rel_contrast, mean_rel_div, tv, tv_scale, nonfinite, _pad;
    double corr[16], contrast_gm[16], var[16], div[16];
};

struct F64Scal {
    double m, M, D, cm, cM, mean, var, g2, mse, div;
};

struct ObjConst {
    double c0[4];
    double zc[4][16];
};

static_assert(sizeof(StatPart) == 64 && offsetof(StatPart, mn) == 0 && offsetof(StatPart, sG2) == 56, "StatPart layout");
static_assert(sizeof(ImgScal) == IMGSCAL_N * 8 && offsetof(ImgScal, m) == 0 && offsetof(ImgScal, sG2) == 64, "ImgScal layout");
static_assert(sizeof(WinConst) == 104 * 8 && offsetof(WinConst, c0_gradmag) == 0 && offsetof(WinConst, cntmax) == 103 * 8, "WinConst layout");
static_assert(sizeof(OutScal) == 72 * 8 && offsetof(OutScal, value) == 0 && offsetof(OutScal, div) == 56 * 8, "OutScal layout");
static_assert(sizeof(F64Scal) == 80 && offsetof(F64Scal, m) == 0 && offsetof(F64Scal, div) == 72, "F64Scal layout");
static_assert(sizeof(ObjConst) == 68 * 8 && offsetof(ObjConst, c0) == 0 && offsetof(ObjConst, zc) == 32, "ObjConst layout");

}
```

Baseline: 182.1 billion.

## Precompute 64-byte per-job segment records and pass edge times as kernel args

Adds a SegRec record holding item fields, segment index, fixed-point shift and tile bounds, built once per list by a new kernel. Splat and gather kernels then load the record in a single vector load instead of chasing order->items and recomputing tile coordinates and shift. Edge timestamps are also copied into a by-value kernel argument when small, which replaces a dependent global load at block start. The cost is extra device memory, one extra kernel per list build, and larger kernel arguments.

Result: slower. 163.7 billion (-10.1%).

```diff
diff --git a/edge-informed-contrast-maximization_amd/csrc/eincm_api.hip b/edge-informed-contrast-maximization_amd/csrc/eincm_api.hip
--- a/edge-informed-contrast-maximization_amd/csrc/eincm_api.hip
+++ b/edge-informed-contrast-maximization_amd/csrc/eincm_api.hip
@@ -106,6 +106,7 @@
     EvalPlan plan{};
     DevIo io{};
     const double* theta_dev = nullptr; ThetaArg targ{};
+    EdgeArg earg{}; int arg_bits = 0;
     int copy_mode = 0;
     int n_pieces = 0;
     size_t piece_len = 0;
@@ -131,6 +132,7 @@
 
     bool staged = false;
     std::vector<int64_t> win_events;
+    std::vector<double> h_edge_ts;
 
     uint32_t* d_xy = nullptr;
     double* d_t = nullptr;
@@ -394,7 +396,12 @@
 
 const EvalKnobs& process_knobs() {
     static const EvalKnobs k{getenv("EINCM_NO_BIG_THETA_ARG") != nullptr, getenv("EINCM_NO_HOST_ASM") != nullptr,
-                             getenv("EINCM_GATHER_ALL_R") ? atoi(getenv("EINCM_GATHER_ALL_R")) : -1};
+                             getenv("EINCM_GATHER_ALL_R") ? atoi(getenv("EINCM_GATHER_ALL_R")) : -1,
+#ifdef EINCM_NO_JOB_RECORDS
+                             true};
+#else
+                             false};
+#endif
     return k;
 }
 struct CreateKnobs { int seg = 0, seg_s = 0, wincap = 0; bool host_binning = false; };
@@ -539,6 +546,8 @@
 int launch_splat(eincm_ctx* c, const double* theta_dev, const ThetaArg& targ) {
     const EvalPlan& P = c->fl.plan;
     const SplatForm& F = P.splat;
+    c->fl.arg_bits = (P.use_arg ? ARG_THETA : 0) | (P.edge_arg ? ARG_EDGE_TS : 0);
+    if (P.edge_arg) memcpy(c->fl.earg.v, c->h_edge_ts.data(), (size_t)c->g.B * c->g.R * sizeof(double));
     {
         StageTimer t(c, EINCM_STAGE_SPLAT, true);
         if (c->splat.n > 0) {
@@ -547,14 +556,15 @@
             Geom gs = c->g;
             gs.wincap = F.wincap; gs.winmaxw = F.winmaxw;
             const dim3 grid(L.grid(gs.R)), block(F.key.threads);
-            const int use_arg = P.use_arg ? 1 : 0;
+            Flight& fl = c->fl;
+            const SegRec* recs = P.job_records ? L.d_recs : nullptr;
             if (F.key.rad == 1)
                 launch_timed(c, EINCM_STAGE_SPLAT, SPLAT_KERNELS[F.row], grid, block, F.lds, gs, L.n, L.d_items, c->d_xy, c->d_t, c->d_Theta,
-                             c->d_edge_ts, c->splat.d_wins, c->d_acc, L.d_order, use_arg, theta_dev, targ,
+                             c->d_edge_ts, c->splat.d_wins, c->d_acc, L.d_order, recs, fl.arg_bits, theta_dev, targ, fl.earg,
                              (const float*)(F.key.weighted ? c->d_w : nullptr));
             else
                 launch_timed(c, EINCM_STAGE_SPLAT, SPLAT_R_KERNELS[F.row], grid, block, F.lds, gs, L.n, L.d_items, c->d_xy, c->d_t, c->d_Theta,
-                             c->d_tmm, c->d_edge_ts, c->d_acc, L.d_order, use_arg, theta_dev, targ);
+                             c->d_tmm, c->d_edge_ts, c->d_acc, L.d_order, recs, fl.arg_bits, theta_dev, targ, fl.earg);
         }
     }
     HIPCHK(c, hipGetLastError());
@@ -944,8 +954,9 @@
                 const int use_arg = P.use_arg ? 1 : 0;
                 if (F.key.rad == 1)
                     launch_timed(c, EINCM_STAGE_GATHER, GATHER_KERNELS[F.row], grid, block, F.lds, gg, L.n, L.d_items, xy_g, t_g, c->d_Theta,
-                                 c->d_edge_ts, c->d_G, c->gather.d_wins, c->d_gTheta, g11, c->d_wc, c->d_gmax, L.d_order, use_arg,
-                                 c->fl.theta_dev, c->fl.targ, P.h, P.w, c->d_AH.p, c->d_AW.p, c->d_tilerng, c->d_gth.p, (int)c->coarse_cap,
+                                 c->d_edge_ts, c->d_G, c->gather.d_wins, c->d_gTheta, g11, c->d_wc, c->d_gmax, L.d_order,
+                                 P.job_records ? L.d_recs : nullptr, c->fl.arg_bits,
+                                 c->fl.theta_dev, c->fl.targ, c->fl.earg, P.h, P.w, c->d_AH.p, c->d_AW.p, c->d_tilerng, c->d_gth.p, (int)c->coarse_cap,
                                  P.grid_tail ? 1 : 0, c->d_gticket, c->gather.d_win_item0, c->h_grad,
                                  (P.grid_tail && ep.use_tv_grad) ? ep.gamma : 0.0, c->d_tvparts, c->d_gth.p + (size_t)c->maxB * c->coarse_cap,
                                  (const float*)(F.key.weighted ? (own_copy ? c->d_w_g : c->d_w) : nullptr));
@@ -1174,6 +1185,7 @@
     for (SegList* L : {&c->gather, &c->splat, &c->splat_sh, &c->gather_2}) {
         TRY(c->mem.alloc_dev(L->d_items, (size_t)c->max_items));
         TRY(c->mem.alloc_dev(L->d_order, (size_t)c->max_items));
+        TRY(c->mem.alloc_dev(L->d_recs, (size_t)c->max_items));
     }
     for (SegList* L : {&c->gather, &c->gather_2}) TRY(c->mem.alloc_dev(L->d_win_item0, B + 1));
     for (SegList* L : {&c->gather, &c->splat}) {
@@ -1281,8 +1293,9 @@
     delete ctx;
 }
 
-static int build_list(eincm_ctx* c, SegList& L, int seg, bool on_host, int ntiles, const double* ev_t, int64_t N)
+static int build_list(eincm_ctx* c, SegList& L, int seg, bool on_host, const Geom& g, const double* ev_t, int64_t N)
 {
+    const int ntiles = g.ntiles;
     std::vector<int32_t> lens;
     cut_segments(c->h_tilecount.data(), c->h_tilecount.size(), ntiles, seg, N, on_host, L, lens);
     if ((int64_t)lens.size() > c->max_items) return fail(c, EINCM_ERR_ARG, "internal: %zu segments exceed capacity", lens.size());
@@ -1296,6 +1309,7 @@
     if (L.n == 0) return EINCM_OK;
     HIPCHK(c, hipMemcpyAsync(L.d_order, L.h_order.data(), (size_t)L.n * sizeof(int32_t), hipMemcpyHostToDevice, c->stream));
     hipLaunchKernelGGL(k_seg_minmax, dim3(std::min(L.n, 4096)), dim3(NT), 0, c->stream, L.n, L.d_items, ev_t);
+    hipLaunchKernelGGL(k_seg_records, dim3((L.n + NT - 1) / NT), dim3(NT), 0, c->stream, g, L.n, L.d_items, L.d_order, L.d_recs);
     HIPCHK(c, hipGetLastError());
     return EINCM_OK;
 }
@@ -1463,7 +1477,7 @@
                            c->gather.d_items);
         if ((rc = copy_for_gather(c))) return rc;
     }
-    if ((rc = build_list(c, c->gather, P.seg, false, g.ntiles, c->d_t_g, P.N))) return rc;
+    if ((rc = build_list(c, c->gather, P.seg, false, g, c->d_t_g, P.N))) return rc;
     c->splat.n = 0;
     if (nblk > 0) {
         if (P.spread && P.weighted)
@@ -1483,7 +1497,7 @@
     } else {
         HIPCHK(c, hipMemsetAsync(c->gather.d_win_item0, 0, (size_t)(a.B + 1) * sizeof(int32_t), c->stream));
     }
-    return build_list(c, c->splat, P.seg_s, false, g.ntiles, c->d_t, P.N);
+    return build_list(c, c->splat, P.seg_s, false, g, c->d_t, P.N);
 }
 
 static int bin_on_host(eincm_ctx* c, const StageArgs& a, StageScratch& sc) {
@@ -1506,9 +1520,9 @@
         if (P.weighted) HIPCHK(c, hipMemcpyAsync(c->d_w, sc.sw.data(), (size_t)P.N * sizeof(float), hipMemcpyHostToDevice, c->stream));
         if ((rc = upload_raw_events(c, a))) return rc;
     }
-    if ((rc = build_list(c, c->gather, P.seg, true, g.ntiles, c->d_t, P.N))) return rc;
+    if ((rc = build_list(c, c->gather, P.seg, true, g, c->d_t, P.N))) return rc;
     if ((rc = copy_for_gather(c))) return rc;
-    if ((rc = build_list(c, c->splat, P.seg_s, true, g.ntiles, c->d_t, P.N))) return rc;
+    if ((rc = build_list(c, c->splat, P.seg_s, true, g, c->d_t, P.N))) return rc;
     HIPCHK(c, hipMemcpyAsync(c->d_edges, sc.ef.data(), sc.ef.size() * sizeof(float), hipMemcpyHostToDevice, c->stream));
     return EINCM_OK;
 }
@@ -1520,9 +1534,9 @@
     if (!sc.edge_ts_uploaded)
         HIPCHK(c, hipMemcpyAsync(c->d_edge_ts, a.edge_ts, (size_t)a.B * a.R * sizeof(double), hipMemcpyHostToDevice, c->stream));
     HIPCHK(c, hipMemsetAsync(c->d_mask, 0, (size_t)a.B * g.H * g.W, c->stream));
-    if ((rc = build_list(c, c->gather_2, P.seg_2, true, g.ntiles, c->d_t, P.N))) return rc;
+    if ((rc = build_list(c, c->gather_2, P.seg_2, true, g, c->d_t, P.N))) return rc;
     c->splat_sh.n = 0;
-    if (P.splat_short && (rc = build_list(c, c->splat_sh, SEG_SHORT, true, g.ntiles, c->d_t, P.N))) return rc;
+    if (P.splat_short && (rc = build_list(c, c->splat_sh, SEG_SHORT, true, g, c->d_t, P.N))) return rc;
     if (c->gather.n > 0 && !P.host_binning) {
         HIPCHK(c, hipMemsetAsync(c->d_cntmax, 0, (size_t)a.B * sizeof(unsigned), c->stream));
         hipLaunchKernelGGL(k_tile_counts, dim3(g.ntiles, a.B), dim3(NT), 0, c->stream, g, c->d_tilebase, c->d_tilecount, c->d_xy,
@@ -1535,6 +1549,7 @@
     c->g = g;
     c->itembase_valid = !P.host_binning && c->gather.n > 0 && c->splat.n > 0;
     c->win_events.assign(a.n_events, a.n_events + a.B);
+    c->h_edge_ts.assign(a.edge_ts, a.edge_ts + (size_t)a.B * a.R);
     if (c->gather.n > 0 && P.host_binning) {
         hipLaunchKernelGGL(k_mask, dim3(std::min(c->gather.n, 2048)), dim3(NT), 0, c->stream, g, c->gather.d_items, c->gather.n, c->d_xy, c->d_mask,
                            (const float*)(P.weighted ? c->d_w : nullptr));
diff --git a/edge-informed-contrast-maximization_amd/csrc/eincm_binning.hip.h b/edge-informed-contrast-maximization_amd/csrc/eincm_binning.hip.h
--- a/edge-informed-contrast-maximization_amd/csrc/eincm_binning.hip.h
+++ b/edge-informed-contrast-maximization_amd/csrc/eincm_binning.hip.h
@@ -303,6 +303,15 @@
     }
 }
 
+__global__ __launch_bounds__(NT) void k_seg_records(Geom g, int n_items, const Item* __restrict__ items, const int32_t* __restrict__ order,
+                                                    SegRec* __restrict__ recs)
+{
+    const int k = blockIdx.x * NT + threadIdx.x;
+    if (k >= n_items) return;
+    const int seg = order[k];
+    recs[k] = seg_record(g, items[seg], seg);
+}
+
 constexpr int EDGE_PARTS = 32;
 constexpr int EDGE_MOM = 3;
 __global__ __launch_bounds__(NT) void k_edges(Geom g, const double* __restrict__ src, float* __restrict__ dst, double* __restrict__ moments)
diff --git a/edge-informed-contrast-maximization_amd/csrc/eincm_kernels.hip.h b/edge-informed-contrast-maximization_amd/csrc/eincm_kernels.hip.h
--- a/edge-informed-contrast-maximization_amd/csrc/eincm_kernels.hip.h
+++ b/edge-informed-contrast-maximization_amd/csrc/eincm_kernels.hip.h
@@ -11,11 +11,6 @@
 constexpr int WIN_CAP_MAX = 9216;
 constexpr float INV_2PI = 0.15915494309189535f;
 constexpr int MAX_CHUNK = 16384;
-__device__ __forceinline__ int fix_shift(int count) {
-    const unsigned c = (unsigned)ceilf((float)count * 0.16f);
-    const int ceillog2 = (c <= 1u) ? 0 : (32 - __clz(c - 1u));
-    return min(30, 32 - ceillog2);
-}
 constexpr float EXP_M05 = 0.6065306597126334f;
 
 __device__ __forceinline__ bool win_active(const Geom& g, int b) { return b >= 64 || ((g.wmask >> b) & 1ull) != 0ull; }
@@ -105,13 +100,10 @@
 
 __device__ __forceinline__ int win_pitch(const Geom& g, int ww) { return g.pitch_aligned ? ((ww + 31) & ~31) : ww; }
 
-__device__ __forceinline__ Window item_window(const Geom& g, const Item& it, const double* __restrict__ mm4, double tau, int wincap, int winmaxw,
-                                              bool aligned_list = true) {
+__device__ __forceinline__ Window window_at(const Geom& g, int x0, int y0, int x1, int y1, double t_lo, double t_hi, const double* __restrict__ mm4,
+                                            double tau, int wincap, int winmaxw, bool aligned_list) {
     const bool aligned = aligned_list && g.pitch_aligned != 0;
-    const int tx = it.tile % g.tilesX, ty = it.tile / g.tilesX;
-    const int x0 = tx * TS, y0 = ty * TS;
-    const int x1 = min(x0 + TS, g.W) - 1, y1 = min(y0 + TS, g.H) - 1;
-    const double dlo = it.t_lo - tau, dhi = it.t_hi - tau;
+    const double dlo = t_lo - tau, dhi = t_hi - tau;
     const double LIM = 4096.0;
     double lo[2], hi[2];
 #pragma unroll
@@ -136,6 +128,17 @@
     }
     Window w; w.ox = bx0; w.oy = by0; w.ww = ww; w.wh = wh;
     return w;
+}
+__device__ __forceinline__ Window item_window(const Geom& g, const Item& it, const double* __restrict__ mm4, double tau, int wincap, int winmaxw,
+                                              bool aligned_list = true) {
+    const int tx = it.tile % g.tilesX, ty = it.tile / g.tilesX;
+    const int x0 = tx * TS, y0 = ty * TS;
+    const int x1 = min(x0 + TS, g.W) - 1, y1 = min(y0 + TS, g.H) - 1;
+    return window_at(g, x0, y0, x1, y1, it.t_lo, it.t_hi, mm4, tau, wincap, winmaxw, aligned_list);
+}
+__device__ __forceinline__ Window item_window(const Geom& g, const SegRec& q, const double* __restrict__ mm4, double tau, int wincap, int winmaxw,
+                                              bool aligned_list = true) {
+    return window_at(g, q.x0, q.y0, q.x1, q.y1, q.t_lo, q.t_hi, mm4, tau, wincap, winmaxw, aligned_list);
 }
 
 __device__ __forceinline__ void warp_axis(int x, double v, double dt, int& ir, float& f) {
@@ -496,6 +499,31 @@
     return true;
 }
 
+__device__ __forceinline__ bool block_to_job(const Geom& g, int n_items, int R, const SegRec* __restrict__ recs, const Item* __restrict__ items,
+                                             const int32_t* __restrict__ order, SegRec& q, int& r) {
+    const int b = blockIdx.x;
+    const int xcd = b % NXCD, slot = b / NXCD;
+    const int rank = (slot / R) * NXCD + xcd;
+    r = slot % R;
+    if (rank >= n_items) return false;
+#ifdef EINCM_NO_JOB_RECORDS
+    const int item = order ? order[rank] : rank;
+    q = seg_record(g, items[item], item);
+#else
+    typedef int32_t rec16 __attribute__((ext_vector_type(16)));
+    static_assert(sizeof(rec16) == sizeof(SegRec), "a record is one 64-byte load");
+    q = __builtin_bit_cast(SegRec, *reinterpret_cast<const rec16*>(recs + rank));
+#endif
+    return true;
+}
+struct EdgeArg { double v[EDGE_ARG_MAX]; };
+constexpr int ARG_THETA = 1, ARG_EDGE_TS = 2;
+__device__ __forceinline__ double edge_time(int use_arg, const EdgeArg& earg, const double* __restrict__ edge_ts, int i) {
+    typedef const double __attribute__((address_space(4))) * const_f64;
+    const double* p = (use_arg & ARG_EDGE_TS) ? &earg.v[i] : edge_ts + i;
+    return *(const_f64)p;
+}
+
 template <int NTH> struct WinWalkT {
     int i, row, col, q, rem, ww;
     __device__ __forceinline__ WinWalkT(int tid, int ww_) : ww(ww_) {
@@ -585,18 +613,21 @@
         const Window* __restrict__ wins,
         unsigned long long* __restrict__ acc,
         const int32_t* __restrict__ order,
-        int use_arg, const double* __restrict__ theta_c, ThetaArg targ,
+        const SegRec* __restrict__ recs,
+        int use_arg_bits, const double* __restrict__ theta_c, ThetaArg targ,
+        EdgeArg earg,
         const float* __restrict__ ev_w = nullptr)
 {
     constexpr int theta_mode = TM;
+    const int use_arg = use_arg_bits & ARG_THETA;
     extern __shared__ __attribute__((aligned(16))) uint32_t ldsu[];
     double2* thtile = reinterpret_cast<double2*>(ldsu + g.wincap);
-    int item, r;
-    if (!block_to_work(n_items, g.R, order, item, r)) return;
-    const Item it = items[item];
+    SegRec it; int r;
+    if (!block_to_job(g, n_items, g.R, recs, items, order, it, r)) return;
+    const int item = it.seg;
     if (!win_active(g, it.win)) return;
-    const double tau = edge_ts[it.win * g.R + r];
-    const int tx0 = (it.tile % g.tilesX) * TS, ty0 = (it.tile / g.tilesX) * TS;
+    const double tau = edge_time(use_arg_bits, earg, edge_ts, it.win * g.R + r);
+    const int tx0 = it.x0, ty0 = it.y0;
     double2 vconst = make_double2(0.0, 0.0);
     Window wn;
     if (theta_mode == THETA_CONST) {
@@ -628,7 +659,7 @@
     const uint32_t* __restrict__ exy = ev_xy + it.begin;
     const double* __restrict__ et = ev_t + it.begin;
     const int n = it.count;
-    const int fshift = fix_shift(n);
+    const int fshift = it.fshift;
     const float FIX_SCALE = ldexpf(1.0f, fshift);
     const int up = ACC_SHIFT - fshift;
 
@@ -1256,8 +1287,9 @@
         long long* __restrict__ gTheta,
         double* __restrict__ g11,
         const WinConst* __restrict__ wc, const unsigned* __restrict__ gmax,
-        const int32_t* __restrict__ order,
-        int use_arg, const double* __restrict__ theta_c, ThetaArg targ,
+        const int32_t* __restrict__ order, const SegRec* __restrict__ recs,
+        int use_arg_bits, const double* __restrict__ theta_c, ThetaArg targ,
+        EdgeArg earg,
         int h, int w, const double* __restrict__ AH, const double* __restrict__ AW, const TileRange* __restrict__ tilerng,
         long long* __restrict__ gth_main, int gth_cap,
         int tail, unsigned* __restrict__ ticket, const int32_t* __restrict__ win_item0, double* __restrict__ grad_out,
@@ -1266,18 +1298,19 @@
 {
     constexpr int theta_mode = TM;
     constexpr bool direct11 = TM == THETA_CONST;
+    const int use_arg = use_arg_bits & ARG_THETA;
     const int wincap = g.wincap_a, winmaxw = g.winmaxw_a;
     extern __shared__ __attribute__((aligned(16))) float lds[];
     __shared__ double red11[NTH / 64];
     unsigned long long* accum = reinterpret_cast<unsigned long long*>(lds + wincap);
     double2* thtile = reinterpret_cast<double2*>(lds + wincap + (direct11 ? 0 : TS * TS * 4));
     float f11x = 0.0f, f11y = 0.0f;
-    int item, r;
+    SegRec it; int r;
     constexpr bool all_r = ALLR != 0;
-    if (!block_to_work(n_items, all_r ? 1 : g.R, order, item, r)) return;
-    const Item it = items[item];
+    if (!block_to_job(g, n_items, all_r ? 1 : g.R, recs, items, order, it, r)) return;
+    const int item = it.seg;
     if (!win_active(g, it.win)) return;
-    double tau = edge_ts[it.win * g.R + r];
+    double tau = edge_time(use_arg_bits, earg, edge_ts, it.win * g.R + r);
     const int lane = threadIdx.x & 63, wv = threadIdx.x >> 6;
     double2 vconst = make_double2(0.0, 0.0);
     Window wn;
@@ -1287,7 +1320,7 @@
         wn = item_window(g, it, mm4, tau, wincap, winmaxw);
     } else if (theta_mode == THETA_POLY) {
         double mm4[4];
-        poly_fill_tile<NTH>(g, it.win, (it.tile % g.tilesX) * TS, (it.tile / g.tilesX) * TS, use_arg, theta_c, targ, thtile,
+        poly_fill_tile<NTH>(g, it.win, it.x0, it.y0, use_arg, theta_c, targ, thtile,
                             reinterpret_cast<double*>(thtile + TS * TS), mm4);
         wn = item_window(g, it, mm4, tau, wincap, winmaxw, false);
     } else {
@@ -1296,8 +1329,7 @@
     int wp = (theta_mode == THETA_CONST) ? win_pitch(g, wn.ww) : wn.ww;
     size_t img = ((size_t)it.win * g.R + r) * g.H * g.W;
     const float* __restrict__ Gi = G + img;
-    const int tx = it.tile % g.tilesX, ty = it.tile / g.tilesX;
-    const int x0 = tx * TS, y0 = ty * TS;
+    const int x0 = it.x0, y0 = it.y0;
     if (theta_mode == THETA_TILE) {
         const double* __restrict__ ThW = Theta + (size_t)it.win * g.H * g.W * 2;
         for (int p = threadIdx.x; p < TS * TS; p += NTH) {
@@ -1393,7 +1425,7 @@
 #endif
     if (!all_r || ++rr >= g.R) break;
     __syncthreads();
-    tau = edge_ts[it.win * g.R + rr];
+    tau = edge_time(use_arg_bits, earg, edge_ts, it.win * g.R + rr);
     if (theta_mode == THETA_POLY) {
         double mm4[4];
         poly_tile_bounds<NTH>(reinterpret_cast<const double*>(thtile + TS * TS), mm4);
diff --git a/edge-informed-contrast-maximization_amd/csrc/eincm_plan.h b/edge-informed-contrast-maximization_amd/csrc/eincm_plan.h
--- a/edge-informed-contrast-maximization_amd/csrc/eincm_plan.h
+++ b/edge-informed-contrast-maximization_amd/csrc/eincm_plan.h
@@ -28,6 +28,7 @@
     double tspan = 1.0;
     Item* d_items = nullptr;
     int32_t* d_order = nullptr;
+    SegRec* d_recs = nullptr;
     std::vector<Item> h_items;
     std::vector<int32_t> h_order;
     int32_t* d_win_item0 = nullptr;
@@ -454,6 +455,8 @@
     bool obj = false; ObjGeom og{};
     int wincap = 0, winmaxw = 0, pitch_aligned = 0, wincap_a = 0, winmaxw_a = 0;
     WinFit win_2{}; bool splat_short = false;
+    bool job_records = false;
+    bool edge_arg = false;
     bool use_arg = false, use_arg_big = false;
     bool need_theta_image = false;
     bool host_asm = false;
@@ -487,6 +490,7 @@
     bool no_big_arg = false;
     bool no_host_asm = false;
     int all_r = -1;
+    bool no_job_records = false;
 };
 
 inline void plan_windows_preset(const PlanCtx& c, EvalPlan& P) {
@@ -568,6 +572,8 @@
     const size_t nall = (size_t)g.B * P.nth;
 
     P.use_arg = !io.theta && !identity && nall <= (size_t)THETA_ARG_MAX;
+    P.job_records = !knobs.no_job_records;
+    P.edge_arg = P.job_records && g.B * g.R <= EDGE_ARG_MAX;
     P.use_arg_big = !io.theta && !identity && nall <= (size_t)THETA_ARG_BIG && !knobs.no_big_arg;
     P.theta_src = io.theta ? EvalPlan::THETA_DEVICE
                 : (P.use_arg_big && (P.use_arg || !two_dof)) ? EvalPlan::THETA_ARGS
diff --git a/edge-informed-contrast-maximization_amd/csrc/eincm_splat_window.hip.h b/edge-informed-contrast-maximization_amd/csrc/eincm_splat_window.hip.h
--- a/edge-informed-contrast-maximization_amd/csrc/eincm_splat_window.hip.h
+++ b/edge-informed-contrast-maximization_amd/csrc/eincm_splat_window.hip.h
@@ -76,17 +76,18 @@
         const double* __restrict__ tmm,
         const double* __restrict__ edge_ts,
         unsigned long long* __restrict__ acc,
-        const int32_t* __restrict__ order,
-        int use_arg, const double* __restrict__ theta_c, ThetaArg targ)
+        const int32_t* __restrict__ order, const SegRec* __restrict__ recs,
+        int use_arg_bits, const double* __restrict__ theta_c, ThetaArg targ, EdgeArg earg)
 {
     constexpr int K = 2 * RAD + 1;
+    const int use_arg = use_arg_bits & ARG_THETA;
     extern __shared__ __attribute__((aligned(16))) unsigned long long lds64[];
     double2* thtile = reinterpret_cast<double2*>(lds64 + g.wincap);
-    int item, r;
-    if (!block_to_work(n_items, g.R, order, item, r)) return;
-    const Item it = items[item];
+    SegRec q; int r;
+    if (!block_to_job(g, n_items, g.R, recs, items, order, q, r)) return;
+    const Item it = q.item();
     if (!win_active(g, it.win)) return;
-    const double tau = edge_ts[it.win * g.R + r];
+    const double tau = edge_time(use_arg_bits, earg, edge_ts, it.win * g.R + r);
     double mm4[4];
     const double2 vconst = window_velocity<TM>(g, it, use_arg, theta_c, targ, tmm, mm4);
     if (TM == THETA_TILE) stage_theta_tile(g, it, Theta, thtile);
diff --git a/edge-informed-contrast-maximization_amd/csrc/eincm_types.h b/edge-informed-contrast-maximization_amd/csrc/eincm_types.h
--- a/edge-informed-contrast-maximization_amd/csrc/eincm_types.h
+++ b/edge-informed-contrast-maximization_amd/csrc/eincm_types.h
@@ -1,4 +1,5 @@
 #pragma once
+#include <math.h>
 #include <stddef.h>
 #include <stdint.h>
 
@@ -39,6 +40,32 @@
     double t_lo, t_hi;
 };
 
+EINCM_HD int fix_shift(int count) {
+    const unsigned c = (unsigned)ceilf((float)count * 0.16f);
+    const int ceillog2 = (c <= 1u) ? 0 : (32 - __builtin_clz(c - 1u));
+    const int k = 32 - ceillog2;
+    return k < 30 ? k : 30;
+}
+
+struct alignas(64) SegRec {
+    int32_t win, tile, begin, count;
+    double t_lo, t_hi;
+    int32_t seg;
+    int32_t fshift;
+    int32_t x0, y0, x1, y1;
+    int32_t _pad[2];
+    EINCM_HD Item item() const { Item it; it.win = win; it.tile = tile; it.begin = begin; it.count = count; it.t_lo = t_lo; it.t_hi = t_hi; return it; }
+};
+EINCM_HD SegRec seg_record(const Geom& g, const Item& it, int seg) {
+    SegRec q;
+    q.win = it.win; q.tile = it.tile; q.begin = it.begin; q.count = it.count; q.t_lo = it.t_lo; q.t_hi = it.t_hi;
+    q.seg = seg; q.fshift = fix_shift(it.count);
+    q.x0 = (it.tile % g.tilesX) * TS; q.y0 = (it.tile / g.tilesX) * TS;
+    q.x1 = (q.x0 + TS < g.W ? q.x0 + TS : g.W) - 1; q.y1 = (q.y0 + TS < g.H ? q.y0 + TS : g.H) - 1;
+    q._pad[0] = 0; q._pad[1] = 0;
+    return q;
+}
+
 struct EvalParams {
     double alpha, beta, gamma, delta;
     int cur_pyr_lvl, contrast_kind;
@@ -47,6 +74,7 @@
 };
 
 constexpr int THETA_ARG_MAX = 128;
+constexpr int EDGE_ARG_MAX = 64;
 constexpr int THETA_ARG_BIG = 4096;
 constexpr int THETA_ARG_MID = 512;
 
@@ -117,6 +145,8 @@
     double zc[4][16];
 };
 
+static_assert(sizeof(SegRec) == 64 && alignof(SegRec) == 64 && offsetof(SegRec, t_lo) == offsetof(Item, t_lo) && offsetof(SegRec, seg) == 32 &&
+              offsetof(SegRec, x0) == 40, "SegRec layout");
 static_assert(sizeof(StatPart) == 64 && offsetof(StatPart, mn) == 0 && offsetof(StatPart, sG2) == 56, "StatPart layout");
 static_assert(sizeof(ImgScal) == IMGSCAL_N * 8 && offsetof(ImgScal, m) == 0 && offsetof(ImgScal, sG2) == 64, "ImgScal layout");
 static_assert(sizeof(WinConst) == 104 * 8 && offsetof(WinConst, c0_gradmag) == 0 && offsetof(WinConst, cntmax) == 103 * 8, "WinConst layout");
```
